# ru-wang/slam-plus-plus

Measured on AMD Instinct MI355X. Metric: Λ-solve block-nnz/sec + batch GN iters/sec, Venice BA, 1→8 MI355X, higher is better.
Workload: dtype f64; 1 GPU; venice871-shaped synthetic BA (871 cams, 530304 points, 2838740 observations, LM-damped); nnzb=3369915, n=1596138, mode=schur+dense, n_reduced=5226, schur_pairs=12875640, parallelism=single GPU

## Files before the change

include/spp_hip.h:

```cpp
#ifndef SPP_HIP_H
#define SPP_HIP_H

#include <stddef.h>
#include <stdint.h>

#ifdef __cplusplus
extern "C" {
#endif

#define SPP_OK            0
#define SPP_NOT_POSDEF    1
#define SPP_E_BADARG     -1
#define SPP_E_NOMEM      -2
#define SPP_E_HIP        -3
#define SPP_E_NO_DEVICE  -4
#define SPP_E_STATE      -5
#define SPP_E_UNSUPPORTED -6

#define SPP_MODE_AUTO     0
#define SPP_MODE_SPARSE   1
#define SPP_MODE_SCHUR    2
#define SPP_MODE_SCHUR_SPARSE 3

#define SPP_FLAG_PROFILE  1
#define SPP_FLAG_SCHUR_PARTIAL 2

typedef struct spp_ctx spp_ctx;

spp_ctx *spp_create(int device, int flags);
void spp_destroy(spp_ctx *ctx);
int spp_free_memory(spp_ctx *ctx);
int spp_last_error(const spp_ctx *ctx, char *buf, size_t buf_size);
double *spp_host_staging(spp_ctx *ctx, int64_t n_doubles);
int spp_set_stream(spp_ctx *ctx, void *hip_stream);
int spp_synchronize(spp_ctx *ctx);

int spp_analyze(spp_ctx *ctx, int64_t nb, const int64_t *h_col_ptr, const int64_t *h_row_idx,
	const int64_t *h_blk_off, const int32_t *h_dim, int mode);

int spp_set_shard(spp_ctx *ctx, int rank, int world_size);

#define SPP_MODE_SCHUR_MIS 4

#define SPP_INFO_MODE           0
#define SPP_INFO_N              1
#define SPP_INFO_NNZB           2
#define SPP_INFO_NVALS          3
#define SPP_INFO_FACTOR_NNZ     4
#define SPP_INFO_FACTOR_FLOPS   5
#define SPP_INFO_N_REDUCED      6
#define SPP_INFO_N_POSES        7
#define SPP_INFO_N_LANDMARKS    8
#define SPP_INFO_SCHUR_PAIRS    9
#define SPP_INFO_N_OBS          10
#define SPP_INFO_SOLVE_BYTES    11
#define SPP_INFO_N_SUPERNODES   12
#define SPP_INFO_N_LEVELS       13
#define SPP_INFO_S_LD           14
#define SPP_INFO_S_NNZB         15
#define SPP_INFO_DENSE_STREAMED 16
int spp_get_info(const spp_ctx *ctx, int what, int64_t *out);
int spp_get_ordering(const spp_ctx *ctx, int64_t *h_order);

#define SPP_ORDER_AMD 0
#define SPP_ORDER_ND  1
int spp_block_ordering(int64_t nb, const int64_t *col_ptr, const int64_t *row_idx, int method, int64_t *h_order);

int spp_schur_plan_host(int64_t nb, const int32_t *dim, const int64_t *col_ptr, const int64_t *row_idx, int shard_rank,
	int shard_world, int sparse_S, int64_t *out, double *seconds);

int spp_factor_solve(spp_ctx *ctx, const double *h_vals, double *h_rhs_inout);

int spp_factor_solve_device(spp_ctx *ctx, const double *d_vals, double *d_rhs_inout);

int spp_schur_buffer_size(const spp_ctx *ctx, int64_t *n_doubles);
int spp_schur_form(spp_ctx *ctx, const double *d_vals, const double *d_rhs, double *d_S_rhs);
int spp_schur_finish(spp_ctx *ctx, const double *d_vals, double *d_S_rhs, double *d_rhs_inout);
int spp_schur_packed_size(const spp_ctx *ctx, int64_t *n_doubles);
int spp_schur_pack(spp_ctx *ctx, const double *d_S_rhs, double *d_packed);
int spp_schur_unpack(spp_ctx *ctx, const double *d_packed, double *d_S_rhs);

int spp_assemble_analyze(spp_ctx *ctx, int64_t nv, const int32_t *h_dim,
	int64_t ne, const int64_t *h_v0, const int64_t *h_v1, int d0, int d1, int rd,
	int64_t unary_vertex);
int spp_assemble_get_structure(const spp_ctx *ctx, int64_t *h_col_ptr, int64_t *h_row_idx,
	int64_t *h_blk_off);
int spp_assemble_device(spp_ctx *ctx, const double *d_J0, const double *d_J1,
	const double *d_Omega, const double *d_r, double damping, double *d_vals_out, double *d_eta_out);
int spp_assemble_set_edge_weights(spp_ctx *ctx, const double *d_w);
int spp_edge_robust_weights_device(spp_ctx *ctx, int64_t n_edges, int rd, int kind, double scale, double param,
	const double *d_r, double *d_w_out);

int spp_se2_linearize_device(spp_ctx *ctx, int64_t n_edges, const int32_t *d_v0, const int32_t *d_v1,
	const double *d_poses, const double *d_measurements, double *d_J0, double *d_J1, double *d_r);
int spp_se2_update_device(spp_ctx *ctx, int64_t n_vertices, double *d_poses, const double *d_dx, int apply,
	double *h_dx_norm2);

int spp_se3_linearize_device(spp_ctx *ctx, int64_t n_edges, const int32_t *d_v0, const int32_t *d_v1,
	const double *d_poses, const double *d_measurements, double *d_J0, double *d_J1, double *d_r);
int spp_se3_update_device(spp_ctx *ctx, int64_t n_vertices, double *d_poses, const double *d_dx, int apply,
	double *h_dx_norm2);

int spp_ba_linearize_device(spp_ctx *ctx, int64_t n_obs, const int32_t *d_cam_of, const int32_t *d_pt_of,
	const double *d_cams, const double *d_intrinsics, const double *d_points, const double *d_measurements,
	double *d_J0, double *d_J1, double *d_r);
int spp_ba_update_device(spp_ctx *ctx, int64_t n_cams, double *d_cams, const int64_t *d_cam_dxoff,
	int64_t n_points, double *d_points, const int64_t *d_pt_dxoff, const double *d_dx, int64_t n_dx, int apply,
	double *h_dx_norm2);

int spp_edge_chi2_device(spp_ctx *ctx, int64_t n_edges, int rd, const double *d_r, const double *d_Omega, double *h_chi2);
int spp_edge_hessian_maxdiag_device(spp_ctx *ctx, int64_t n_edges, int rd, int d0, int d1, const double *d_J0,
	const double *d_J1, const double *d_Omega, double *h_max);
int spp_lm_gain_denominator_device(spp_ctx *ctx, int64_t n, const double *d_dx, const double *d_eta, double alpha,
	double *h_out);

int spp_device_malloc(spp_ctx *ctx, size_t bytes, void **d_ptr);
int spp_device_free(spp_ctx *ctx, void *d_ptr);
int spp_memcpy_h2d(spp_ctx *ctx, void *d_dst, const void *h_src, size_t bytes);
int spp_memcpy_d2h(spp_ctx *ctx, void *h_dst, const void *d_src, size_t bytes);
int spp_memcpy_d2d(spp_ctx *ctx, void *d_dst, const void *d_src, size_t bytes);

int spp_set_profiling(spp_ctx *ctx, int on);

#define SPP_PHASE_PERMUTE   0
#define SPP_PHASE_SCHUR_INV 1
#define SPP_PHASE_SCHUR_GEMM 2
#define SPP_PHASE_SCHUR_RHS 3
#define SPP_PHASE_FACTOR    4
#define SPP_PHASE_TRISOLVE  5
#define SPP_PHASE_BACKSUBST 6
#define SPP_PHASE_ASSEMBLE  7
#define SPP_PHASE_TOTAL     8
#define SPP_N_PHASES        9
int spp_get_phase_ms(spp_ctx *ctx, double *ms_out );
int spp_get_dominant_kernel(spp_ctx *ctx, double *ms_total, int64_t *n_launches, double *flops);

int spp_microbench_copy(spp_ctx *ctx, size_t bytes, int iters, double *gb_per_s);
int spp_microbench_mfma_f64(spp_ctx *ctx, int iters, double *tflops);
int spp_microbench_ctile(spp_ctx *ctx, int n, int iters, double *gb_per_s);
int spp_microbench_update(spp_ctx *ctx, int64_t m, int iters, double *ms_per_launch);

int spp_dense_potrf_upper(spp_ctx *ctx, double *d_A, int64_t n, int64_t ld);
int spp_dense_posv(spp_ctx *ctx, double *d_A, int64_t n, int64_t ld, double *d_b);
int spp_dense_posv_masked(spp_ctx *ctx, double *d_A, int64_t n, int64_t ld, double *d_b, const uint64_t *words, int64_t nwords);
int spp_tile_mask_host(int64_t n, int bs, int64_t nblk, const int32_t *i1, const int32_t *i2, int has_rhs, int fill,
	uint64_t *words, int64_t *n_updates);
int spp_schur_tile_mask_host(int64_t nb, const int32_t *dim, const int64_t *col_ptr, const int64_t *row_idx, int shard_rank,
	int shard_world, uint64_t *words);
int spp_tail_order_host(int64_t n, int has_rhs, const uint64_t *words, int64_t nwords, int resident, int early, double beta,
	int32_t *table, int32_t *info);
int spp_dense_gemm_tn_sub(spp_ctx *ctx, int64_t m, int64_t n, int64_t k,
	const double *d_A, int64_t lda, const double *d_B, int64_t ldb, double *d_C, int64_t ldc);
int spp_dense_gemm_tn_sub_upper(spp_ctx *ctx, int64_t m, int64_t n, int64_t k,
	const double *d_A, int64_t lda, const double *d_B, int64_t ldb, double *d_C, int64_t ldc);
int spp_dense_front_factor(spp_ctx *ctx, double *d_F, int64_t ld, int64_t w, int64_t h, double *d_image);

const char *spp_version(void);

#ifdef __cplusplus
}
#endif
#endif
```

slam_plus_plus_amd/api.py:

```python
import ctypes
import os

import numpy as np

_HERE = os.path.dirname(os.path.abspath(__file__))
LIB_PATH = os.environ.get("SPP_LIB") or os.path.join(_HERE, "libspp_hip.so")

SPP_OK, SPP_NOT_POSDEF = 0, 1
MODE_AUTO, MODE_SPARSE, MODE_SCHUR, MODE_SCHUR_SPARSE, MODE_SCHUR_MIS = 0, 1, 2, 3, 4
FLAG_PROFILE = 1
INFO = dict(MODE=0, N=1, NNZB=2, NVALS=3, FACTOR_NNZ=4, FACTOR_FLOPS=5, N_REDUCED=6, N_POSES=7,
            N_LANDMARKS=8, SCHUR_PAIRS=9, N_OBS=10, SOLVE_BYTES=11, N_SUPERNODES=12, N_LEVELS=13, S_LD=14, S_NNZB=15, DENSE_STREAMED=16)
PHASES = ["permute", "schur_inv", "schur_gemm", "schur_rhs", "factor", "trisolve", "backsubst", "assemble", "total"]

EXPORTS = [
    "spp_create", "spp_destroy", "spp_free_memory", "spp_last_error", "spp_host_staging", "spp_set_stream", "spp_synchronize",
    "spp_analyze", "spp_set_shard", "spp_get_info", "spp_get_ordering", "spp_factor_solve",
    "spp_factor_solve_device", "spp_schur_buffer_size", "spp_schur_form", "spp_schur_finish",
    "spp_schur_packed_size", "spp_schur_pack", "spp_schur_unpack",
    "spp_assemble_analyze", "spp_assemble_get_structure", "spp_assemble_device", "spp_assemble_set_edge_weights", "spp_device_malloc",
    "spp_device_free", "spp_memcpy_h2d", "spp_memcpy_d2h", "spp_memcpy_d2d", "spp_get_phase_ms", "spp_get_dominant_kernel",
    "spp_microbench_copy", "spp_microbench_mfma_f64", "spp_microbench_ctile", "spp_microbench_update", "spp_block_ordering", "spp_schur_plan_host", "spp_set_profiling", "spp_se2_linearize_device", "spp_se2_update_device", "spp_ba_linearize_device", "spp_ba_update_device", "spp_se3_linearize_device", "spp_se3_update_device", "spp_edge_chi2_device", "spp_edge_robust_weights_device", "spp_edge_hessian_maxdiag_device",
    "spp_lm_gain_denominator_device", "spp_dense_potrf_upper", "spp_dense_posv",
    "spp_dense_posv_masked", "spp_tile_mask_host", "spp_schur_tile_mask_host", "spp_tail_order_host",
    "spp_dense_gemm_tn_sub", "spp_dense_gemm_tn_sub_upper", "spp_dense_front_factor", "spp_version",
]

_lib = None
_c_i64p = ctypes.POINTER(ctypes.c_int64)
_c_i32p = ctypes.POINTER(ctypes.c_int32)
_c_f64p = ctypes.POINTER(ctypes.c_double)


class SppError(RuntimeError):
    """std::runtime_error of the C++ adapter (reference LinearSolver_Schur_GPU.cpp:734-797)."""


def load_library():
    global _lib
    if _lib is not None:
        return _lib
    if not os.path.exists(LIB_PATH):
        raise SppError("libspp_hip.so is not built: run `python -m slam_plus_plus_amd.build` "
                       "(hipcc --offload-arch=gfx950); there is no CPU fallback")
    lib = ctypes.CDLL(LIB_PATH)
    vp, i64, i32, dbl, cint = ctypes.c_void_p, ctypes.c_int64, ctypes.c_int32, ctypes.c_double, ctypes.c_int
    sig = {
        "spp_create": (vp, [cint, cint]),
        "spp_destroy": (None, [vp]),
        "spp_free_memory": (cint, [vp]),
        "spp_last_error": (cint, [vp, ctypes.c_char_p, ctypes.c_size_t]),
        "spp_host_staging": (vp, [vp, i64]),
        "spp_set_stream": (cint, [vp, vp]),
        "spp_synchronize": (cint, [vp]),
        "spp_analyze": (cint, [vp, i64, vp, vp, vp, vp, cint]),
        "spp_set_shard": (cint, [vp, cint, cint]),
        "spp_get_info": (cint, [vp, cint, _c_i64p]),
        "spp_get_ordering": (cint, [vp, vp]),
        "spp_factor_solve": (cint, [vp, vp, vp]),
        "spp_factor_solve_device": (cint, [vp, vp, vp]),
        "spp_schur_buffer_size": (cint, [vp, _c_i64p]),
        "spp_schur_form": (cint, [vp, vp, vp, vp]),
        "spp_schur_finish": (cint, [vp, vp, vp, vp]),
        "spp_schur_packed_size": (cint, [vp, _c_i64p]),
        "spp_schur_pack": (cint, [vp, vp, vp]),
        "spp_schur_unpack": (cint, [vp, vp, vp]),
        "spp_assemble_analyze": (cint, [vp, i64, vp, i64, vp, vp, cint, cint, cint, i64]),
        "spp_assemble_get_structure": (cint, [vp, vp, vp, vp]),
        "spp_assemble_device": (cint, [vp, vp, vp, vp, vp, dbl, vp, vp]),
        "spp_assemble_set_edge_weights": (cint, [vp, vp]),
        "spp_device_malloc": (cint, [vp, ctypes.c_size_t, ctypes.POINTER(vp)]),
        "spp_device_free": (cint, [vp, vp]),
        "spp_memcpy_h2d": (cint, [vp, vp, vp, ctypes.c_size_t]),
        "spp_memcpy_d2h": (cint, [vp, vp, vp, ctypes.c_size_t]),
        "spp_memcpy_d2d": (cint, [vp, vp, vp, ctypes.c_size_t]),
        "spp_get_phase_ms": (cint, [vp, _c_f64p]),
        "spp_get_dominant_kernel": (cint, [vp, _c_f64p, _c_i64p, _c_f64p]),
        "spp_microbench_copy": (cint, [vp, ctypes.c_size_t, cint, _c_f64p]),
        "spp_microbench_mfma_f64": (cint, [vp, cint, _c_f64p]),
        "spp_microbench_ctile": (cint, [vp, cint, cint, _c_f64p]),
        "spp_microbench_update": (cint, [vp, ctypes.c_int64, cint, _c_f64p]),
        "spp_block_ordering": (cint, [ctypes.c_int64, vp, vp, cint, vp]),
        "spp_schur_plan_host": (cint, [ctypes.c_int64, vp, vp, vp, cint, cint, cint, vp, vp]),
        "spp_set_profiling": (cint, [vp, cint]),
        "spp_se2_linearize_device": (cint, [vp, ctypes.c_int64, vp, vp, vp, vp, vp, vp, vp]),
        "spp_se2_update_device": (cint, [vp, ctypes.c_int64, vp, vp, cint, _c_f64p]),
        "spp_se3_linearize_device": (cint, [vp, ctypes.c_int64, vp, vp, vp, vp, vp, vp, vp]),
        "spp_se3_update_device": (cint, [vp, ctypes.c_int64, vp, vp, cint, _c_f64p]),
        "spp_edge_chi2_device": (cint, [vp, ctypes.c_int64, cint, vp, vp, _c_f64p]),
        "spp_edge_robust_weights_device": (cint, [vp, ctypes.c_int64, cint, cint, dbl, dbl, vp, vp]),
        "spp_edge_hessian_maxdiag_device": (cint, [vp, ctypes.c_int64, cint, cint, cint, vp, vp, vp, _c_f64p]),
        "spp_lm_gain_denominator_device": (cint, [vp, ctypes.c_int64, vp, vp, ctypes.c_double, _c_f64p]),
        "spp_ba_linearize_device": (cint, [vp, ctypes.c_int64, vp, vp, vp, vp, vp, vp, vp, vp, vp]),
        "spp_ba_update_device": (cint, [vp, ctypes.c_int64, vp, vp, ctypes.c_int64, vp, vp, vp, ctypes.c_int64, cint, _c_f64p]),
        "spp_dense_potrf_upper": (cint, [vp, vp, i64, i64]),
        "spp_dense_posv": (cint, [vp, vp, i64, i64, vp]),
        "spp_dense_posv_masked": (cint, [vp, vp, i64, i64, vp, vp, i64]),
        "spp_tile_mask_host": (cint, [i64, cint, i64, vp, vp, cint, cint, vp, vp]),
        "spp_schur_tile_mask_host": (cint, [i64, vp, vp, vp, cint, cint, vp]),
        "spp_tail_order_host": (cint, [i64, cint, vp, i64, cint, cint, dbl, vp, vp]),
        "spp_dense_gemm_tn_sub": (cint, [vp, i64, i64, i64, vp, i64, vp, i64, vp, i64]),
        "spp_dense_gemm_tn_sub_upper": (cint, [vp, i64, i64, i64, vp, i64, vp, i64, vp, i64]),
        "spp_dense_front_factor": (cint, [vp, vp, i64, i64, i64, vp]),
        "spp_version": (ctypes.c_char_p, []),
    }
    for name, (res, args) in sig.items():
        fn = getattr(lib, name)
        fn.restype = res
        fn.argtypes = args
    _lib = lib
    return lib


def _ptr(a):
    return a.ctypes.data_as(ctypes.c_void_p)


ORDER_AMD, ORDER_ND = 0, 1


def block_ordering(lam, method=ORDER_AMD):
    lib = load_library()
    col_ptr = np.ascontiguousarray(lam.col_ptr, dtype=np.int64)
    row_idx = np.ascontiguousarray(lam.row_idx, dtype=np.int64)
    out = np.empty(lam.nb, dtype=np.int64)
    code = lib.spp_block_ordering(lam.nb, _ptr(col_ptr), _ptr(row_idx), method, _ptr(out))
    if code != 0:
        raise SppError("spp_block_ordering failed: %d" % code)
    return out


def schur_plan_host(lam, shard_rank=0, shard_world=1, sparse_S=False, mis=False):
    lib = load_library()
    col_ptr = np.ascontiguousarray(lam.col_ptr, dtype=np.int64)
    row_idx = np.ascontiguousarray(lam.row_idx, dtype=np.int64)
    dim = np.ascontiguousarray(lam.dim, dtype=np.int32)
    out = np.zeros(8, dtype=np.int64)
    sec = ctypes.c_double(0.0)
    code = lib.spp_schur_plan_host(lam.nb, _ptr(dim), _ptr(col_ptr), _ptr(row_idx), shard_rank, shard_world,
                                   (1 if sparse_S else 0) | (2 if mis else 0), _ptr(out), ctypes.byref(sec))
    if code != 0:
        raise SppError("spp_schur_plan_host failed: %d" % code)
    keys = ("nc", "nl", "no", "n_pairs", "n_sblk", "n_items", "n_multi", "checksum")
    d = dict(zip(keys, (int(v) for v in out)))
    d["seconds"] = sec.value
    return d


def tile_mask_host(n, bs, i1, i2, has_rhs=True, fill=True):
    lib = load_library()
    i1 = np.ascontiguousarray(i1, dtype=np.int32)
    i2 = np.ascontiguousarray(i2, dtype=np.int32)
    words = np.zeros(64, dtype=np.uint64)
    upd = ctypes.c_int64(0)
    code = lib.spp_tile_mask_host(n, bs, i1.size, _ptr(i1), _ptr(i2), 1 if has_rhs else 0, 1 if fill else 0, _ptr(words),
                                  ctypes.byref(upd))
    if code < 0:
        raise SppError("spp_tile_mask_host failed: %d" % code)
    return words[:code].copy(), upd.value


def schur_tile_mask_host(lam, shard_rank=0, shard_world=1):
    lib = load_library()
    col_ptr = np.ascontiguousarray(lam.col_ptr, dtype=np.int64)
    row_idx = np.ascontiguousarray(lam.row_idx, dtype=np.int64)
    dim = np.ascontiguousarray(lam.dim, dtype=np.int32)
    words = np.zeros(64, dtype=np.uint64)
    code = lib.spp_schur_tile_mask_host(lam.nb, _ptr(dim), _ptr(col_ptr), _ptr(row_idx), shard_rank, shard_world, _ptr(words))
    if code < 0:
        raise SppError("spp_schur_tile_mask_host failed: %d" % code)
    return words[:code].copy()


def tail_order_host(n, words, has_rhs=True, resident=256, early=True, beta=0.0):
    lib = load_library()
    words = np.ascontiguousarray(words if words is not None else [], dtype=np.uint64)
    table = np.zeros(64 * 65 // 2 + 64, dtype=np.int32)
    info = np.zeros(5, dtype=np.int32)
    code = lib.spp_tail_order_host(int(n), 1 if has_rhs else 0, _ptr(words) if words.size else None, words.size, int(resident),
                                   1 if early else 0, float(beta), _ptr(table), _ptr(info))
    if code < 0:
        raise SppError("spp_tail_order_host failed: %d" % code)
    tiles = [(int(t) >> 16, int(t) & 0xffff) for t in table[:code]]
    return tiles, dict(zip(("n_early", "r_star", "rows_resident", "live_demand", "widest"), (int(v) for v in info)))


class DeviceArray:

    def __init__(self, ctx, n, dtype=np.float64):
        self.ctx, self.n, self.dtype = ctx, int(n), np.dtype(dtype)
        p = ctypes.c_void_p()
        ctx._check(ctx.lib.spp_device_malloc(ctx.h, self.n * self.dtype.itemsize, ctypes.byref(p)))
        self.ptr = p.value

    @classmethod
    def from_host(cls, ctx, arr):
        arr = np.ascontiguousarray(arr)
        d = cls(ctx, arr.size, arr.dtype)
        d.upload(arr)
        return d

    def upload(self, arr):
        arr = np.ascontiguousarray(arr, dtype=self.dtype)
        assert arr.size == self.n
        self.ctx._check(self.ctx.lib.spp_memcpy_h2d(self.ctx.h, self.ptr, _ptr(arr), arr.nbytes))

    def download(self):
        out = np.empty(self.n, dtype=self.dtype)
        self.ctx._check(self.ctx.lib.spp_memcpy_d2h(self.ctx.h, _ptr(out), self.ptr, out.nbytes))
        return out

    def copy_from(self, other):
        assert other.n * other.dtype.itemsize <= self.n * self.dtype.itemsize
        self.ctx._check(self.ctx.lib.spp_memcpy_d2d(self.ctx.h, self.ptr, other.ptr, other.n * other.dtype.itemsize))

    def free(self):
        if self.ptr:
            self.ctx.lib.spp_device_free(self.ctx.h, self.ptr)
            self.ptr = None


class Context:

    def __init__(self, device=0, flags=0):
        self.lib = load_library()
        self.h = self.lib.spp_create(int(device), int(flags))
        if not self.h:
            raise SppError("spp_create failed: no usable HIP device %d (the solver has no CPU fallback)" % device)

    def close(self):
        if getattr(self, "h", None):
            self.lib.spp_destroy(self.h)
            self.h = None

    def __del__(self):
        try:
            self.close()
        except Exception:
            pass

    def last_error(self):
        buf = ctypes.create_string_buffer(1024)
        self.lib.spp_last_error(self.h, buf, 1024)
        return buf.value.decode(errors="replace")

    def _check(self, code):
        if code < 0:
            if code == -2:
                raise MemoryError(self.last_error())
            raise SppError("spp error %d: %s" % (code, self.last_error()))
        return code

    def analyze(self, bcsc, mode=MODE_AUTO):
        self._keep = bcsc
        return self._check(self.lib.spp_analyze(self.h, bcsc.nb, _ptr(bcsc.col_ptr), _ptr(bcsc.row_idx),
                                                 _ptr(bcsc.blk_off), _ptr(bcsc.dim), mode))

    def set_shard(self, rank, world):
        return self._check(self.lib.spp_set_shard(self.h, rank, world))

    def info(self, key):
        out = ctypes.c_int64()
        self._check(self.lib.spp_get_info(self.h, INFO[key], ctypes.byref(out)))
        return out.value

    def ordering(self, nb):
        out = np.empty(nb, dtype=np.int64)
        self._check(self.lib.spp_get_ordering(self.h, _ptr(out)))
        return out

    def se2_linearize_device(self, n_edges, d_v0, d_v1, d_poses, d_meas, d_J0, d_J1, d_r):
        return self._check(self.lib.spp_se2_linearize_device(self.h, n_edges, d_v0, d_v1, d_poses, d_meas, d_J0, d_J1, d_r))

    def se2_update_device(self, n_vertices, d_poses, d_dx, apply=True):
        out = ctypes.c_double()
        self._check(self.lib.spp_se2_update_device(self.h, n_vertices, d_poses, d_dx, 1 if apply else 0, ctypes.byref(out)))
        return out.value ** 0.5

    def se3_linearize_device(self, n_edges, d_v0, d_v1, d_poses, d_meas, d_J0, d_J1, d_r):
        return self._check(self.lib.spp_se3_linearize_device(self.h, n_edges, d_v0, d_v1, d_poses, d_meas, d_J0, d_J1, d_r))

    def se3_update_device(self, n_vertices, d_poses, d_dx, apply=True):
        out = ctypes.c_double()
        self._check(self.lib.spp_se3_update_device(self.h, n_vertices, d_poses, d_dx, 1 if apply else 0, ctypes.byref(out)))
        return out.value ** 0.5

    def edge_robust_weights_device(self, n_edges, rd, d_r, d_w, scale, param=1.345, kind=0):
        return self._check(self.lib.spp_edge_robust_weights_device(self.h, n_edges, rd, kind, float(scale), float(param), d_r, d_w))

    def edge_chi2_device(self, n_edges, rd, d_r, d_Om):
        out = ctypes.c_double()
        self._check(self.lib.spp_edge_chi2_device(self.h, n_edges, rd, d_r, d_Om, ctypes.byref(out)))
        return out.value

    def edge_hessian_maxdiag_device(self, n_edges, rd, d0, d1, d_J0, d_J1, d_Om):
        out = ctypes.c_double()
        self._check(self.lib.spp_edge_hessian_maxdiag_device(self.h, n_edges, rd, d0, d1, d_J0, d_J1, d_Om, ctypes.byref(out)))
        return out.value

    def lm_gain_denominator_device(self, n, d_dx, d_eta, alpha):
        out = ctypes.c_double()
        self._check(self.lib.spp_lm_gain_denominator_device(self.h, n, d_dx, d_eta, float(alpha), ctypes.byref(out)))
        return out.value

    def ba_linearize_device(self, n_obs, d_cam_of, d_pt_of, d_cams, d_intr, d_points, d_meas, d_J0, d_J1, d_r):
        return self._check(self.lib.spp_ba_linearize_device(self.h, n_obs, d_cam_of, d_pt_of, d_cams, d_intr, d_points,
                                                            d_meas, d_J0, d_J1, d_r))

    def ba_update_device(self, n_cams, d_cams, d_cam_dxoff, n_points, d_points, d_pt_dxoff, d_dx, n_dx, apply=True):
        out = ctypes.c_double()
        self._check(self.lib.spp_ba_update_device(self.h, n_cams, d_cams, d_cam_dxoff, n_points, d_points, d_pt_dxoff,
                                                  d_dx, n_dx, 1 if apply else 0, ctypes.byref(out)))
        return out.value ** 0.5

    def set_profiling(self, on):
        return self._check(self.lib.spp_set_profiling(self.h, 1 if on else 0))

    def set_stream(self, stream_handle):
        return self._check(self.lib.spp_set_stream(self.h, ctypes.c_void_p(stream_handle)))

    def synchronize(self):
        return self._check(self.lib.spp_synchronize(self.h))

    def host_staging(self, n):
        p = self.lib.spp_host_staging(self.h, int(n))
        if not p:
            raise MemoryError(self.last_error())
        return np.ctypeslib.as_array(ctypes.cast(p, ctypes.POINTER(ctypes.c_double)), shape=(int(n),))

    def factor_solve(self, vals, rhs):
        vals = np.ascontiguousarray(vals, dtype=np.float64)
        x = np.array(rhs, dtype=np.float64, copy=True)
        code = self._check(self.lib.spp_factor_solve(self.h, _ptr(vals), _ptr(x)))
        return code, x

    def factor_solve_device(self, d_vals, d_rhs):
        return self._check(self.lib.spp_factor_solve_device(self.h, d_vals, d_rhs))

    def schur_buffer_size(self):
        out = ctypes.c_int64()
        self._check(self.lib.spp_schur_buffer_size(self.h, ctypes.byref(out)))
        return out.value

    def schur_packed_size(self):
        out = ctypes.c_int64()
        self._check(self.lib.spp_schur_packed_size(self.h, ctypes.byref(out)))
        return out.value

    def schur_pack(self, d_S, d_packed):
        return self._check(self.lib.spp_schur_pack(self.h, d_S, d_packed))

    def schur_unpack(self, d_packed, d_S):
        return self._check(self.lib.spp_schur_unpack(self.h, d_packed, d_S))

    def schur_form(self, d_vals, d_rhs, d_S):
        return self._check(self.lib.spp_schur_form(self.h, d_vals, d_rhs, d_S))

    def schur_finish(self, d_vals, d_S, d_rhs):
        return self._check(self.lib.spp_schur_finish(self.h, d_vals, d_S, d_rhs))

    def assemble_analyze(self, dim, v0, v1, d0, d1, rd, unary_vertex=-1):
        dim = np.ascontiguousarray(dim, dtype=np.int32)
        v0 = np.ascontiguousarray(v0, dtype=np.int64)
        v1 = np.ascontiguousarray(v1, dtype=np.int64)
        self._check(self.lib.spp_assemble_analyze(self.h, dim.size, _ptr(dim), v0.size, _ptr(v0), _ptr(v1),
                                                   d0, d1, rd, int(unary_vertex)))
        nb, nnzb = dim.size, self.info("NNZB")
        col_ptr = np.empty(nb + 1, dtype=np.int64)
        row_idx = np.empty(nnzb, dtype=np.int64)
        blk_off = np.empty(nnzb, dtype=np.int64)
        self._check(self.lib.spp_assemble_get_structure(self.h, _ptr(col_ptr), _ptr(row_idx), _ptr(blk_off)))
        from .blockcsc import BlockCSC
        return BlockCSC(dim, col_ptr, row_idx, blk_off, None, nvals=self.info("NVALS"))

    def assemble_set_edge_weights(self, d_w):
        return self._check(self.lib.spp_assemble_set_edge_weights(self.h, d_w))

    def assemble_device(self, d_J0, d_J1, d_Om, d_r, damping, d_vals, d_eta):
        return self._check(self.lib.spp_assemble_device(self.h, d_J0, d_J1, d_Om, d_r, float(damping), d_vals, d_eta))

    def phase_ms(self):
        out = np.zeros(len(PHASES))
        self._check(self.lib.spp_get_phase_ms(self.h, out.ctypes.data_as(_c_f64p)))
        return dict(zip(PHASES, out.tolist()))

    def dominant_kernel(self):
        ms, n, fl = ctypes.c_double(), ctypes.c_int64(), ctypes.c_double()
        self._check(self.lib.spp_get_dominant_kernel(self.h, ctypes.byref(ms), ctypes.byref(n), ctypes.byref(fl)))
        return ms.value, n.value, fl.value

    def microbench_copy(self, nbytes=1 << 30, iters=10):
        out = ctypes.c_double()
        self._check(self.lib.spp_microbench_copy(self.h, nbytes, iters, ctypes.byref(out)))
        return out.value

    def microbench_ctile(self, n=8192, iters=10):
        out = ctypes.c_double()
        self._check(self.lib.spp_microbench_ctile(self.h, n, iters, ctypes.byref(out)))
        return out.value

    def microbench_update(self, m=5120, iters=20):
        out = ctypes.c_double()
        self._check(self.lib.spp_microbench_update(self.h, m, iters, ctypes.byref(out)))
        return out.value

    def microbench_mfma_f64(self, iters=4000):
        out = ctypes.c_double()
        self._check(self.lib.spp_microbench_mfma_f64(self.h, iters, ctypes.byref(out)))
        return out.value


class CLinearSolver_HIP:
    _Tag = "CBlockwiseLinearSolverTag"

    def __init__(self, device=0, mode=MODE_AUTO, flags=0):
        self._ctx = Context(device, flags)
        self._mode = mode
        self._have_symbolic = False
        self._sig = None

    def Free_Memory(self):
        self._ctx._check(self._ctx.lib.spp_free_memory(self._ctx.h))
        self._have_symbolic = False

    def Clear_SymbolicDecomposition(self):
        self._have_symbolic = False

    def SymbolicDecomposition_Blocky(self, r_lambda):
        self._ctx.analyze(r_lambda, self._mode)
        self._have_symbolic = True
        self._sig = self._signature(r_lambda)
        return True

    @staticmethod
    def _signature(r_lambda):
        try:
            import xxhash
            h = xxhash.xxh3_64()
            for a in (r_lambda.col_ptr, r_lambda.row_idx, r_lambda.dim):
                h.update(np.ascontiguousarray(a).view(np.uint8))
            digest = h.intdigest()
        except ImportError:
            import zlib
            digest = 0
            for a in (r_lambda.col_ptr, r_lambda.row_idx, r_lambda.dim):
                digest = zlib.adler32(np.ascontiguousarray(a).view(np.uint8), digest)
        return (r_lambda.nb, r_lambda.nnzb, digest)

    def Solve_PosDef_Blocky(self, r_lambda, r_eta):
        assert r_eta.shape[0] == r_lambda.n, "eta length must equal the matrix dimension"
        if not self._have_symbolic or self._sig is None or self._sig != self._signature(r_lambda):
            self.SymbolicDecomposition_Blocky(r_lambda)
        code, x = self._ctx.factor_solve(r_lambda.vals, r_eta)
        if code == SPP_NOT_POSDEF:
            return False
        r_eta[:] = x
        return True

    def Solve_PosDef(self, r_lambda, r_eta):
        self.Clear_SymbolicDecomposition()
        return self.Solve_PosDef_Blocky(r_lambda, r_eta)

    @property
    def ctx(self):
        return self._ctx
```

slam_plus_plus_amd/csrc/spp_api.cpp:

```cpp

#include "spp_internal.h"
#include <string.h>
#include <new>

using namespace spp;

namespace spp {

void phases_reset(spp_ctx *ctx)
{
	if(!(ctx->flags & SPP_FLAG_PROFILE))
		return;
	if(!ctx->timer.created) {
		for(int i = 0; i < 2 * SPP_N_PHASES; ++ i)
			SPP_HIP_CHECK(hipEventCreate(&ctx->timer.ev[i]));
		ctx->timer.created = true;
	}
	for(int i = 0; i < SPP_N_PHASES; ++ i) {
		ctx->timer.used[i] = false;
		ctx->phase_ms[i] = 0;
	}
	ctx->dom_used = 0;
	ctx->dom_flops = 0;
}
// ... 166 lines not shown
	if(!ctx || n_doubles < 0)
		return nullptr;
	if((size_t)n_doubles <= ctx->h_staging_cap && ctx->h_staging)
		return ctx->h_staging;
	(void)hipSetDevice(ctx->device);
	(void)hipStreamSynchronize(ctx->stream);
	if(ctx->h_staging) {
		(void)hipHostFree(ctx->h_staging);
		ctx->h_staging = nullptr;
		ctx->h_staging_cap = 0;
	}
	const size_t want = (size_t)(n_doubles > 0 ? n_doubles : 1);
	if(hipHostMalloc((void**)&ctx->h_staging, want * sizeof(double), hipHostMallocDefault) != hipSuccess) {
		(void)hipGetLastError();
		ctx->h_staging = nullptr;
		ctx->last_error = "hipHostMalloc of the staging buffer failed";
		return nullptr;
	}
	ctx->h_staging_cap = want;
	return ctx->h_staging;
}

int spp_set_stream(spp_ctx *ctx, void *hip_stream)
{
	if(!ctx)
		return SPP_E_BADARG;
	(void)hipStreamSynchronize(ctx->stream);
	if(ctx->own_stream && ctx->stream)
		(void)hipStreamDestroy(ctx->stream);
	ctx->stream = (hipStream_t)hip_stream;
	ctx->own_stream = false;
	return SPP_OK;
}

int spp_synchronize(spp_ctx *ctx)
{
	if(!ctx)
		return SPP_E_BADARG;
	SPP_TRY(ctx)
	SPP_HIP_CHECK(hipStreamSynchronize(ctx->stream));
	dense_chain_check(ctx);
	return SPP_OK;
	SPP_CATCH(ctx)
}

int spp_set_profiling(spp_ctx *ctx, int on)
{
	if(!ctx)
		return SPP_E_BADARG;
	ctx->flags = on ? (ctx->flags | SPP_FLAG_PROFILE) : (ctx->flags & ~SPP_FLAG_PROFILE);
	return SPP_OK;
}

int spp_set_shard(spp_ctx *ctx, int rank, int world_size)
{
	if(!ctx || world_size < 1 || rank < 0 || rank >= world_size)
		return SPP_E_BADARG;
	ctx->shard_rank = rank;
	ctx->shard_world = world_size;
	return SPP_OK;
}

int spp_analyze(spp_ctx *ctx, int64_t nb, const int64_t *col_ptr, const int64_t *row_idx,
	const int64_t *blk_off, const int32_t *dim, int mode)
{
	if(!ctx)
		return SPP_E_BADARG;
	SPP_TRY(ctx)
	SPP_REQUIRE(nb > 0 && col_ptr && row_idx && blk_off && dim, SPP_E_BADARG, "spp_analyze: null or empty structure");
	SPP_REQUIRE(col_ptr[0] == 0 && col_ptr[nb] >= nb, SPP_E_BADARG, "spp_analyze: column pointers must start at 0 and hold every diagonal block");
	SPP_HIP_CHECK(hipSetDevice(ctx->device));
	ctx->mode = -1;
	VClock clk("spp_analyze");
	Structure st;
	st.nb = nb;
	st.nnzb = col_ptr[nb];
	st.col_ptr.assign(col_ptr, col_ptr + nb + 1);
	SPP_REQUIRE(st.nnzb >= nb, SPP_E_BADARG, "spp_analyze: fewer blocks than block columns");
	for(int64_t j = 0; j < nb; ++ j)
		SPP_REQUIRE(col_ptr[j + 1] > col_ptr[j], SPP_E_BADARG, "every block column needs its diagonal block");
	st.dim.assign(dim, dim + nb);
	st.base.resize(nb + 1);
	st.base[0] = 0;
	for(int64_t j = 0; j < nb; ++ j) {
		SPP_REQUIRE(dim[j] > 0 && dim[j] <= 8, SPP_E_BADARG, "block widths must be in 1..8");
		st.base[j + 1] = st.base[j] + dim[j];
	}
	st.n = st.base[nb];
	st.row_idx.resize(st.nnzb);
	st.blk_off.resize(st.nnzb);
	{
		const int nt = plan_threads(st.nnzb);
		std::vector<int64_t> jcut, nvals_t(nt, 0);
		balanced_cuts(st.col_ptr, nt, jcut);
		run_threads(nt, [&](int t) {
			const int64_t p0 = col_ptr[jcut[t]], p1 = col_ptr[jcut[t + 1]];
			if(p1 > p0) {
				memcpy(st.row_idx.data() + p0, row_idx + p0, (size_t)(p1 - p0) * sizeof(int64_t));
				memcpy(st.blk_off.data() + p0, blk_off + p0, (size_t)(p1 - p0) * sizeof(int64_t));
			}
			int64_t nv = 0;
			for(int64_t j = jcut[t]; j < jcut[t + 1]; ++ j) {
				for(int64_t p = col_ptr[j]; p < col_ptr[j + 1]; ++ p) {
					const int64_t i = row_idx[p];
					SPP_REQUIRE(i >= 0 && i <= j, SPP_E_BADARG, "only the upper triangle may be stored");
					SPP_REQUIRE(p == col_ptr[j] || row_idx[p - 1] < i, SPP_E_BADARG, "rows must ascend within a column");
					SPP_REQUIRE(blk_off[p] >= 0, SPP_E_BADARG, "negative block offset");
					nv = std::max<int64_t>(nv, blk_off[p] + (int64_t)dim[i] * dim[j]);
				}
				SPP_REQUIRE(row_idx[col_ptr[j + 1] - 1] == j, SPP_E_BADARG, "diagonal block missing (must be last in its column)");
			}
			nvals_t[t] = nv;
		});
		st.nvals = 0;
		for(int t = 0; t < nt; ++ t)
			st.nvals = std::max(st.nvals, nvals_t[t]);
	}
	ctx->st = std::move(st);
	Structure &st_ref = ctx->st;
	clk.lap("structure copied + validated");
	ctx->schur.release_all();
	sparse_release(ctx);
	clk.lap("old plans released");
	int dp, dl;
	int chosen = mode;
	if(mode == SPP_MODE_AUTO) {
		chosen = SPP_MODE_SPARSE;
		if(schur_applicable(st_ref, &dp, &dl)) {
			int64_t n_red = 0;
			for(int64_t j = 0; j < nb; ++ j)
				n_red += (dim[j] == dp) ? dp : 0;
			chosen = (n_red <= 16384) ? SPP_MODE_SCHUR : SPP_MODE_SCHUR_SPARSE;
		}
	}
	SPP_REQUIRE(chosen == SPP_MODE_SCHUR || chosen == SPP_MODE_SPARSE || chosen == SPP_MODE_SCHUR_SPARSE ||
		chosen == SPP_MODE_SCHUR_MIS, SPP_E_BADARG, "unknown mode");
	SPP_REQUIRE((chosen != SPP_MODE_SPARSE && chosen != SPP_MODE_SCHUR_MIS) || ctx->shard_world == 1, SPP_E_UNSUPPORTED,
		"only the Schur modes shard (over landmarks); pose graphs run as replicas (DESIGN.md, multi-GPU)");
	ctx->mode = -1;
	if(chosen == SPP_MODE_SCHUR || chosen == SPP_MODE_SCHUR_SPARSE || chosen == SPP_MODE_SCHUR_MIS) {
		const bool mis = chosen == SPP_MODE_SCHUR_MIS;
		const bool sparse_S = chosen != SPP_MODE_SCHUR;
		build_schur_plan(ctx, sparse_S, mis);
		clk.lap("schur plan (all of it)");
		ctx->schur.mis = mis;
		ctx->order.clear();
		ctx->order.reserve((size_t)st_ref.nb);
		if(sparse_S) {
			sparse_analyze(ctx, ctx->schur.s_st);
			std::vector<int64_t> red = ctx->order;
			ctx->order.clear();
			for(size_t i = 0; i < red.size(); ++ i)
				ctx->order.push_back(ctx->schur.pose_block[red[i]]);
			chosen = SPP_MODE_SCHUR;
		} else
		for(size_t i = 0; i < ctx->schur.pose_block.size(); ++ i)
			ctx->order.push_back(ctx->schur.pose_block[i]);
		for(int64_t j = 0; j < st_ref.nb; ++ j)
			if(ctx->schur.is_lm[j])
				ctx->order.push_back(j);
	} else
		sparse_analyze(ctx, ctx->st);
	ctx->mode = chosen;
	clk.lap("plan + ordering");
	return SPP_OK;
	SPP_CATCH(ctx)
}

int spp_get_info(const spp_ctx *ctx, int what, int64_t *out)
{
	if(!ctx || !out)
		return SPP_E_BADARG;
	if(ctx->mode < 0 && what != SPP_INFO_NNZB && what != SPP_INFO_NVALS && what != SPP_INFO_N && what != SPP_INFO_DENSE_STREAMED)
		return SPP_E_STATE;
	switch(what) {
	case SPP_INFO_MODE: *out = (ctx->mode != SPP_MODE_SCHUR) ? ctx->mode : ctx->schur.mis ? SPP_MODE_SCHUR_MIS :
		ctx->schur.sparse_S ? SPP_MODE_SCHUR_SPARSE : SPP_MODE_SCHUR; break;
	case SPP_INFO_N: *out = ctx->st.n; break;
	case SPP_INFO_NNZB: *out = ctx->st.nnzb; break;
	case SPP_INFO_NVALS: *out = ctx->st.nvals; break;
	case SPP_INFO_FACTOR_NNZ: *out = ctx->factor_nnz; break;
	case SPP_INFO_FACTOR_FLOPS: *out = ctx->factor_flops; break;
	case SPP_INFO_N_REDUCED: *out = (ctx->mode == SPP_MODE_SCHUR) ? ctx->schur.n_red : 0; break;
	case SPP_INFO_N_POSES: *out = (ctx->mode == SPP_MODE_SCHUR) ? ctx->schur.nc : ctx->st.nb; break;
	case SPP_INFO_N_LANDMARKS: *out = (ctx->mode == SPP_MODE_SCHUR) ? ctx->schur.nl : 0; break;
	case SPP_INFO_SCHUR_PAIRS: *out = (ctx->mode == SPP_MODE_SCHUR) ? ctx->schur.n_pairs : 0; break;
	case SPP_INFO_N_OBS: *out = (ctx->mode == SPP_MODE_SCHUR) ? ctx->schur.no : 0; break;
	case SPP_INFO_SOLVE_BYTES: *out = ctx->solve_bytes; break;
	case SPP_INFO_N_SUPERNODES: *out = ctx->sparse ? sparse_info(ctx, what) : 0; break;
	case SPP_INFO_N_LEVELS: *out = ctx->sparse ? sparse_info(ctx, what) : 0; break;
	case SPP_INFO_S_LD: *out = (ctx->mode == SPP_MODE_SCHUR && !ctx->schur.sparse_S) ? ctx->schur.ld : 0; break;
	case SPP_INFO_S_NNZB: *out = (ctx->mode == SPP_MODE_SCHUR) ? ctx->schur.n_sblk : 0; break;
	case SPP_INFO_DENSE_STREAMED: *out = ctx->dense.tail_rows_last; break;
	default: return SPP_E_BADARG;
	}
	return SPP_OK;
}

int spp_get_ordering(const spp_ctx *ctx, int64_t *h_order)
{
	if(!ctx || !h_order)
		return SPP_E_BADARG;
	if(ctx->mode < 0)
		return SPP_E_STATE;
	for(size_t i = 0; i < ctx->order.size(); ++ i)
		h_order[i] = ctx->order[i];
	return SPP_OK;
}

int spp_block_ordering(int64_t nb, const int64_t *col_ptr, const int64_t *row_idx, int method, int64_t *h_order)
{
	if(nb <= 0 || !col_ptr || !row_idx || !h_order || (method != SPP_ORDER_AMD && method != SPP_ORDER_ND))
		return SPP_E_BADARG;
	try {
		for(int64_t j = 0; j < nb; ++ j)
			for(int64_t p = col_ptr[j]; p < col_ptr[j + 1]; ++ p)
				if(row_idx[p] < 0 || row_idx[p] > j)
					return SPP_E_BADARG;
		std::vector<int64_t> order;
		if(method == SPP_ORDER_AMD)
			min_degree_order(nb, col_ptr, row_idx, order);
		else
			nested_dissection_order(nb, col_ptr, row_idx, order);
		for(int64_t k = 0; k < nb; ++ k)
			h_order[k] = order[k];
		return SPP_OK;
	} catch(const std::bad_alloc &) {
		return SPP_E_NOMEM;
	} catch(...) {
		return SPP_E_HIP;
	}
}

static bool structure_of_pattern(int64_t nb, const int32_t *dim, const int64_t *col_ptr, const int64_t *row_idx, Structure &st)
{
	st.nb = nb;
	st.nnzb = col_ptr[nb];
	st.col_ptr.assign(col_ptr, col_ptr + nb + 1);
	st.row_idx.assign(row_idx, row_idx + st.nnzb);
	st.dim.assign(dim, dim + nb);
	st.base.resize(nb + 1);
	st.base[0] = 0;
	for(int64_t j = 0; j < nb; ++ j)
		st.base[j + 1] = st.base[j] + dim[j];
	st.n = st.base[nb];
	st.blk_off.resize(st.nnzb);
	int64_t off = 0;
	for(int64_t j = 0; j < nb; ++ j)
		for(int64_t p = col_ptr[j]; p < col_ptr[j + 1]; ++ p) {
			if(row_idx[p] < 0 || row_idx[p] > j)
				return false;
			st.blk_off[p] = off;
			off += (int64_t)dim[row_idx[p]] * dim[j];
		}
	st.nvals = off;
	return true;
}

int spp_schur_plan_host(int64_t nb, const int32_t *dim, const int64_t *col_ptr, const int64_t *row_idx, int shard_rank,
	int shard_world, int sparse_S, int64_t *out, double *seconds)
{
	if(nb <= 0 || !dim || !col_ptr || !row_idx || !out || shard_world < 1 || shard_rank < 0 || shard_rank >= shard_world)
		return SPP_E_BADARG;
	try {
		Structure st;
		if(!structure_of_pattern(nb, dim, col_ptr, row_idx, st))
			return SPP_E_BADARG;
		const double sec = schur_plan_host_probe(st, shard_rank, shard_world, (sparse_S & 1) != 0, (sparse_S & 2) != 0, out);
		if(seconds)
			*seconds = sec;
		return SPP_OK;
	} catch(const Error &e) {
		return e.code;
	} catch(const std::bad_alloc &) {
		return SPP_E_NOMEM;
	} catch(...) {
		return SPP_E_HIP;
	}
}

int spp_schur_tile_mask_host(int64_t nb, const int32_t *dim, const int64_t *col_ptr, const int64_t *row_idx, int shard_rank,
	int shard_world, uint64_t *words)
{
	if(nb <= 0 || !dim || !col_ptr || !row_idx || !words || shard_world < 1 || shard_rank < 0 || shard_rank >= shard_world)
		return SPP_E_BADARG;
	try {
		Structure st;
		if(!structure_of_pattern(nb, dim, col_ptr, row_idx, st))
			return SPP_E_BADARG;
		std::vector<uint64_t> w;
		schur_tile_mask_host_probe(st, shard_rank, shard_world, w);
		for(size_t q = 0; q < w.size(); ++ q)
			words[q] = w[q];
		return (int)w.size();
	} catch(const Error &e) {
		return e.code;
	} catch(const std::bad_alloc &) {
		return SPP_E_NOMEM;
	} catch(...) {
		return SPP_E_HIP;
	}
}

int spp_schur_buffer_size(const spp_ctx *ctx, int64_t *n_doubles)
{
	if(!ctx || !n_doubles)
		return SPP_E_BADARG;
	if(ctx->mode != SPP_MODE_SCHUR)
		return SPP_E_STATE;
	*n_doubles = schur_buffer_doubles(ctx);
	return SPP_OK;
}

int spp_schur_form(spp_ctx *ctx, const double *d_vals, const double *d_rhs, double *d_S_rhs)
{
	if(!ctx || !d_vals || !d_rhs || !d_S_rhs)
		return SPP_E_BADARG;
	SPP_TRY(ctx)
	SPP_REQUIRE(ctx->mode == SPP_MODE_SCHUR, SPP_E_STATE, "spp_schur_form: analyze in Schur mode first");
	SPP_HIP_CHECK(hipSetDevice(ctx->device));
	phases_reset(ctx);
	phase_begin(ctx, SPP_PHASE_TOTAL);
	schur_form(ctx, d_vals, d_rhs, d_S_rhs);
	return SPP_OK;
	SPP_CATCH(ctx)
}

int spp_schur_packed_size(const spp_ctx *ctx, int64_t *n_doubles)
{
	if(!ctx || !n_doubles)
		return SPP_E_BADARG;
	if(ctx->mode != SPP_MODE_SCHUR)
		return SPP_E_STATE;
	if(ctx->schur.sparse_S) {
		*n_doubles = schur_buffer_doubles(ctx);
		return SPP_OK;
	}
	const int64_t nblk = ctx->schur.ld / DENSE_NB;
	*n_doubles = (int64_t)DENSE_NB * DENSE_NB * (nblk * (nblk + 1) / 2);
	return SPP_OK;
}

int spp_schur_pack(spp_ctx *ctx, const double *d_S_rhs, double *d_packed)
{
	if(!ctx || !d_S_rhs || !d_packed)
		return SPP_E_BADARG;
	SPP_TRY(ctx)
	SPP_REQUIRE(ctx->mode == SPP_MODE_SCHUR, SPP_E_STATE, "spp_schur_pack: analyze in Schur mode first");
	SPP_HIP_CHECK(hipSetDevice(ctx->device));
	if(ctx->schur.sparse_S)
		SPP_HIP_CHECK(hipMemcpyAsync(d_packed, d_S_rhs, (size_t)schur_buffer_doubles(ctx) * sizeof(double),
			hipMemcpyDeviceToDevice, ctx->stream));
	else
		schur_pack(ctx, const_cast<double*>(d_S_rhs), d_packed, true);
	return SPP_OK;
	SPP_CATCH(ctx)
}

int spp_schur_unpack(spp_ctx *ctx, const double *d_packed, double *d_S_rhs)
{
	if(!ctx || !d_S_rhs || !d_packed)
		return SPP_E_BADARG;
	SPP_TRY(ctx)
	SPP_REQUIRE(ctx->mode == SPP_MODE_SCHUR, SPP_E_STATE, "spp_schur_unpack: analyze in Schur mode first");
	SPP_HIP_CHECK(hipSetDevice(ctx->device));
	if(ctx->schur.sparse_S)
		SPP_HIP_CHECK(hipMemcpyAsync(d_S_rhs, d_packed, (size_t)schur_buffer_doubles(ctx) * sizeof(double),
			hipMemcpyDeviceToDevice, ctx->stream));
	else
		schur_pack(ctx, d_S_rhs, const_cast<double*>(d_packed), false);
	return SPP_OK;
	SPP_CATCH(ctx)
}

int spp_schur_finish(spp_ctx *ctx, const double *d_vals, double *d_S_rhs, double *d_rhs_inout)
{
	if(!ctx || !d_vals || !d_rhs_inout || !d_S_rhs)
		return SPP_E_BADARG;
	SPP_TRY(ctx)
	SPP_REQUIRE(ctx->mode == SPP_MODE_SCHUR, SPP_E_STATE, "spp_schur_finish: analyze in Schur mode first");
	SPP_HIP_CHECK(hipSetDevice(ctx->device));
	int ret = schur_finish(ctx, d_vals, d_S_rhs, d_rhs_inout);
	phase_end(ctx, SPP_PHASE_TOTAL);
	phases_collect(ctx);
	dense_chain_check(ctx);
	return ret;
	SPP_CATCH(ctx)
}

int spp_factor_solve_device(spp_ctx *ctx, const double *d_vals, double *d_rhs)
{
	if(!ctx || !d_vals || !d_rhs)
		return SPP_E_BADARG;
	SPP_TRY(ctx)
	SPP_REQUIRE(ctx->mode >= 0, SPP_E_STATE, "spp_factor_solve: call spp_analyze first");
	SPP_HIP_CHECK(hipSetDevice(ctx->device));
	phases_reset(ctx);
	phase_begin(ctx, SPP_PHASE_TOTAL);
	int ret;
	if(ctx->mode == SPP_MODE_SCHUR) {
		SPP_REQUIRE(ctx->shard_world == 1, SPP_E_STATE,
			"sharded ctx: use spp_schur_form / all-reduce / spp_schur_finish");
		ctx->schur.S.reserve((size_t)schur_buffer_doubles(ctx));
		schur_form(ctx, d_vals, d_rhs, ctx->schur.S.p);
		ret = schur_finish(ctx, d_vals, ctx->schur.S.p, d_rhs);
	} else
		ret = sparse_factor_solve(ctx, d_vals, d_rhs);
	phase_end(ctx, SPP_PHASE_TOTAL);
	phases_collect(ctx);
	SPP_HIP_CHECK(hipStreamSynchronize(ctx->stream));
	dense_chain_check(ctx);
	return ret;
	SPP_CATCH(ctx)
}

int spp_factor_solve(spp_ctx *ctx, const double *h_vals, double *h_rhs)
{
	if(!ctx || !h_vals || !h_rhs)
		return SPP_E_BADARG;
	SPP_TRY(ctx)
	SPP_REQUIRE(ctx->mode >= 0, SPP_E_STATE, "spp_factor_solve: call spp_analyze first");
	SPP_HIP_CHECK(hipSetDevice(ctx->device));
	ctx->d_vals.reserve((size_t)ctx->st.nvals);
	ctx->d_rhs.reserve((size_t)ctx->st.n);
	SPP_HIP_CHECK(hipMemcpyAsync(ctx->d_vals.p, h_vals, ctx->st.nvals * sizeof(double), hipMemcpyHostToDevice, ctx->stream));
	SPP_HIP_CHECK(hipMemcpyAsync(ctx->d_rhs.p, h_rhs, ctx->st.n * sizeof(double), hipMemcpyHostToDevice, ctx->stream));
	int ret = spp_factor_solve_device(ctx, ctx->d_vals.p, ctx->d_rhs.p);
	if(ret != SPP_OK)
		return ret;
	SPP_HIP_CHECK(hipMemcpyAsync(h_rhs, ctx->d_rhs.p, ctx->st.n * sizeof(double), hipMemcpyDeviceToHost, ctx->stream));
	SPP_HIP_CHECK(hipStreamSynchronize(ctx->stream));
	return SPP_OK;
	SPP_CATCH(ctx)
}

int spp_assemble_analyze(spp_ctx *ctx, int64_t nv, const int32_t *h_dim, int64_t ne, const int64_t *h_v0,
	const int64_t *h_v1, int d0, int d1, int rd, int64_t unary_vertex)
{
	if(!ctx || !h_dim || !h_v0 || !h_v1 || nv <= 0 || ne <= 0)
		return SPP_E_BADARG;
	SPP_TRY(ctx)
	SPP_HIP_CHECK(hipSetDevice(ctx->device));
	assemble_analyze(ctx, nv, h_dim, ne, h_v0, h_v1, d0, d1, rd, unary_vertex);
	return SPP_OK;
	SPP_CATCH(ctx)
}

int spp_assemble_get_structure(const spp_ctx *ctx, int64_t *h_col_ptr, int64_t *h_row_idx, int64_t *h_blk_off)
{
	if(!ctx || !ctx->assemble)
		return SPP_E_STATE;
	assemble_get_structure(ctx, h_col_ptr, h_row_idx, h_blk_off);
	return SPP_OK;
}

int spp_assemble_device(spp_ctx *ctx, const double *d_J0, const double *d_J1, const double *d_Omega,
	const double *d_r, double damping, double *d_vals_out, double *d_eta_out)
{
	if(!ctx || !d_J0 || !d_J1 || !d_Omega || !d_r || !d_vals_out || !d_eta_out)
		return SPP_E_BADARG;
	SPP_TRY(ctx)
	SPP_REQUIRE(ctx->assemble, SPP_E_STATE, "spp_assemble_device: call spp_assemble_analyze first");
	SPP_HIP_CHECK(hipSetDevice(ctx->device));
	phases_reset(ctx);
	phase_begin(ctx, SPP_PHASE_ASSEMBLE);
	assemble_run(ctx, d_J0, d_J1, d_Omega, d_r, damping, d_vals_out, d_eta_out);
	phase_end(ctx, SPP_PHASE_ASSEMBLE);
	phases_collect(ctx);
	return SPP_OK;
	SPP_CATCH(ctx)
}

int spp_assemble_set_edge_weights(spp_ctx *ctx, const double *d_w)
{
	if(!ctx)
		return SPP_E_BADARG;
	SPP_TRY(ctx)
	SPP_REQUIRE(ctx->assemble, SPP_E_STATE, "spp_assemble_set_edge_weights: call spp_assemble_analyze first");
	assemble_set_edge_weights(ctx, d_w);
	return SPP_OK;
	SPP_CATCH(ctx)
}

int spp_se2_linearize_device(spp_ctx *ctx, int64_t n_edges, const int32_t *d_v0, const int32_t *d_v1,
	const double *d_poses, const double *d_measurements, double *d_J0, double *d_J1, double *d_r)
{
	if(!ctx || n_edges < 0 || !d_v0 || !d_v1 || !d_poses || !d_measurements || !d_J0 || !d_J1 || !d_r)
		return SPP_E_BADARG;
	SPP_TRY(ctx)
	SPP_HIP_CHECK(hipSetDevice(ctx->device));
	se2_linearize(ctx, n_edges, d_v0, d_v1, d_poses, d_measurements, d_J0, d_J1, d_r);
	return SPP_OK;
	SPP_CATCH(ctx)
}

int spp_se2_update_device(spp_ctx *ctx, int64_t n_vertices, double *d_poses, const double *d_dx, int apply,
	double *h_dx_norm2)
{
	if(!ctx || n_vertices < 0 || !d_poses || !d_dx)
		return SPP_E_BADARG;
	SPP_TRY(ctx)
	SPP_HIP_CHECK(hipSetDevice(ctx->device));
	const double n2 = se2_update(ctx, n_vertices, d_poses, d_dx, apply != 0);
	if(h_dx_norm2)
		*h_dx_norm2 = n2;
	return SPP_OK;
	SPP_CATCH(ctx)
}

int spp_se3_linearize_device(spp_ctx *ctx, int64_t n_edges, const int32_t *d_v0, const int32_t *d_v1,
	const double *d_poses, const double *d_measurements, double *d_J0, double *d_J1, double *d_r)
{
	if(!ctx || n_edges < 0 || !d_v0 || !d_v1 || !d_poses || !d_measurements || !d_J0 || !d_J1 || !d_r)
		return SPP_E_BADARG;
	SPP_TRY(ctx)
	SPP_HIP_CHECK(hipSetDevice(ctx->device));
	se3_linearize(ctx, n_edges, d_v0, d_v1, d_poses, d_measurements, d_J0, d_J1, d_r);
	return SPP_OK;
	SPP_CATCH(ctx)
}

int spp_se3_update_device(spp_ctx *ctx, int64_t n_vertices, double *d_poses, const double *d_dx, int apply,
	double *h_dx_norm2)
{
	if(!ctx || n_vertices < 0 || !d_poses || !d_dx)
		return SPP_E_BADARG;
	SPP_TRY(ctx)
	SPP_HIP_CHECK(hipSetDevice(ctx->device));
	const double n2 = se3_update(ctx, n_vertices, d_poses, d_dx, apply != 0);
	if(h_dx_norm2)
		*h_dx_norm2 = n2;
	return SPP_OK;
	SPP_CATCH(ctx)
}

int spp_ba_linearize_device(spp_ctx *ctx, int64_t n_obs, const int32_t *d_cam_of, const int32_t *d_pt_of,
	const double *d_cams, const double *d_intrinsics, const double *d_points, const double *d_measurements,
	double *d_J0, double *d_J1, double *d_r)
{
	if(!ctx || n_obs < 0 || !d_cam_of || !d_pt_of || !d_cams || !d_intrinsics || !d_points || !d_measurements ||
	   !d_J0 || !d_J1 || !d_r)
		return SPP_E_BADARG;
	SPP_TRY(ctx)
	SPP_HIP_CHECK(hipSetDevice(ctx->device));
	ba_linearize(ctx, n_obs, d_cam_of, d_pt_of, d_cams, d_intrinsics, d_points, d_measurements, d_J0, d_J1, d_r);
	return SPP_OK;
	SPP_CATCH(ctx)
}

int spp_ba_update_device(spp_ctx *ctx, int64_t n_cams, double *d_cams, const int64_t *d_cam_dxoff,
	int64_t n_points, double *d_points, const int64_t *d_pt_dxoff, const double *d_dx, int64_t n_dx, int apply,
	double *h_dx_norm2)
{
	if(!ctx || n_cams < 0 || n_points < 0 || n_dx < 0 || !d_dx || (n_cams && (!d_cams || !d_cam_dxoff)) ||
	   (n_points && (!d_points || !d_pt_dxoff)))
		return SPP_E_BADARG;
	SPP_TRY(ctx)
	SPP_HIP_CHECK(hipSetDevice(ctx->device));
	const double n2 = ba_update(ctx, n_cams, d_cams, d_cam_dxoff, n_points, d_points, d_pt_dxoff, d_dx, n_dx, apply != 0);
	if(h_dx_norm2)
		*h_dx_norm2 = n2;
	return SPP_OK;
	SPP_CATCH(ctx)
}

int spp_edge_robust_weights_device(spp_ctx *ctx, int64_t n_edges, int rd, int kind, double scale, double param,
	const double *d_r, double *d_w_out)
{
	if(!ctx || n_edges < 0 || !d_r || !d_w_out)
		return SPP_E_BADARG;
	SPP_TRY(ctx)
	SPP_HIP_CHECK(hipSetDevice(ctx->device));
	edge_robust_weights(ctx, n_edges, rd, kind, scale, param, d_r, d_w_out);
	return SPP_OK;
	SPP_CATCH(ctx)
}

int spp_edge_chi2_device(spp_ctx *ctx, int64_t n_edges, int rd, const double *d_r, const double *d_Omega, double *h_chi2)
{
	if(!ctx || n_edges < 0 || !d_r || !d_Omega || !h_chi2)
		return SPP_E_BADARG;
	SPP_TRY(ctx)
	SPP_HIP_CHECK(hipSetDevice(ctx->device));
	*h_chi2 = edge_chi2(ctx, n_edges, rd, d_r, d_Omega);
	return SPP_OK;
	SPP_CATCH(ctx)
}

int spp_edge_hessian_maxdiag_device(spp_ctx *ctx, int64_t n_edges, int rd, int d0, int d1, const double *d_J0,
	const double *d_J1, const double *d_Omega, double *h_max)
{
	if(!ctx || n_edges < 0 || !d_J0 || !d_J1 || !d_Omega || !h_max)
		return SPP_E_BADARG;
	SPP_TRY(ctx)
	SPP_HIP_CHECK(hipSetDevice(ctx->device));
	*h_max = edge_hessian_maxdiag(ctx, n_edges, rd, d0, d1, d_J0, d_J1, d_Omega);
	return SPP_OK;
	SPP_CATCH(ctx)
}

int spp_lm_gain_denominator_device(spp_ctx *ctx, int64_t n, const double *d_dx, const double *d_eta, double alpha,
	double *h_out)
{
	if(!ctx || n < 0 || !d_dx || !d_eta || !h_out)
		return SPP_E_BADARG;
	SPP_TRY(ctx)
// ... 279 lines not shown
```

slam_plus_plus_amd/csrc/spp_internal.h:

```cpp
#pragma once

#include <hip/hip_runtime.h>
#include <stdint.h>
#include <string>
#include <vector>
#include <sys/mman.h>
#include <utility>
#include <new>
#include <exception>
#include <thread>
#include <stdexcept>
#include <algorithm>
#include <string.h>
#include <chrono>
#include <stdio.h>
#include <stdlib.h>
#include "../../include/spp_hip.h"
#include "spp_switches.h"

namespace spp {

struct Error : std::runtime_error {
	int code;
	Error(int c, const std::string &what) : std::runtime_error(what), code(c) {}
};

#define SPP_HIP_CHECK(expr) do { hipError_t e_ = (expr); if(e_ != hipSuccess) \
	throw spp::Error(SPP_E_HIP, std::string(#expr " failed: ") + hipGetErrorString(e_)); } while(0)
#define SPP_REQUIRE(cond, code, msg) do { if(!(cond)) throw spp::Error((code), (msg)); } while(0)

inline bool first_on_this_device(uint64_t &seen)
{
	int dev = 0;
	(void)hipGetDevice(&dev);
	const uint64_t bit = uint64_t(1) << (dev & 63);
	if(seen & bit)
		return false;
	seen |= bit;
	return true;
}

struct VClock {
	const char *who;
	std::chrono::steady_clock::time_point t;
	bool on;
	explicit VClock(const char *w) : who(w), t(std::chrono::steady_clock::now()), on(switches().verbose) {}
	void lap(const char *what)
	{
		if(!on)
			return;
		const std::chrono::steady_clock::time_point n = std::chrono::steady_clock::now();
		fprintf(stderr, "[spp] %s: %-34s %8.2f ms\n", who, what, std::chrono::duration<double>(n - t).count() * 1e3);
		t = n;
	}
};

template <class T>
struct HugeAlloc {
	typedef T value_type;
	HugeAlloc() {}
	template <class U> HugeAlloc(const HugeAlloc<U>&) {}
	T *allocate(size_t n)
	{
		const size_t bytes = n * sizeof(T), huge = (size_t)2 << 20;
		void *q = nullptr;
		if(bytes >= ((size_t)4 << 20)) {
			if(posix_memalign(&q, huge, (bytes + huge - 1) & ~(huge - 1)) != 0)
				q = nullptr;
#ifdef MADV_HUGEPAGE
			if(q)
				madvise(q, bytes, MADV_HUGEPAGE);
#endif
		}
		if(!q)
			q = malloc(bytes ? bytes : 1);
		if(!q)
			throw std::bad_alloc();
		return (T*)q;
	}
	void deallocate(T *p, size_t) { free(p); }
	template <class U> void construct(U *p) { ::new((void*)p) U; }
	template <class U, class A0, class... A> void construct(U *p, A0 &&a0, A &&... a) { ::new((void*)p) U(std::forward<A0>(a0), std::forward<A>(a)...); }
	template <class U> bool operator==(const HugeAlloc<U>&) const { return true; }
	template <class U> bool operator!=(const HugeAlloc<U>&) const { return false; }
};
template <class T> using HVec = std::vector<T, HugeAlloc<T> >;

template <class T>
struct DevBuf {
	T *p = nullptr;
	size_t cap = 0;
	bool owned = true;
	DevBuf() {}
	DevBuf(const DevBuf&) = delete;
	DevBuf &operator=(const DevBuf&) = delete;
	~DevBuf() { release(); }
	void release()
	{
		if(p && owned)
			(void)hipFree(p);
		p = nullptr;
		cap = 0;
		owned = true;
	}
	void view(T *ptr, size_t n)
	{
		release();
		p = ptr;
		cap = n;
		owned = false;
	}
	void reserve(size_t n)
	{
		if(n <= cap && owned)
			return;
		release();
		size_t want = n;
		hipError_t e = hipMalloc((void**)&p, want * sizeof(T));
		if(e != hipSuccess) {
			p = nullptr;
			throw Error(SPP_E_NOMEM, "hipMalloc of " + std::to_string(want * sizeof(T)) + " bytes failed");
		}
		cap = want;
	}
	template <class A>
	void upload(const std::vector<T, A> &h, hipStream_t s)
	{
		reserve(h.size() ? h.size() : 1);
		if(!h.empty())
			SPP_HIP_CHECK(hipMemcpyAsync(p, h.data(), h.size() * sizeof(T), hipMemcpyHostToDevice, s));
	}
};

struct UploadArena {
	hipStream_t stream;
	std::vector<unsigned char> host;
	struct Item { void **pp; size_t *pcap; bool *powned; size_t off, n; };
	std::vector<Item> items;
	explicit UploadArena(hipStream_t s) : stream(s) { host.reserve(size_t(1) << 20); }
	template <class T, class A>
	void add(DevBuf<T> &b, const std::vector<T, A> &v)
	{
		if(v.size() * sizeof(T) > (size_t(256) << 10)) {
			b.upload(v, stream);
			return;
		}
		b.release();
		const size_t off = (host.size() + 255) & ~(size_t)255, bytes = std::max<size_t>(v.size(), 1) * sizeof(T);
		host.resize(off + bytes);
		if(!v.empty())
			memcpy(host.data() + off, v.data(), v.size() * sizeof(T));
		Item it = {(void**)&b.p, &b.cap, &b.owned, off, std::max<size_t>(v.size(), 1)};
		items.push_back(it);
	}
	void commit(DevBuf<unsigned char> &store)
	{
		store.release();
		store.reserve(std::max<size_t>(host.size(), 256));
		if(!host.empty())
			SPP_HIP_CHECK(hipMemcpyAsync(store.p, host.data(), host.size(), hipMemcpyHostToDevice, stream));
		for(size_t i = 0; i < items.size(); ++ i) {
			*items[i].pp = store.p + items[i].off;
			*items[i].pcap = items[i].n;
			*items[i].powned = false;
		}
	}
};

struct Structure {
	int64_t nb = 0, n = 0, nnzb = 0, nvals = 0;
	HVec<int64_t> col_ptr, row_idx, blk_off, base;
	HVec<int32_t> dim;
};

struct SaccItem {
	int32_t beg, end;
	int32_t kind;
	int32_t pad;
	int64_t dst;
	int64_t aoff;
};

struct SchurPlan {
	int dp = 0, dl = 0;
	int64_t nc = 0, nl = 0;
	int64_t nl_total = 0;
	int64_t no = 0;
	int64_t n_red = 0, ld = 0;
	int64_t n_sblk = 0;
	int64_t n_pairs = 0;
	int64_t n_items = 0, n_multi = 0;
	bool add_A = true;
	bool u_landmark_major = true;
	bool factored = true;
	bool sparse_S = false;
	bool mis = false;
	Structure s_st;
	DevBuf<int64_t> sblk_voff;
	std::vector<int64_t> pose_block;
	std::vector<int64_t> lm_block;
	std::vector<uint8_t> is_lm;
	std::vector<uint64_t> tile_mask;
	DevBuf<int32_t> lm_ptr;
	DevBuf<int32_t> bs_ptr;
	int64_t n_bs = 0;
	DevBuf<int64_t> lm_coff;
	DevBuf<int64_t> lm_rbase;
	DevBuf<int32_t> obs_pose;
	DevBuf<int32_t> obs_lm;
	DevBuf<int64_t> obs_off;
	DevBuf<int64_t> pose_rbase;
	DevBuf<int32_t> cam_ptr;
	DevBuf<int32_t> cam_obs;
	DevBuf<int32_t> obs_wpos;
	DevBuf<SaccItem> items;
	DevBuf<int32_t> xcd_beg;
	int32_t xcd_max_items = 0;
	DevBuf<int32_t> sblk_i1, sblk_i2;
	DevBuf<int64_t> sblk_aoff;
	DevBuf<int32_t> pair_a, pair_b;
	DevBuf<int32_t> multi_blk;
	DevBuf<int32_t> multi_ptr;
	DevBuf<double> cinv;
	DevBuf<double> lfac;
	DevBuf<double> W;
	DevBuf<double> Up;
	DevBuf<double> xw;
	DevBuf<double> partial;
	DevBuf<double> S;
	void release_all();
};

struct DenseWork {
	DevBuf<double> tinv;
	DevBuf<int> info;
	DevBuf<double> tinv_all;
	int64_t tinv_half = 0;
	DevBuf<double> xtmp;
	DevBuf<int> flags;
	DevBuf<int> tail_pub;
	DevBuf<double> tail_dinv;
	int tail_epoch = 0;
	DevBuf<int> tail_order;
	std::vector<int> tail_order_host;
	int tail_order_tr = 0, tail_order_tc = 0;
	std::vector<uint64_t> tail_order_bits;
	bool tail_order_pre = false, tail_order_masked = false;
	int tail_resident = -1;
	const std::vector<uint64_t> *tile_mask = nullptr;
	int tail_rows_last = 0;
	bool tail_disabled = false;
	DevBuf<double> trsv_m;
	DevBuf<double> trsv_pay;
	uint64_t epoch = 0;
	int *h_chain_err = nullptr;
	hipStream_t aux = nullptr;
	hipEvent_t ev[2] = {nullptr, nullptr};
	DevBuf<int> sync;
	DevBuf<int> fuse_cnt;
	std::vector<int> fuse_expect;
	bool fuse_dirty = false;
	int64_t ident_from = -1;
	hipStream_t chain = nullptr;
	hipEvent_t ev_chain = nullptr;
	DevBuf<int> la_cnt;
	DevBuf<long long> la_trace;
	int la_state = 0;
	int la_reserve = 0;
	int la_ncu = 0;
	int sync_epoch = 0;
	int sync_state = 0;
	hipStream_t sync_stream = nullptr;
};

struct SparsePlan;

struct AssemblePlan;

struct PhaseTimer {
	hipEvent_t ev[2 * SPP_N_PHASES];
	bool used[SPP_N_PHASES];
	bool created = false;
};

}

struct spp_ctx {
	int device = 0;
	int flags = 0;
	hipStream_t stream = nullptr;
	bool own_stream = false;
	std::string last_error;
	int mode = -1;
	int shard_rank = 0, shard_world = 1;
	spp::Structure st;
	std::vector<int64_t> order;
	std::thread plan_trash;
	spp::SchurPlan schur;
	spp::DenseWork dense;
	spp::SparsePlan *sparse = nullptr;
	spp::AssemblePlan *assemble = nullptr;
	spp::DevBuf<double> d_vals, d_rhs;
	double *h_staging = nullptr;
	size_t h_staging_cap = 0;
	spp::DevBuf<double> geom_partial;
	spp::PhaseTimer timer;
	double phase_ms[SPP_N_PHASES] = {0};
	std::vector<hipEvent_t> dom_events;
	size_t dom_used = 0;
	double dom_flops = 0;
	int64_t factor_flops = 0, solve_bytes = 0, factor_nnz = 0;
};

namespace spp {

void se2_linearize(spp_ctx *ctx, int64_t ne, const int32_t *d_v0, const int32_t *d_v1, const double *d_poses,
	const double *d_meas, double *d_J0, double *d_J1, double *d_r);
double se2_update(spp_ctx *ctx, int64_t nv, double *d_poses, const double *d_dx, bool apply);
double edge_chi2(spp_ctx *ctx, int64_t ne, int rd, const double *d_r, const double *d_Om);
void edge_robust_weights(spp_ctx *ctx, int64_t ne, int rd, int kind, double scale, double param, const double *d_r, double *d_w);
double edge_hessian_maxdiag(spp_ctx *ctx, int64_t ne, int rd, int d0, int d1, const double *d_J0, const double *d_J1,
	const double *d_Om);
double lm_gain_denominator(spp_ctx *ctx, int64_t n, const double *d_dx, const double *d_rhs, double alpha);
void se3_linearize(spp_ctx *ctx, int64_t ne, const int32_t *d_v0, const int32_t *d_v1, const double *d_poses,
	const double *d_meas, double *d_J0, double *d_J1, double *d_r);
double se3_update(spp_ctx *ctx, int64_t nv, double *d_poses, const double *d_dx, bool apply);
void ba_linearize(spp_ctx *ctx, int64_t no, const int32_t *d_cam_of, const int32_t *d_pt_of, const double *d_cams,
	const double *d_intr, const double *d_pts, const double *d_meas, double *d_J0, double *d_J1, double *d_r);
double ba_update(spp_ctx *ctx, int64_t nc, double *d_cams, const int64_t *d_cam_dxoff, int64_t np, double *d_pts,
	const int64_t *d_pt_dxoff, const double *d_dx, int64_t n_dx, bool apply);

void min_degree_order(int64_t nb, const int64_t *col_ptr, const int64_t *row_idx, std::vector<int64_t> &order);
void nested_dissection_order(int64_t nb, const int64_t *col_ptr, const int64_t *row_idx, std::vector<int64_t> &order);
void build_schur_plan(spp_ctx *ctx, bool sparse_S, bool mis = false);
int64_t schur_buffer_doubles(const spp_ctx *ctx);
bool schur_applicable(const Structure &st, int *dp, int *dl);
double schur_plan_host_probe(const Structure &st, int shard_rank, int shard_world, bool sparse_S, bool mis, int64_t *out);

void sparse_analyze(spp_ctx *ctx, const Structure &st);
int sparse_factor_solve(spp_ctx *ctx, const double *d_vals, double *d_rhs);
void sparse_release(spp_ctx *ctx);
void sparse_dag_disable(spp_ctx *ctx);
int64_t sparse_info(const spp_ctx *ctx, int what);

void schur_form(spp_ctx *ctx, const double *d_vals, const double *d_rhs, double *d_S_rhs);
int schur_finish(spp_ctx *ctx, const double *d_vals, double *d_S_rhs, double *d_rhs);
void schur_pack(spp_ctx *ctx, double *S, double *packed, bool pack);

constexpr int DENSE_NB = 128;
int dense_potrf_upper(spp_ctx *ctx, double *d_A, int64_t n, int64_t ld, bool keep_inverses);
void dense_potrf_upper_enqueue(spp_ctx *ctx, double *d_A, int64_t n, int64_t ld);
int dense_info_fetch(spp_ctx *ctx, bool *dag_aborted = nullptr);
void dense_potrs_upper(spp_ctx *ctx, const double *d_R, int64_t n, int64_t ld, double *d_b);
void dense_aux_park(int device, hipStream_t s);
void dense_factor_steps(spp_ctx *ctx, double *d_A, int64_t ld, int64_t n, int64_t rows, int64_t ncols,
	int64_t nsteps, bool has_rhs);
void dense_info_reset(spp_ctx *ctx);
void dense_reserve(spp_ctx *ctx, int64_t nblk);

void dense_chain_check(spp_ctx *ctx);
void dense_set_padding(spp_ctx *ctx, double *d_A, int64_t ld, int64_t n);
struct TileMaskGuard {
	DenseWork &d;
	TileMaskGuard(DenseWork &dw, const std::vector<uint64_t> *m) : d(dw) { d.tile_mask = (m && !m->empty()) ? m : nullptr; }
	~TileMaskGuard() { d.tile_mask = nullptr; }
};
void tile_mask_mark(int64_t n, int bs, int64_t nblk, const int32_t *i1, const int32_t *i2, std::vector<uint64_t> &words);
int64_t tile_mask_close(int64_t n, bool has_rhs, bool fill, std::vector<uint64_t> &words);
void schur_tile_mask_host_probe(const Structure &st, int shard_rank, int shard_world, std::vector<uint64_t> &words);
void tail_order_table(const std::vector<uint64_t> &bits, int Tr, int Tc, bool have_pre, double beta, int resident, bool early,
	std::vector<int> &order, int *info);
int dense_front_factor(spp_ctx *ctx, double *d_F, int64_t ld, int64_t w, int64_t h, double *d_image);
bool dense_gemm_tn_sub(spp_ctx *ctx, int64_t m, int64_t n, int64_t k, const double *A, int64_t lda,
	const double *B, int64_t ldb, double *C, int64_t ldc, bool upper_only);
double microbench_copy(spp_ctx *ctx, size_t bytes, int iters);
double microbench_mfma_f64(spp_ctx *ctx, int iters);
double microbench_ctile(spp_ctx *ctx, int n, int iters);
double microbench_update(spp_ctx *ctx, int64_t m, int iters);

void assemble_analyze(spp_ctx *ctx, int64_t nv, const int32_t *dim, int64_t ne, const int64_t *v0,
	const int64_t *v1, int d0, int d1, int rd, int64_t unary_vertex);
void assemble_run(spp_ctx *ctx, const double *J0, const double *J1, const double *Om, const double *r,
	double damping, double *vals, double *eta);
void assemble_set_edge_weights(spp_ctx *ctx, const double *d_w);
void assemble_release(spp_ctx *ctx);
void assemble_get_structure(const spp_ctx *ctx, int64_t *col_ptr, int64_t *row_idx, int64_t *blk_off);

void phase_begin(spp_ctx *ctx, int phase);
void phase_end(spp_ctx *ctx, int phase);
void phases_reset(spp_ctx *ctx);
void phases_collect(spp_ctx *ctx);
void dom_begin(spp_ctx *ctx);
void dom_end(spp_ctx *ctx, double flops);

template <class F>
inline void run_threads(int nt, F fn)
{
	if(nt <= 1) {
		fn(0);
		return;
	}
	std::vector<std::thread> th;
	std::exception_ptr err[64];
	for(int t = 1; t < nt; ++ t)
		th.emplace_back([&, t]() { try { fn(t); } catch(...) { err[t] = std::current_exception(); } });
	try { fn(0); } catch(...) { err[0] = std::current_exception(); }
	for(size_t t = 0; t < th.size(); ++ t)
		th[t].join();
	for(int t = 0; t < nt; ++ t)
		if(err[t])
			std::rethrow_exception(err[t]);
}

inline int plan_threads(int64_t work)
{
	const int env = switches().plan_threads;
	int nt = env ? env : (int)std::min<unsigned>(16u, std::max(1u, std::thread::hardware_concurrency()));
	if(work < switches().plan_min_work)
		nt = 1;
	return std::min(nt, 64);
}

template <class V>
inline void balanced_cuts(const V &w_prefix, int nt, std::vector<int64_t> &cut)
{
	const int64_t n = (int64_t)w_prefix.size() - 1, total = w_prefix[n];
	cut.assign(nt + 1, n);
	cut[0] = 0;
	for(int t = 1; t < nt; ++ t)
		cut[t] = std::lower_bound(w_prefix.begin(), w_prefix.end(), total * t / nt) - w_prefix.begin();
	for(int t = 1; t <= nt; ++ t)
		cut[t] = std::max(cut[t], cut[t - 1]);
	cut[nt] = n;
}


}
```

slam_plus_plus_amd/csrc/spp_schur.hip:

```cpp

#include "spp_internal.h"

namespace spp {

template <int DL>
__device__ __forceinline__ void cinv_block(const double *__restrict__ m, double *o)
{
	if(DL == 3) {
#define M_(i, j) m[(i) + 3 * (j)]
#define COF_(i, j) (M_(((i) + 1) % 3, ((j) + 1) % 3) * M_(((i) + 2) % 3, ((j) + 2) % 3) - \
	M_(((i) + 1) % 3, ((j) + 2) % 3) * M_(((i) + 2) % 3, ((j) + 1) % 3))
		const double c00 = COF_(0, 0), c10 = COF_(1, 0), c20 = COF_(2, 0);
		const double det = c00 * M_(0, 0) + c10 * M_(1, 0) + c20 * M_(2, 0);
		const double id = -1.0 / det;
		o[0] = c00 * id; o[3] = c10 * id; o[6] = c20 * id;
		o[1] = COF_(0, 1) * id; o[4] = COF_(1, 1) * id; o[7] = COF_(2, 1) * id;
		o[2] = COF_(0, 2) * id; o[5] = COF_(1, 2) * id; o[8] = COF_(2, 2) * id;
#undef COF_
#undef M_
	} else if(DL == 2) {
		const double det = m[0] * m[3] - m[2] * m[1];
		const double id = -1.0 / det;
		o[0] = m[3] * id; o[2] = -m[2] * id;
		o[1] = -m[1] * id; o[3] = m[0] * id;
	} else {
		double a[DL][DL], b[DL][DL];
#pragma unroll
		for(int i = 0; i < DL; ++ i)
#pragma unroll
			for(int j = 0; j < DL; ++ j) {
				a[i][j] = m[i + DL * j];
				b[i][j] = (i == j) ? 1.0 : 0.0;
			}
#pragma unroll
		for(int k = 0; k < DL; ++ k) {
			const double ip = 1.0 / a[k][k];
#pragma unroll
			for(int j = 0; j < DL; ++ j) {
				a[k][j] *= ip;
				b[k][j] *= ip;
			}
#pragma unroll
			for(int i = 0; i < DL; ++ i) {
				if(i == k)
					continue;
				const double f = a[i][k];
#pragma unroll
				for(int j = 0; j < DL; ++ j) {
					a[i][j] -= f * a[k][j];
					b[i][j] -= f * b[k][j];
				}
			}
		}
#pragma unroll
		for(int i = 0; i < DL; ++ i)
#pragma unroll
			for(int j = 0; j < DL; ++ j)
				o[i + DL * j] = -b[i][j];
	}
}

template <int DL>
__device__ __forceinline__ void lfac_block(const double *__restrict__ m, double *F)
{
	double G[DL][DL], Gi[DL][DL];
#pragma unroll
	for(int j = 0; j < DL; ++ j)
#pragma unroll
		for(int i = 0; i < DL; ++ i) {
			G[i][j] = 0;
			if(i < j)
				continue;
			double sum = m[i + DL * j];
#pragma unroll
			for(int t = 0; t < DL; ++ t)
				if(t < j)
					sum -= G[i][t] * G[j][t];
			G[i][j] = (i == j) ? sqrt(sum) : sum / G[j][j];
		}
#pragma unroll
	for(int j = 0; j < DL; ++ j)
#pragma unroll
		for(int i = 0; i < DL; ++ i) {
			Gi[i][j] = 0;
			if(i < j)
				continue;
			if(i == j) {
				Gi[i][j] = 1.0 / G[j][j];
				continue;
			}
			double sum = 0;
#pragma unroll
			for(int t = 0; t < DL; ++ t)
				if(t >= j && t < i)
					sum += G[i][t] * Gi[t][j];
			Gi[i][j] = -sum / G[i][i];
		}
#pragma unroll
	for(int q = 0; q < DL; ++ q)
#pragma unroll
		for(int t = 0; t < DL; ++ t)
			F[t + DL * q] = Gi[q][t];
}

template <int DL>
__global__ __launch_bounds__(256)
void cinv_kernel(int64_t nl, const int64_t *__restrict__ lm_coff, const double *__restrict__ vals,
	double *__restrict__ cinv, double *__restrict__ lfac)
{
	const int64_t l = (int64_t)blockIdx.x * blockDim.x + threadIdx.x;
	if(l >= nl)
		return;
	const double *m = vals + lm_coff[l];
	double o[DL * DL];
	cinv_block<DL>(m, o);
#pragma unroll
	for(int e = 0; e < DL * DL; ++ e)
		cinv[l * DL * DL + e] = o[e];
	if(lfac) {
		double F[DL * DL];
		lfac_block<DL>(m, F);
#pragma unroll
		for(int e = 0; e < DL * DL; ++ e)
			lfac[l * DL * DL + e] = F[e];
	}
}

template <int DP, int DL>
__device__ __forceinline__ void load_U(const double *__restrict__ vals, int64_t oo, double *U)
{
	const double *src = vals + (oo >> 1);
	if(oo & 1) {
#pragma unroll
		for(int r = 0; r < DP; ++ r)
#pragma unroll
			for(int q = 0; q < DL; ++ q)
				U[r + DP * q] = src[q + DL * r];
	} else {
#pragma unroll
		for(int e = 0; e < DP * DL; ++ e)
			U[e] = src[e];
	}
}

template <int DP, int DL>
__global__ __launch_bounds__(256)
void obs_kernel(int64_t no, const int32_t *__restrict__ obs_lm, const int64_t *__restrict__ obs_off,
	const int64_t *__restrict__ lm_rbase, const double *__restrict__ vals, const double *__restrict__ rhs,
	const double *__restrict__ cinv, const int32_t *__restrict__ obs_wpos, double *__restrict__ W,
	double *__restrict__ Up, double *__restrict__ xw, int u_lm)
{
	constexpr int BLK = DP * DL, ST = BLK | 1;
	__shared__ double img_all[4][64 * ST];
	__shared__ int32_t slot_all[4][64];
	const int lane = threadIdx.x & 63, wave = threadIdx.x >> 6;
	double *img = img_all[wave];
	int32_t *slot = slot_all[wave];
	const int64_t a0 = ((int64_t)blockIdx.x * 4 + wave) * 64, a = a0 + lane;
	const bool active = a < no;
	const int nact = (no - a0 < 64) ? (int)((no - a0 > 0) ? (no - a0) : 0) : 64;
	const int64_t oo = active ? obs_off[a] : 0;
	const int32_t l = active ? obs_lm[a] : 0;
	slot[lane] = active ? obs_wpos[a] : 0;
	double U[BLK];
	if(active)
		load_U<DP, DL>(vals, oo, U);
	else {
#pragma unroll
		for(int e = 0; e < BLK; ++ e)
			U[e] = 0;
	}
	double Ci[DL * DL];
#pragma unroll
	for(int e = 0; e < DL * DL; ++ e)
		Ci[e] = cinv[(int64_t)l * DL * DL + e];
	double lv[DL];
#pragma unroll
	for(int q = 0; q < DL; ++ q)
		lv[q] = active ? rhs[lm_rbase[l] + q] : 0.0;
	double Wl[DP], Wv[BLK];
#pragma unroll
	for(int r = 0; r < DP; ++ r)
		Wl[r] = 0;
#pragma unroll
	for(int q = 0; q < DL; ++ q)
#pragma unroll
		for(int r = 0; r < DP; ++ r) {
			double sum = 0;
#pragma unroll
			for(int t = 0; t < DL; ++ t)
				sum += U[r + DP * t] * Ci[t + DL * q];
			Wv[r + DP * q] = sum;
			Wl[r] += sum * lv[q];
		}
#pragma unroll
	for(int e = 0; e < BLK; ++ e)
		img[lane * ST + e] = Wv[e];
	__syncthreads();
	for(int p = lane; p < nact * BLK; p += 64) {
		const int j = p / BLK, e = p - j * BLK;
		W[(int64_t)slot[j] * BLK + e] = img[j * ST + e];
	}
	__syncthreads();
#pragma unroll
	for(int e = 0; e < BLK; ++ e)
		img[lane * ST + e] = U[e];
	__syncthreads();
	for(int p = lane; p < nact * BLK; p += 64) {
		const int j = p / BLK, e = p - j * BLK;
		Up[(u_lm ? a0 + j : (int64_t)slot[j]) * BLK + e] = img[j * ST + e];
	}
	__syncthreads();
#pragma unroll
	for(int r = 0; r < DP; ++ r)
		img[lane * (DP | 1) + r] = Wl[r];
	__syncthreads();
	for(int p = lane; p < nact * DP; p += 64) {
		const int j = p / DP, r = p - j * DP;
		xw[(int64_t)slot[j] * DP + r] = img[j * (DP | 1) + r];
	}
}

template <int BLK> struct VSplit { static constexpr int IL = (BLK == 18) ? 16 : BLK, SIDE = BLK - IL; };

template <int DP, int DL>
__global__ __launch_bounds__(256)
void obs_fact_kernel(int64_t no, const int32_t *__restrict__ obs_lm, const int64_t *__restrict__ obs_off,
	const int64_t *__restrict__ lm_rbase, const double *__restrict__ vals, const double *__restrict__ rhs,
	const double *__restrict__ lfac, const int64_t *__restrict__ lm_coff, const int32_t *__restrict__ obs_wpos, double *__restrict__ Vm, double *__restrict__ Vs,
	double *__restrict__ xw)
{
	constexpr int BLK = DP * DL, ST = BLK | 1, IL = VSplit<BLK>::IL, SIDE = VSplit<BLK>::SIDE;
	__shared__ double img_all[4][64 * ST];
	__shared__ int32_t slot_all[4][64];
	const int lane = threadIdx.x & 63, wave = threadIdx.x >> 6;
	double *img = img_all[wave];
	int32_t *slot = slot_all[wave];
	const int64_t a0 = ((int64_t)blockIdx.x * 4 + wave) * 64, a = a0 + lane;
	const bool active = a < no;
	const int nact = (no - a0 < 64) ? (int)((no - a0 > 0) ? (no - a0) : 0) : 64;
	const int64_t oo = active ? obs_off[a] : 0;
	const int32_t l = active ? obs_lm[a] : 0;
	slot[lane] = active ? obs_wpos[a] : 0;
	double U[BLK];
	if(active)
		load_U<DP, DL>(vals, oo, U);
	else {
#pragma unroll
		for(int e = 0; e < BLK; ++ e)
			U[e] = 0;
	}
	double F[DL * DL], lv[DL], tv[DL];
	if(lfac) {
#pragma unroll
		for(int e = 0; e < DL * DL; ++ e)
			F[e] = lfac[(int64_t)l * DL * DL + e];
	} else
		lfac_block<DL>(vals + lm_coff[l], F);
#pragma unroll
	for(int q = 0; q < DL; ++ q)
		lv[q] = active ? rhs[lm_rbase[l] + q] : 0.0;
#pragma unroll
	for(int q = 0; q < DL; ++ q) {
		double sum = 0;
#pragma unroll
		for(int u = 0; u < DL; ++ u)
			if(u <= q)
				sum += F[u + DL * q] * lv[u];
		tv[q] = sum;
	}
	double V[BLK], Wl[DP];
#pragma unroll
	for(int r = 0; r < DP; ++ r)
		Wl[r] = 0;
#pragma unroll
	for(int q = 0; q < DL; ++ q)
#pragma unroll
		for(int r = 0; r < DP; ++ r) {
			double sum = 0;
#pragma unroll
			for(int t = 0; t < DL; ++ t)
				if(t <= q)
					sum += U[r + DP * t] * F[t + DL * q];
			V[r + DP * q] = sum;
			Wl[r] -= sum * tv[q];
		}
#pragma unroll
	for(int e = 0; e < BLK; ++ e)
		img[lane * ST + e] = V[e];
	__syncthreads();
	for(int p = lane; p < nact * IL; p += 64) {
		const int j = p / IL, e = p - j * IL;
		Vm[a0 * IL + p] = img[j * ST + e];
	}
	if(SIDE)
		for(int p = lane; p < nact * SIDE; p += 64) {
			const int j = p / (SIDE ? SIDE : 1), e = p - j * SIDE;
			Vs[a0 * SIDE + p] = img[j * ST + IL + e];
		}
	__syncthreads();
#pragma unroll
	for(int r = 0; r < DP; ++ r)
		img[lane * (DP | 1) + r] = Wl[r];
	__syncthreads();
	for(int p = lane; p < nact * DP; p += 64) {
		const int j = p / DP, r = p - j * DP;
		xw[(int64_t)slot[j] * DP + r] = img[j * (DP | 1) + r];
	}
}

constexpr int SACC_WAVES = 4;
#ifndef SPP_SACC_RP
#define SPP_SACC_RP 64
#endif
#ifndef SPP_SACC_UCOL
#define SPP_SACC_UCOL 0
#endif
#ifndef SPP_SACC_GLDS
#define SPP_SACC_GLDS 1
#endif

__device__ __forceinline__ SaccItem sacc_load_item(const SaccItem *__restrict__ items, int32_t idx, int32_t lim)
{
	SaccItem r;
	r.beg = r.end = 0;
	r.kind = -1;
	r.pad = 0;
	r.dst = 0;
	r.aoff = -1;
	if(idx < lim)
		r = items[idx];
	return r;
}

#ifndef SPP_SACC_EU
#define SPP_SACC_EU 2
#endif
template <int DP, int DL, bool FACT>
__global__ __launch_bounds__(SACC_WAVES * 64) __attribute__((amdgpu_waves_per_eu(SPP_SACC_EU, SPP_SACC_EU)))
void s_accum_kernel(const SaccItem *__restrict__ items, const int32_t *__restrict__ xcd_beg, int chunk,
	const int32_t *__restrict__ pair_a, const int32_t *__restrict__ pair_b,
	const double *__restrict__ W, const double *__restrict__ Up, const double *__restrict__ vals,
	double *__restrict__ S, int64_t ld, double *__restrict__ partial)
{
	constexpr int NE = DP * DP, BLK = DP * DL;
	constexpr int IL = VSplit<BLK>::IL, SIDE = VSplit<BLK>::SIDE;
	constexpr int PW = (BLK & 1) ? 1 : 2;
	constexpr int PCS = BLK / PW;
	constexpr int PPI = 64 / PCS;
	constexpr int RP = SPP_SACC_RP;
	constexpr int NG = (RP + PPI - 1) / PPI;
	constexpr bool GLDS = (PW == 2) && (SPP_SACC_GLDS != 0);
	constexpr int ST = GLDS ? BLK : (BLK | 1);
	constexpr int NE2 = (NE + 1) / 2;
	constexpr int RS = 2 * NE2 + 2;
	constexpr int NSEG = 64 / NE2 < 3 ? 64 / NE2 : 3;
	constexpr int LW = (2 * RP * ST > RP * RS) ? 2 * RP * ST : RP * RS;
	__shared__ __attribute__((aligned(16))) double lds[SACC_WAVES][LW];
	const int wave = __builtin_amdgcn_readfirstlane(threadIdx.x >> 6), lane = threadIdx.x & 63;
	const int x = blockIdx.x & 7;
	const int32_t lim = xcd_beg[x + 1];
	int32_t idx = xcd_beg[x] + (int32_t)(blockIdx.x >> 3) * SACC_WAVES * chunk + wave;
	if(idx >= lim)
		return;
	int left = chunk;
	double *sw = lds[wave], *su = sw + RP * ST, *rw = sw;
	const int my_pair = lane / PCS, my_piece = lane % PCS;
	SaccItem cur = sacc_load_item(items, idx, lim);
	SaccItem nxt = sacc_load_item(items, (left > 1) ? idx + SACC_WAVES : lim, lim);
	SaccItem nn = nxt;
	int32_t q0 = cur.beg;
	int32_t pa = -1, pb = -1;
	if(lane < RP && q0 + lane < cur.end) {
		pa = pair_a[q0 + lane];
		pb = pair_b[q0 + lane];
	}
	double acc[NE];
#pragma unroll
	for(int e = 0; e < NE; ++ e)
		acc[e] = 0;
	for(;;) {
		const int nround = (cur.end - q0 < RP) ? cur.end - q0 : RP;
		const bool mine = lane < nround;
		const bool last = q0 + RP >= cur.end;
		const int32_t nq0 = last ? nxt.beg : q0 + RP, nend = last ? nxt.end : cur.end;
		int32_t pa_n = -1, pb_n = -1;
		if(lane < RP && nq0 + lane < nend) {
			pa_n = pair_a[nq0 + lane];
			pb_n = pair_b[nq0 + lane];
		}
		double aval0 = 0, aval1 = 0;
		if(last) {
			nn = sacc_load_item(items, (left > 2) ? idx + 2 * SACC_WAVES : lim, lim);
			if(cur.aoff >= 0 && lane < NE2) {
				aval0 = vals[cur.aoff + 2 * lane];
				if(2 * lane + 1 < NE)
					aval1 = vals[cur.aoff + 2 * lane + 1];
			}
		}
		if constexpr(GLDS) {
			int32_t ia[NG], ib[NG];
#pragma unroll
			for(int g = 0; g < NG; ++ g) {
				const int p = g * PPI + my_pair;
				ia[g] = __shfl(pa, p & 63);
				ib[g] = __shfl(pb, p & 63);
			}
#pragma unroll
			for(int g = 0; g < NG; ++ g) {
				const int p = g * PPI + my_pair;
				if(my_pair < PPI && p < nround) {
					const double *srca, *srcb;
					if(FACT) {
						const bool side = SIDE && 2 * my_piece >= IL;
						srca = side ? Up + (int64_t)ia[g] * SIDE + (2 * my_piece - IL) : W + (int64_t)ia[g] * IL + 2 * my_piece;
						srcb = side ? Up + (int64_t)ib[g] * SIDE + (2 * my_piece - IL) : W + (int64_t)ib[g] * IL + 2 * my_piece;
					} else {
						srca = W + (int64_t)ia[g] * BLK + 2 * my_piece;
						srcb = Up + (int64_t)ib[g] * BLK + 2 * my_piece;
					}
					__builtin_amdgcn_global_load_lds((const __attribute__((address_space(1))) void*)srca,
						(__attribute__((address_space(3))) void*)(sw + g * PPI * BLK), 16, 0, 0);
					__builtin_amdgcn_global_load_lds((const __attribute__((address_space(1))) void*)srcb,
						(__attribute__((address_space(3))) void*)(su + g * PPI * BLK), 16, 0, 0);
				}
			}
			asm volatile("s_waitcnt vmcnt(0)" ::: "memory");
		} else {
		constexpr int GC = (NG < 10) ? NG : 10;
#pragma unroll
		for(int g0 = 0; g0 < NG; g0 += GC) {
			int32_t ia[GC], ib[GC];
#pragma unroll
			for(int gg = 0; gg < GC; ++ gg) {
				const int p = (g0 + gg) * PPI + my_pair;
				ia[gg] = __shfl(pa, p & 63);
				ib[gg] = __shfl(pb, p & 63);
			}
			double tw[GC][PW], tu[GC][PW];
#pragma unroll
			for(int gg = 0; gg < GC; ++ gg) {
				int32_t xa = ia[gg] < 0 ? 0 : ia[gg], xb = ib[gg] < 0 ? 0 : ib[gg];
				if(PW == 2) {
					const double2 a2 = *(const double2*)(W + (int64_t)xa * BLK + 2 * my_piece);
					const double2 b2 = *(const double2*)((FACT ? W : Up) + (int64_t)xb * BLK + 2 * my_piece);
					tw[gg][0] = a2.x; tw[gg][PW - 1] = a2.y;
					tu[gg][0] = b2.x; tu[gg][PW - 1] = b2.y;
				} else {
					tw[gg][0] = W[(int64_t)xa * BLK + my_piece];
					tu[gg][0] = (FACT ? W : Up)[(int64_t)xb * BLK + my_piece];
				}
			}
#pragma unroll
			for(int gg = 0; gg < GC; ++ gg) {
				const int g = g0 + gg;
				const int p = g * PPI + my_pair;
				if(g < NG && my_pair < PPI && p < RP) {
#pragma unroll
					for(int t = 0; t < PW; ++ t) {
						sw[p * ST + PW * my_piece + t] = tw[gg][t];
						su[p * ST + PW * my_piece + t] = tu[gg][t];
					}
				}
			}
		}
		}
		__builtin_amdgcn_fence(__ATOMIC_ACQ_REL, "wavefront");
		__builtin_amdgcn_wave_barrier();
		if(mine) {
#if SPP_SACC_UCOL
			double w[BLK];
#pragma unroll
			for(int e = 0; e < BLK; ++ e)
				w[e] = sw[lane * ST + e];
#pragma unroll
			for(int c = 0; c < DP; ++ c) {
				double uc[DL];
#pragma unroll
				for(int t = 0; t < DL; ++ t)
					uc[t] = su[lane * ST + c + DP * t];
#pragma unroll
				for(int r = 0; r < DP; ++ r) {
					double sp = 0;
#pragma unroll
					for(int t = 0; t < DL; ++ t)
						sp += w[r + DP * t] * uc[t];
					acc[r + DP * c] += sp;
				}
			}
#else
			double w[BLK], u[BLK];
#pragma unroll
			for(int e = 0; e < BLK; ++ e) {
				w[e] = sw[lane * ST + e];
				u[e] = su[lane * ST + e];
			}
#pragma unroll
			for(int c = 0; c < DP; ++ c)
#pragma unroll
				for(int r = 0; r < DP; ++ r) {
					double sp = 0;
#pragma unroll
					for(int t = 0; t < DL; ++ t)
						sp += w[r + DP * t] * u[c + DP * t];
					acc[r + DP * c] += FACT ? -sp : sp;
				}
#endif
		}
		__builtin_amdgcn_fence(__ATOMIC_ACQ_REL, "wavefront");
		__builtin_amdgcn_wave_barrier();
		if(last) {
			int nact = cur.end - cur.beg;
			if(nact > RP)
				nact = RP;
			if(lane < RP) {
#pragma unroll
				for(int e = 0; e < NE; ++ e)
					rw[lane * RS + e] = acc[e];
			}
			__builtin_amdgcn_fence(__ATOMIC_ACQ_REL, "wavefront");
			__builtin_amdgcn_wave_barrier();
			const int seg_len = (nact + NSEG - 1) / NSEG;
			const int e2 = lane % NE2, sq = lane / NE2;
			double s0 = 0, s1 = 0;
			if(sq < NSEG) {
				const double *src = rw + (sq * seg_len) * RS + 2 * e2;
				const int len = (seg_len < RP - sq * seg_len) ? seg_len : RP - sq * seg_len;
				int l = 0;
				for(; l + 8 <= len; l += 8) {
					double2 t[8];
#pragma unroll
					for(int u = 0; u < 8; ++ u)
						t[u] = *(const double2*)(src + (l + u) * RS);
#pragma unroll
					for(int u = 0; u < 8; ++ u) {
						s0 += t[u].x;
						s1 += t[u].y;
					}
				}
				for(; l < len; ++ l) {
					const double2 t = *(const double2*)(src + l * RS);
					s0 += t.x;
					s1 += t.y;
				}
			}
			__builtin_amdgcn_fence(__ATOMIC_ACQ_REL, "wavefront");
			__builtin_amdgcn_wave_barrier();
			{
				const double g0 = s0, g1 = s1;
#pragma unroll
				for(int q = 1; q < NSEG; ++ q) {
					s0 += __shfl(g0, (lane + q * NE2) & 63);
					s1 += __shfl(g1, (lane + q * NE2) & 63);
				}
			}
			if(lane < NE2) {
				const int e = 2 * lane;
				const bool two = e + 1 < NE;
				double *dst;
				int64_t o0 = e, o1 = e + 1;
				if(cur.kind == 2)
					dst = partial + cur.dst;
				else {
					dst = S + cur.dst;
					if(cur.aoff >= 0) {
						s0 = aval0 + s0;
						s1 = aval1 + s1;
					}
					if(cur.kind == 0) {
						o0 = e % DP + (e / DP) * ld;
						o1 = (e + 1) % DP + ((e + 1) / DP) * ld;
					}
				}
				dst[o0] = s0;
				if(two)
					dst[o1] = s1;
			}
#pragma unroll
			for(int e = 0; e < NE; ++ e)
				acc[e] = 0;
			idx += SACC_WAVES;
			-- left;
			cur = nxt;
			nxt = nn;
			if(left == 0 || cur.kind < 0)
				break;
		}
		q0 = nq0;
		pa = pa_n;
		pb = pb_n;
	}
}

template <int DP>
__global__ __launch_bounds__(256)
void s_multi_kernel(int64_t n_multi, const int32_t *__restrict__ multi_blk, const int32_t *__restrict__ multi_ptr,
	const int32_t *__restrict__ sblk_i1, const int32_t *__restrict__ sblk_i2, const int64_t *__restrict__ sblk_aoff,
	const double *__restrict__ partial, const double *__restrict__ vals, int add_A, double *__restrict__ S, int64_t ld,
	const int64_t *__restrict__ sblk_voff)
{
	const int64_t m = (int64_t)blockIdx.x * (blockDim.x >> 6) + (threadIdx.x >> 6);
	const int lane = threadIdx.x & 63;
	if(m >= n_multi || lane >= DP * DP)
		return;
	const int32_t b = multi_blk[m];
	double acc = 0;
	for(int32_t s = multi_ptr[m]; s < multi_ptr[m + 1]; ++ s)
		acc += partial[(int64_t)s * DP * DP + lane];
	const int64_t aoff = sblk_aoff[b];
	if(add_A && aoff >= 0)
		acc = vals[aoff + lane] + acc;
	if(sblk_voff) {
		S[sblk_voff[b] + lane] = acc;
		return;
	}
	const int r = lane % DP, c = lane / DP;
	S[((int64_t)sblk_i1[b] * DP + r) + ((int64_t)sblk_i2[b] * DP + c) * ld] = acc;
}

template <int DP>
__global__ __launch_bounds__(256)
void rhs_kernel(int64_t nc, const int32_t *__restrict__ cam_ptr, const int32_t *__restrict__ cam_obs,
	const int64_t *__restrict__ pose_rbase, const double *__restrict__ xw, const double *__restrict__ rhs,
	int add_eta, double *__restrict__ xcol)
{
	const int64_t i = (int64_t)blockIdx.x * (blockDim.x >> 6) + (threadIdx.x >> 6);
	const int lane = threadIdx.x & 63;
	if(i >= nc)
		return;
	double s[DP];
#pragma unroll
	for(int r = 0; r < DP; ++ r)
		s[r] = 0;
	for(int32_t q = cam_ptr[i] + lane; q < cam_ptr[i + 1]; q += 64) {
		const double *x = xw + (int64_t)q * DP;
#pragma unroll
		for(int r = 0; r < DP; ++ r)
			s[r] += x[r];
	}
#pragma unroll
	for(int r = 0; r < DP; ++ r) {
#pragma unroll
		for(int off = 32; off > 0; off >>= 1)
			s[r] += __shfl_xor(s[r], off);
	}
	if(lane < DP) {
		double v = 0;
#pragma unroll
		for(int r = 0; r < DP; ++ r)
			if(lane == r)
				v = s[r];
		if(add_eta)
			v += rhs[pose_rbase[i] + lane];
		xcol[i * DP + lane] = v;
	}
}

template <int DP, int DL>
__global__ __launch_bounds__(256)
void backsubst_obs_kernel(int64_t no, const int32_t *__restrict__ obs_pose, const int64_t *__restrict__ obs_off,
	const double *__restrict__ vals, const double *__restrict__ dx, double *__restrict__ tq)
{
	const int64_t a = (int64_t)blockIdx.x * blockDim.x + threadIdx.x;
	if(a >= no)
		return;
	double u[DP * DL];
	load_U<DP, DL>(vals, obs_off[a], u);
	double dv[DP];
	const double *d = dx + (int64_t)obs_pose[a] * DP;
#pragma unroll
	for(int r = 0; r < DP; ++ r)
		dv[r] = d[r];
#pragma unroll
	for(int q = 0; q < DL; ++ q) {
		double sum = 0;
#pragma unroll
		for(int r = 0; r < DP; ++ r)
			sum += dv[r] * u[r + DP * q];
		tq[a * DL + q] = sum;
	}
}

template <int DL>
__global__ __launch_bounds__(256)
void backsubst_lm_kernel(int64_t nl, const int32_t *__restrict__ lm_ptr, const int64_t *__restrict__ lm_rbase,
	const double *__restrict__ tq, const double *__restrict__ cinv, const int64_t *__restrict__ lm_coff, const double *__restrict__ vals,
	double *__restrict__ rhs)
{
	const int64_t l = (int64_t)blockIdx.x * blockDim.x + threadIdx.x;
	if(l >= nl)
		return;
	double t[DL];
	const int64_t rb = lm_rbase[l];
#pragma unroll
	for(int q = 0; q < DL; ++ q)
		t[q] = -rhs[rb + q];
	for(int32_t a = lm_ptr[l]; a < lm_ptr[l + 1]; ++ a) {
#pragma unroll
		for(int q = 0; q < DL; ++ q)
			t[q] += tq[(int64_t)a * DL + q];
	}
	double Ci[DL * DL];
	if(cinv) {
#pragma unroll
		for(int e = 0; e < DL * DL; ++ e)
			Ci[e] = cinv[l * DL * DL + e];
	} else
		cinv_block<DL>(vals + lm_coff[l], Ci);
#pragma unroll
	for(int q = 0; q < DL; ++ q) {
		double sum = 0;
#pragma unroll
		for(int u = 0; u < DL; ++ u)
			sum += Ci[q + DL * u] * t[u];
		rhs[rb + q] = sum;
	}
}

template <int DP, int DL>
__global__ __launch_bounds__(256)
void backsubst_fused_kernel(const int32_t *__restrict__ bs_ptr, const int32_t *__restrict__ lm_ptr, const int32_t *__restrict__ obs_pose,
	const int64_t *__restrict__ obs_off, const int64_t *__restrict__ lm_rbase, const double *__restrict__ cinv,
	const int64_t *__restrict__ lm_coff, const double *__restrict__ vals, const double *__restrict__ dx, double *__restrict__ rhs)
{
	__shared__ double tq[256 * DL];
	const int32_t l0 = bs_ptr[blockIdx.x], l1 = bs_ptr[blockIdx.x + 1];
	const int32_t a0 = lm_ptr[l0], na = lm_ptr[l1] - a0;
	const int t = threadIdx.x;
	if(t < na) {
		const int64_t a = (int64_t)a0 + t;
		double u[DP * DL];
		load_U<DP, DL>(vals, obs_off[a], u);
		double dv[DP];
		const double *d = dx + (int64_t)obs_pose[a] * DP;
#pragma unroll
		for(int r = 0; r < DP; ++ r)
			dv[r] = d[r];
#pragma unroll
		for(int q = 0; q < DL; ++ q) {
			double sum = 0;
#pragma unroll
			for(int r = 0; r < DP; ++ r)
				sum += dv[r] * u[r + DP * q];
			tq[t * DL + q] = sum;
		}
	}
	__syncthreads();
	if(t >= l1 - l0)
		return;
	const int64_t l = (int64_t)l0 + t;
	double tv[DL];
	const int64_t rb = lm_rbase[l];
#pragma unroll
	for(int q = 0; q < DL; ++ q)
		tv[q] = -rhs[rb + q];
	for(int32_t a = lm_ptr[l] - a0, e = lm_ptr[l + 1] - a0; a < e; ++ a) {
#pragma unroll
		for(int q = 0; q < DL; ++ q)
			tv[q] += tq[a * DL + q];
	}
	double Ci[DL * DL];
	if(cinv) {
#pragma unroll
		for(int e = 0; e < DL * DL; ++ e)
			Ci[e] = cinv[l * DL * DL + e];
	} else
		cinv_block<DL>(vals + lm_coff[l], Ci);
#pragma unroll
	for(int q = 0; q < DL; ++ q) {
		double sum = 0;
#pragma unroll
		for(int u = 0; u < DL; ++ u)
			sum += Ci[q + DL * u] * tv[u];
		rhs[rb + q] = sum;
	}
}

template <int DP>
__global__ __launch_bounds__(256)
void scatter_dx_kernel(int64_t nc, const int64_t *__restrict__ pose_rbase, const double *__restrict__ dx,
	double *__restrict__ rhs)
{
	const int64_t e = (int64_t)blockIdx.x * blockDim.x + threadIdx.x;
	if(e >= nc * DP)
		return;
	rhs[pose_rbase[e / DP] + e % DP] = dx[e];
}

template <int DP, int DL>
static void schur_form_t(spp_ctx *ctx, const double *d_vals, const double *d_rhs, double *S)
{
	SchurPlan &sp = ctx->schur;
	hipStream_t s = ctx->stream;
	const int64_t ld = sp.ld;
	const int64_t *voff = sp.sparse_S ? sp.sblk_voff.p : nullptr;
	double *xcol = sp.sparse_S ? S + sp.s_st.nvals : S + sp.n_red * ld;
	phase_begin(ctx, SPP_PHASE_SCHUR_INV);
	if(S == sp.S.p && !sp.sparse_S && ctx->shard_world == 1 && sp.n_sblk == sp.nc * (sp.nc + 1) / 2 && sp.n_red == sp.nc * DP)
		SPP_HIP_CHECK(hipMemsetAsync(S + sp.n_red * ld, 0, (size_t)(schur_buffer_doubles(ctx) - sp.n_red * ld) * sizeof(double), s));
	else
		SPP_HIP_CHECK(hipMemsetAsync(S, 0, (size_t)schur_buffer_doubles(ctx) * sizeof(double), s));
	constexpr int VIL = VSplit<DP * DL>::IL;
	double *Vm = sp.W.p, *Vs = sp.W.p + sp.no * VIL;
	const bool onfly = sp.factored && DL <= 3;
	if(sp.nl && !onfly)
		hipLaunchKernelGGL((cinv_kernel<DL>), dim3((unsigned)((sp.nl + 255) / 256)), dim3(256), 0, s,
			sp.nl, sp.lm_coff.p, d_vals, sp.cinv.p, sp.factored ? sp.lfac.p : nullptr);
	if(sp.no && sp.factored)
		hipLaunchKernelGGL((obs_fact_kernel<DP, DL>), dim3((unsigned)((sp.no + 255) / 256)), dim3(256), 0, s,
			sp.no, sp.obs_lm.p, sp.obs_off.p, sp.lm_rbase.p, d_vals, d_rhs, onfly ? (const double*)nullptr : (const double*)sp.lfac.p, sp.lm_coff.p,
			sp.obs_wpos.p, Vm, Vs, sp.xw.p);
	else if(sp.no)
		hipLaunchKernelGGL((obs_kernel<DP, DL>), dim3((unsigned)((sp.no + 255) / 256)), dim3(256), 0, s,
			sp.no, sp.obs_lm.p, sp.obs_off.p, sp.lm_rbase.p, d_vals, d_rhs, sp.cinv.p, sp.obs_wpos.p, sp.W.p, sp.Up.p, sp.xw.p, sp.u_landmark_major ? 1 : 0);
	phase_end(ctx, SPP_PHASE_SCHUR_INV);
	phase_begin(ctx, SPP_PHASE_SCHUR_GEMM);
	if(sp.n_items) {
		int chunk = switches().sacc_chunk;
		if(chunk <= 0)
			chunk = (int)((sp.xcd_max_items + SACC_WAVES * 64 - 1) / (SACC_WAVES * 64));
		const int64_t per = (int64_t)SACC_WAVES * chunk;
		if(sp.factored)
			hipLaunchKernelGGL((s_accum_kernel<DP, DL, true>), dim3((unsigned)(8 * ((sp.xcd_max_items + per - 1) / per))), dim3(SACC_WAVES * 64), 0, s,
				sp.items.p, sp.xcd_beg.p, chunk, sp.pair_a.p, sp.pair_b.p, Vm, Vs, d_vals, S, ld, sp.partial.p);
		else
			hipLaunchKernelGGL((s_accum_kernel<DP, DL, false>), dim3((unsigned)(8 * ((sp.xcd_max_items + per - 1) / per))), dim3(SACC_WAVES * 64), 0, s,
				sp.items.p, sp.xcd_beg.p, chunk, sp.pair_a.p, sp.pair_b.p, sp.W.p, sp.Up.p, d_vals, S, ld, sp.partial.p);
	}
	if(sp.n_multi)
		hipLaunchKernelGGL((s_multi_kernel<DP>), dim3((unsigned)((sp.n_multi + 3) / 4)), dim3(256), 0, s,
			sp.n_multi, sp.multi_blk.p, sp.multi_ptr.p, sp.sblk_i1.p, sp.sblk_i2.p, sp.sblk_aoff.p,
			sp.partial.p, d_vals, sp.add_A ? 1 : 0, S, ld, voff);
	phase_end(ctx, SPP_PHASE_SCHUR_GEMM);
	phase_begin(ctx, SPP_PHASE_SCHUR_RHS);
	if(sp.nc)
		hipLaunchKernelGGL((rhs_kernel<DP>), dim3((unsigned)((sp.nc + 3) / 4)), dim3(256), 0, s,
			sp.nc, sp.cam_ptr.p, sp.cam_obs.p, sp.pose_rbase.p, sp.xw.p, d_rhs, sp.add_A ? 1 : 0, xcol);
	phase_end(ctx, SPP_PHASE_SCHUR_RHS);
	SPP_HIP_CHECK(hipGetLastError());
}

template <int DP, int DL>
static int schur_finish_t(spp_ctx *ctx, const double *d_vals, double *S, double *d_rhs)
{
	SchurPlan &sp = ctx->schur;
	hipStream_t s = ctx->stream;
	const int64_t ld = sp.ld;
	double *xcol;
	if(sp.sparse_S) {
		xcol = S + sp.s_st.nvals;
		const int ret = sparse_factor_solve(ctx, S, xcol);
		if(ret != SPP_OK)
			return ret;
	} else {
		phase_begin(ctx, SPP_PHASE_FACTOR);
		dense_set_padding(ctx, S, ld, sp.n_red);
		{
			TileMaskGuard guard(ctx->dense, &sp.tile_mask);
			dense_potrf_upper_enqueue(ctx, S, sp.n_red, ld);
		}
		phase_end(ctx, SPP_PHASE_FACTOR);
		xcol = S + sp.n_red * ld;
		phase_begin(ctx, SPP_PHASE_TRISOLVE);
		dense_potrs_upper(ctx, S, sp.n_red, ld, xcol);
		phase_end(ctx, SPP_PHASE_TRISOLVE);
	}
	phase_begin(ctx, SPP_PHASE_BACKSUBST);
	static_assert(DL <= DP, "the products U^T dx reuse the W l buffer (DP doubles per observation)");
	const int bs_fused = switches().backsubst_fused;
	const double *cinv_arg = (sp.factored && DL <= 3) ? (const double*)nullptr : (const double*)sp.cinv.p;
	if(bs_fused && sp.n_bs > 0)
		hipLaunchKernelGGL((backsubst_fused_kernel<DP, DL>), dim3((unsigned)sp.n_bs), dim3(256), 0, s,
			sp.bs_ptr.p, sp.lm_ptr.p, sp.obs_pose.p, sp.obs_off.p, sp.lm_rbase.p, cinv_arg, sp.lm_coff.p, d_vals, xcol, d_rhs);
	else {
		if(sp.no)
			hipLaunchKernelGGL((backsubst_obs_kernel<DP, DL>), dim3((unsigned)((sp.no + 255) / 256)), dim3(256), 0, s,
				sp.no, sp.obs_pose.p, sp.obs_off.p, d_vals, xcol, sp.xw.p);
		if(sp.nl)
			hipLaunchKernelGGL((backsubst_lm_kernel<DL>), dim3((unsigned)((sp.nl + 255) / 256)), dim3(256), 0, s,
				sp.nl, sp.lm_ptr.p, sp.lm_rbase.p, sp.xw.p, cinv_arg, sp.lm_coff.p, d_vals, d_rhs);
	}
	if(sp.nc)
		hipLaunchKernelGGL((scatter_dx_kernel<DP>), dim3((unsigned)((sp.nc * DP + 255) / 256)), dim3(256), 0, s,
			sp.nc, sp.pose_rbase.p, xcol, d_rhs);
	phase_end(ctx, SPP_PHASE_BACKSUBST);
	SPP_HIP_CHECK(hipGetLastError());
	if(!sp.sparse_S && dense_info_fetch(ctx))
		return SPP_NOT_POSDEF;
	return SPP_OK;
}

template <bool PACK>
__global__ __launch_bounds__(256)
void schur_pack_kernel(double *__restrict__ S, int64_t ld, double *__restrict__ packed)
{
	const int64_t k = blockIdx.y;
	const int64_t rows = 128 * (k + 1);
	const int64_t e = (int64_t)blockIdx.x * 256 + threadIdx.x;
	if(e >= rows * 128)
		return;
	const int64_t r = e % rows, c = e / rows;
	double *ps = S + r + (128 * k + c) * ld;
	double *pp = packed + 128 * 128 * (k * (k + 1) / 2) + e;
	if(PACK)
		*pp = *ps;
	else
		*ps = *pp;
}

void schur_pack(spp_ctx *ctx, double *S, double *packed, bool pack)
{
	const int64_t ld = ctx->schur.ld, nblk = ld / 128;
	dim3 grid((unsigned)((ld * 128 + 255) / 256), (unsigned)nblk);
	if(pack)
// ... 28 lines not shown
```

slam_plus_plus_amd/csrc/spp_switches.h:

```cpp
#pragma once

#include <stdint.h>
#include <stdlib.h>
#include <string.h>
#include <algorithm>

namespace spp {

constexpr long long WAIT_TICKS_PER_MS = 100000;
constexpr long long WAIT_TICKS_DEFAULT = 500 * WAIT_TICKS_PER_MS;

enum Ordering { ORDERING_AUTO, ORDERING_AMD, ORDERING_ND };
constexpr int MID_FRONT_MAX = 640;

struct Switches {
	bool verbose;
	int plan_threads;
	int64_t plan_min_work;

	int dense_sched;
	int fused;
	int aux_reserve_cus;
	int tile_444;
	int dense_la;
	int la_chain_mask;
	int la_g2;
	int la_bulk_acquire;
	int64_t la_slots;
	int la_trace;
	int tail_rows;
	int tail_mask;
	double tail_order_beta;
	int tail_early;
	long long tail_timeout_ticks;
	int tail_trace;
	int trsv_chain;
	int trsv_mform;

	bool sacc_ulm;
	bool sacc_factored;
	int64_t sacc_tile;
	int64_t sacc_tile_cols;
	int sacc_xcd;
	int sacc_chunk;
	int backsubst_fused;

	int mid_front_max;
	Ordering ordering;
	int64_t amalg_small;
	double amalg_zeros;
	int64_t amalg_relax_h;
	double amalg_zeros_small;
	bool sparse_teams;
	int sparse_team_max;
	int sparse_team_cols;
	int sparse_dag;
	int dag_split;
	long long dag_timeout_ticks;
	int dag_trace;
};

inline int env_int(const char *name, int dflt)
{
	const char *e = getenv(name);
	return e ? atoi(e) : dflt;
}

inline long long env_i64(const char *name, long long dflt)
{
	const char *e = getenv(name);
	return e ? atoll(e) : dflt;
}

inline double env_double(const char *name, double dflt)
{
	const char *e = getenv(name);
	return e ? atof(e) : dflt;
}

inline Switches parse_switches()
{
	Switches w;
	w.verbose = getenv("SPP_VERBOSE") != nullptr;
	const char *threads = getenv("SPP_PLAN_THREADS");
	w.plan_threads = threads ? std::max(1, atoi(threads)) : 0;
	w.plan_min_work = std::max<int64_t>(1, env_i64("SPP_PLAN_MIN_WORK", int64_t(1) << 18));

	w.dense_sched = env_int("SPP_DENSE_SCHED", 1);
	w.fused = env_int("SPP_FUSED", 1);
	w.aux_reserve_cus = env_int("SPP_AUX_RESERVE_CUS", 32);
	w.tile_444 = env_int("SPP_TILE_444", 0);
	w.dense_la = env_int("SPP_DENSE_LA", 0);
	w.la_chain_mask = env_int("SPP_LA_CHAIN_MASK", 1);
	w.la_g2 = env_int("SPP_LA_G2", 0);
	w.la_bulk_acquire = env_int("SPP_LA_BULK_ACQUIRE", 1);
	w.la_slots = env_i64("SPP_LA_SLOTS", 0);
	w.la_trace = env_int("SPP_LA_TRACE", 0);
	w.tail_rows = env_int("SPP_DENSE_TAIL", 1) ? env_int("SPP_TAIL_ROWS", 44) : 0;
	w.tail_mask = env_int("SPP_TAIL_MASK", 1);
	w.tail_order_beta = env_double("SPP_TAIL_ORDER_BETA", 0.0);
	w.tail_early = env_int("SPP_TAIL_EARLY", 1);
	w.tail_timeout_ticks = env_i64("SPP_TAIL_TIMEOUT_TICKS", WAIT_TICKS_DEFAULT);
	w.tail_trace = env_int("SPP_TAIL_TRACE", 0);
	w.trsv_chain = env_int("SPP_TRSV_CHAIN", 2);
	w.trsv_mform = env_int("SPP_TRSV_MFORM", 1);

	w.sacc_ulm = env_int("SPP_SACC_ULM", 1) != 0;
	w.sacc_factored = env_int("SPP_SACC_FACTORED", 1) != 0;
	w.sacc_tile = std::max<int64_t>(1, env_i64("SPP_SACC_TILE", 4));
	w.sacc_tile_cols = env_i64("SPP_SACC_TILE_COLS", -2);
	w.sacc_xcd = env_int("SPP_SACC_XCD", 1);
	w.sacc_chunk = env_int("SPP_SACC_CHUNK", 1);
	w.backsubst_fused = env_int("SPP_BACKSUBST_FUSED", 1);

	w.mid_front_max = std::max(128, std::min(MID_FRONT_MAX, env_int("SPP_MID_FRONT_MAX", 320)));
	const char *ordering = getenv("SPP_ORDERING");
	w.ordering = !ordering ? ORDERING_AUTO : (!strcmp(ordering, "nd") ? ORDERING_ND : ORDERING_AMD);
	w.amalg_small = env_i64("SPP_AMALG_SMALL", 32);
	w.amalg_zeros = env_double("SPP_AMALG_ZEROS", 0.12);
	w.amalg_relax_h = env_i64("SPP_AMALG_RELAX_H", 96);
	w.amalg_zeros_small = env_double("SPP_AMALG_ZEROS_SMALL", 0.2);
	w.sparse_teams = env_int("SPP_SPARSE_TEAMS", 1) != 0;
	w.sparse_team_max = std::max(1, std::min(64, env_int("SPP_SPARSE_TEAM_MAX", 40)));
	w.sparse_team_cols = std::max(8, std::min(256, env_int("SPP_SPARSE_TEAM_COLS", 16)));
	w.sparse_dag = env_int("SPP_SPARSE_DAG", 1);
	w.dag_split = env_int("SPP_DAG_SPLIT", 1);
	w.dag_timeout_ticks = env_i64("SPP_DAG_TIMEOUT_TICKS", WAIT_TICKS_DEFAULT);
	w.dag_trace = env_int("SPP_DAG_TRACE", 0);
	return w;
}

inline const Switches &switches()
{
	static const Switches w = parse_switches();
	return w;
}

}
```

slam_plus_plus_amd/csrc/spp_symbolic.cpp:

```cpp

#include "spp_internal.h"
#include <sys/mman.h>
#include <stdlib.h>
#include <algorithm>
#include <numeric>
#include <string.h>
#include <stdlib.h>
#include <stdio.h>
#include <thread>
#include <memory>
#include <chrono>
#include <exception>

namespace spp {

void SchurPlan::release_all()
{
	lm_ptr.release(); bs_ptr.release(); n_bs = 0; lm_coff.release(); lm_rbase.release(); obs_pose.release(); obs_lm.release();
	obs_off.release(); pose_rbase.release(); cam_ptr.release(); cam_obs.release(); items.release();
	obs_wpos.release(); xcd_beg.release(); sblk_i1.release(); sblk_i2.release(); sblk_aoff.release();
	sblk_voff.release(); s_st = Structure(); sparse_S = false; mis = false;
	pair_a.release(); pair_b.release(); multi_blk.release(); multi_ptr.release(); cinv.release(); lfac.release();
	W.release(); Up.release(); xw.release(); partial.release(); S.release();
	pose_block.clear(); lm_block.clear(); is_lm.clear(); tile_mask.clear();
}

bool schur_applicable(const Structure &st, int *dp_out, int *dl_out)
{
	int d_a = -1, d_b = -1;
	for(int64_t j = 0; j < st.nb; ++ j) {
		int d = st.dim[j];
		if(d_a < 0 || d == d_a) d_a = d;
		else if(d_b < 0 || d == d_b) d_b = d;
		else return false;
	}
	if(d_a < 0 || d_b < 0)
		return false;
	int dp = std::max(d_a, d_b), dl = std::min(d_a, d_b);
	if(!((dp == 6 && dl == 3) || (dp == 3 && dl == 2)))
		return false;
	int64_t n_lm = 0;
	for(int64_t j = 0; j < st.nb; ++ j) {
		if(st.dim[j] == dl)
			++ n_lm;
		for(int64_t p = st.col_ptr[j]; p < st.col_ptr[j + 1]; ++ p) {
			int64_t i = st.row_idx[p];
			if(i != j && st.dim[i] == dl && st.dim[j] == dl)
				return false;
		}
	}
	if(n_lm == 0)
		return false;
	*dp_out = dp;
	*dl_out = dl;
	return true;
}

static const int PAIR_CHUNK = 2048;

int64_t schur_buffer_doubles(const spp_ctx *ctx)
{
	const SchurPlan &sp = ctx->schur;
	return sp.sparse_S ? sp.s_st.nvals + sp.n_red : sp.ld * sp.ld;
}

static bool mis_partition(const Structure &st, std::vector<uint8_t> &is_lm, int *d_out)
{
	const int d = st.dim[0];
	for(int64_t j = 0; j < st.nb; ++ j)
		if(st.dim[j] != d)
			return false;
	if(d != 3 && d != 6)
		return false;
	std::vector<std::vector<int32_t> > adj(st.nb);
	for(int64_t j = 0; j < st.nb; ++ j)
		for(int64_t p = st.col_ptr[j]; p < st.col_ptr[j + 1]; ++ p) {
			const int64_t i = st.row_idx[p];
			if(i != j) {
				adj[i].push_back((int32_t)j);
				adj[j].push_back((int32_t)i);
			}
		}
	std::vector<int32_t> order(st.nb);
	for(int64_t j = 0; j < st.nb; ++ j)
		order[j] = (int32_t)j;
	std::stable_sort(order.begin(), order.end(), [&](int32_t a, int32_t b) { return adj[a].size() < adj[b].size(); });
	is_lm.assign(st.nb, 0);
	std::vector<uint8_t> blocked(st.nb, 0);
	int64_t n_lm = 0;
	for(int64_t q = 0; q < st.nb; ++ q) {
		const int32_t v = order[q];
		if(blocked[v])
			continue;
		is_lm[v] = 1;
		++ n_lm;
		for(size_t e = 0; e < adj[v].size(); ++ e)
			blocked[adj[v][e]] = 1;
	}
	*d_out = d;
	return n_lm > 0 && n_lm < st.nb;
}

template <class T>
struct RawBuf {
	T *p = nullptr;
	size_t n = 0;
	RawBuf() {}
	RawBuf(const RawBuf&) = delete;
	RawBuf &operator=(const RawBuf&) = delete;
	~RawBuf() { free(p); }
	void resize(size_t m)
	{
		free(p);
		p = nullptr;
		if(m) {
			const size_t bytes = m * sizeof(T);
			if(bytes >= ((size_t)8 << 20)) {
				void *q = nullptr;
				if(posix_memalign(&q, (size_t)2 << 20, (bytes + (((size_t)2 << 20) - 1)) & ~(((size_t)2 << 20) - 1)) == 0) {
					p = (T*)q;
#ifdef MADV_HUGEPAGE
					madvise(q, bytes, MADV_HUGEPAGE);
#endif
				}
			}
			if(!p)
				p = (T*)malloc(bytes);
			if(!p)
				throw std::bad_alloc();
		}
		n = m;
	}
	size_t size() const { return n; }
	T &operator[](size_t i) { return p[i]; }
	const T &operator[](size_t i) const { return p[i]; }
};

void tile_mask_mark(int64_t n, int bs, int64_t nblk, const int32_t *i1, const int32_t *i2, std::vector<uint64_t> &words)
{
	words.clear();
	const int64_t Tr = (n + DENSE_NB - 1) / DENSE_NB, Tc = n / DENSE_NB + 1;
	if(Tr < 1 || Tc > 64)
		return;
	words.assign((size_t)Tr, 0);
	for(int64_t q = 0; q < nblk; ++ q) {
		const int64_t a = std::min(i1[q], i2[q]), b = std::max(i1[q], i2[q]);
		const int64_t r0 = a * bs / DENSE_NB, r1 = std::min<int64_t>(a * bs + bs - 1, n - 1) / DENSE_NB;
		const int64_t c0 = b * bs / DENSE_NB, c1 = std::min<int64_t>(b * bs + bs - 1, n - 1) / DENSE_NB;
		if(a < 0 || r0 >= Tr || c0 >= Tr)
			continue;
		words[r0] |= (1ull << c0) | (1ull << c1);
		words[r1] |= (1ull << c0) | (1ull << c1);
	}
}

int64_t tile_mask_close(int64_t n, bool has_rhs, bool fill, std::vector<uint64_t> &words)
{
	const int64_t Tr = (n + DENSE_NB - 1) / DENSE_NB, Tc = has_rhs ? n / DENSE_NB + 1 : Tr;
	if(Tr < 1 || Tc > 64 || (int64_t)words.size() != Tr) {
		words.clear();
		return -1;
	}
	const uint64_t cols = Tc == 64 ? ~0ull : (1ull << Tc) - 1;
	for(int64_t i = 0; i < Tr; ++ i) {
		words[i] |= 1ull << i;
		if(has_rhs)
			words[i] |= 1ull << (n / DENSE_NB);
		words[i] &= cols & ~((1ull << i) - 1);
	}
	int64_t updates = 0;
	for(int64_t k = 0; k < Tr; ++ k) {
		const uint64_t r = words[k] & ~((2ull << k) - 1);
		for(uint64_t m = r; m; m &= m - 1) {
			const int a = __builtin_ctzll(m);
			if(a >= Tr)
				break;
			const uint64_t f = r & ~((1ull << a) - 1);
			if(fill)
				words[a] |= f;
			updates += __builtin_popcountll(words[a] & f);
		}
	}
	return updates;
}

void tail_order_table(const std::vector<uint64_t> &bits, int Tr, int Tc, bool have_pre, double beta, int resident, bool early,
	std::vector<int> &order, int *info)
{
	std::vector<std::pair<double, int> > key;
	for(int i = 0; i < Tr; ++ i)
		for(int j = i; j < Tc; ++ j)
			if((bits[(size_t)i + 1] >> j) & 1)
				key.push_back(std::make_pair((double)i + beta * (double)j, (i << 16) | j));
	std::stable_sort(key.begin(), key.end(), [](const std::pair<double, int> &x, const std::pair<double, int> &y) { return x.first < y.first; });
	order.resize(key.size());
	for(size_t q = 0; q < key.size(); ++ q)
		order[q] = key[q].second;
	int widest = 1;
	for(int i = 0; i < Tr; ++ i)
		widest = std::max(widest, (int)__builtin_popcountll(bits[(size_t)i + 1]));
	const int D = std::max(resident, 0) / widest;
	if(info) {
		info[0] = 0;
		info[1] = Tr;
		info[2] = D;
		info[3] = 0;
		info[4] = widest;
	}
	if(!early || resident <= 0)
		return;
	auto first_step = [&](const int i, const int j) -> int {
		for(int k = have_pre ? -1 : 0; k < i; ++ k) {
			const uint64_t w = bits[(size_t)k + 1];
			if((w >> i) & (w >> j) & 1)
				return k;
		}
		return i;
	};
	int r_star = Tr;
	for(int i = Tr - 1; i >= 0; -- i) {
		bool all_lag = true;
		for(int j = i; j < Tc && all_lag; ++ j)
			if((bits[(size_t)i + 1] >> j) & 1)
				all_lag = i - first_step(i, j) > D;
		if(!all_lag)
			break;
		r_star = i;
	}
	int n_early = 0;
	std::vector<int> live((size_t)Tr + 1, 0);
	for(size_t q = 0; q < order.size(); ++ q) {
		const int i = order[q] >> 16, j = order[q] & 0xffff;
		if(i >= r_star)
			++ n_early;
		else {
			++ live[(size_t)std::max(first_step(i, j), 0)];
			-- live[(size_t)i + 1];
		}
	}
	int demand = 0;
	for(int r = 0, run = 0; r < Tr; ++ r) {
		run += live[(size_t)r];
		demand = std::max(demand, run);
	}
	if(info)
		info[3] = demand;
	if(n_early == 0 || n_early > resident / 2 || resident - n_early < demand)
		return;
	std::stable_partition(order.begin(), order.end(), [r_star](const int t) { return (t >> 16) >= r_star; });
	if(info) {
		info[0] = n_early;
		info[1] = r_star;
	}
}

static void schur_tile_mask(const Structure &st, const std::vector<uint8_t> &is_lm, const std::vector<int32_t> &pose_of,
	int dp, int64_t n_red, std::vector<uint64_t> &words)
{
	tile_mask_mark(n_red, dp, 0, nullptr, nullptr, words);
	if(words.empty())
		return;
	const int64_t Tr = (int64_t)words.size();
	auto tiles_of = [&](int32_t pose) -> uint64_t {
		return (1ull << ((int64_t)pose * dp / DENSE_NB)) | (1ull << (((int64_t)pose * dp + dp - 1) / DENSE_NB));
	};
	auto mark = [&](uint64_t rows, const uint64_t cols) {
		for(; rows; rows &= rows - 1) {
			const int a = __builtin_ctzll(rows);
			if(a < Tr)
				words[a] |= cols;
		}
	};
	std::vector<uint64_t> seen(st.nb, 0);
	for(int64_t j = 0; j < st.nb; ++ j)
		for(int64_t p = st.col_ptr[j]; p < st.col_ptr[j + 1]; ++ p) {
			const int64_t i = st.row_idx[p];
			if(!is_lm[i] && !is_lm[j])
				mark(tiles_of(pose_of[i]), tiles_of(pose_of[j]));
			else if(!is_lm[i])
				seen[j] |= tiles_of(pose_of[i]);
			else if(!is_lm[j])
				seen[i] |= tiles_of(pose_of[j]);
		}
	for(int64_t j = 0; j < st.nb; ++ j)
		if(seen[j])
			mark(seen[j], seen[j]);
	tile_mask_close(n_red, true, true, words);
}

struct SchurPlanHost {
	int dp = 0, dl = 0;
	int64_t nc = 0, nl = 0, nl_total = 0, no = 0, n_red = 0, ld = 0, n_sblk = 0, n_pairs = 0, n_items = 0, n_multi = 0, n_ablk = 0;
	int32_t n_slots = 0, xcd_max_items = 0;
	bool u_landmark_major = true, factored = true;
	std::vector<int64_t> pose_block, lm_block;
	std::vector<uint8_t> is_lm;
	HVec<int32_t> lm_ptr, obs_pose, obs_lm, cam_obs, wpos;
	std::vector<int32_t> bs_ptr;
	std::vector<int32_t> cam_ptr, sblk_i1, sblk_i2, multi_blk, multi_ptr, xb;
	RawBuf<int32_t> pair_a, pair_b;
	HVec<int64_t> lm_coff, obs_off, lm_rbase;
	std::vector<int64_t> sblk_aoff, sblk_voff, pose_rbase;
	std::vector<SaccItem> recs;
	Structure s_st;
	std::vector<uint64_t> tile_mask;
};

static void schur_plan_host(const Structure &st, int shard_rank, int shard_world, bool sparse_S, bool mis, SchurPlanHost &h)
{
	VClock clk("schur plan");
	int dp, dl;
	std::vector<uint8_t> &is_lm = h.is_lm;
	if(mis) {
		SPP_REQUIRE(mis_partition(st, is_lm, &dp), SPP_E_UNSUPPORTED,
			"MIS Schur mode needs a graph of one block width (3 or 6) with at least one edge");
		dl = dp;
	} else {
		SPP_REQUIRE(schur_applicable(st, &dp, &dl), SPP_E_UNSUPPORTED,
			"Schur mode needs exactly two block widths ({6,3} or {3,2}) and a block-diagonal landmark part");
		is_lm.assign(st.nb, 0);
		for(int64_t j = 0; j < st.nb; ++ j)
			is_lm[j] = st.dim[j] == dl;
	}
	h.dp = dp;
	h.dl = dl;

	std::vector<int32_t> pose_of(st.nb, -1), lm_of(st.nb, -1);
	int64_t nc = 0, nl_total = 0, nl = 0;
	for(int64_t j = 0; j < st.nb; ++ j) {
		if(!is_lm[j]) {
			pose_of[j] = (int32_t)nc ++;
			h.pose_block.push_back(j);
		} else {
			if(nl_total % shard_world == shard_rank) {
				lm_of[j] = (int32_t)nl ++;
				h.lm_block.push_back(j);
			}
			++ nl_total;
		}
	}
	h.nc = nc;
	h.nl = nl;
	h.nl_total = nl_total;
	const bool add_A = (shard_rank == 0);
	h.n_red = nc * dp;
	h.ld = ((h.n_red + 1 + DENSE_NB - 1) / DENSE_NB) * DENSE_NB;
	SPP_REQUIRE(sparse_S || h.ld <= 65536, SPP_E_UNSUPPORTED,
		"reduced camera system too large for the dense path (use SPP_MODE_SCHUR_SPARSE)");
	if(!sparse_S)
		schur_tile_mask(st, is_lm, pose_of, dp, h.n_red, h.tile_mask);

	struct Obs { int32_t lm, pose; int64_t off; };
	HVec<int64_t> &lm_coff = h.lm_coff;
	lm_coff.assign(nl, -1);
	struct ABlk { int32_t i1, i2; int64_t off; };
	std::vector<ABlk> ablk;
	HVec<int32_t> &lm_ptr = h.lm_ptr, &obs_pose = h.obs_pose, &obs_lm = h.obs_lm;
	HVec<int64_t> &obs_off = h.obs_off;
	bool obs_sorted = true;
	const int nts = plan_threads(st.nnzb);
	std::vector<int64_t> jcut;
	balanced_cuts(st.col_ptr, nts, jcut);
	{
		std::vector<int64_t> n_obs_t(nts + 1, 0), n_ab_t(nts + 1, 0);
		auto classify = [&](int64_t j, int64_t p, Obs &o) -> int {
			const int64_t i = st.row_idx[p];
			const bool pi = !is_lm[i], pj = !is_lm[j];
			if(pi && pj)
				return 0;
			if(!pi && !pj)
				return 1;
			if(pi) {
				if(lm_of[j] < 0)
					return 3;
				o = {lm_of[j], pose_of[i], st.blk_off[p] << 1};
			} else {
				if(lm_of[i] < 0)
					return 3;
				o = {lm_of[i], pose_of[j], (st.blk_off[p] << 1) | 1};
			}
			return 2;
		};
		run_threads(nts, [&](int t) {
			int64_t n_o = 0, n_a = 0;
			Obs o;
			for(int64_t j = jcut[t]; j < jcut[t + 1]; ++ j)
				for(int64_t p = st.col_ptr[j]; p < st.col_ptr[j + 1]; ++ p) {
					const int k = classify(j, p, o);
					n_o += k == 2;
					n_a += k == 0;
				}
			n_obs_t[t + 1] = n_o;
			n_ab_t[t + 1] = n_a;
		});
		for(int t = 0; t < nts; ++ t) {
			n_obs_t[t + 1] += n_obs_t[t];
			n_ab_t[t + 1] += n_ab_t[t];
		}
		const int64_t no_all = n_obs_t[nts];
		SPP_REQUIRE(no_all < (int64_t(1) << 31), SPP_E_UNSUPPORTED, "too many observations for 32-bit obs indices");
		obs_pose.resize(no_all);
		obs_lm.resize(no_all);
		obs_off.resize(no_all);
		ablk.resize(n_ab_t[nts]);
		std::vector<char> sorted_t(nts, 1);
		run_threads(nts, [&](int t) {
			int64_t a = n_obs_t[t], q = n_ab_t[t];
			Obs o, prev = {-1, -1, 0};
			bool sorted = true;
			for(int64_t j = jcut[t]; j < jcut[t + 1]; ++ j)
				for(int64_t p = st.col_ptr[j]; p < st.col_ptr[j + 1]; ++ p) {
					const int k = classify(j, p, o);
					if(k == 0)
						ablk[q ++] = {pose_of[st.row_idx[p]], pose_of[j], st.blk_off[p]};
					else if(k == 1) {
						if(lm_of[j] >= 0)
							lm_coff[lm_of[j]] = st.blk_off[p];
					} else if(k == 2) {
						if(o.lm < prev.lm || (o.lm == prev.lm && o.pose < prev.pose))
							sorted = false;
						prev = o;
						obs_lm[a] = o.lm;
						obs_pose[a] = o.pose;
						obs_off[a] = o.off;
						++ a;
					}
				}
			sorted_t[t] = sorted;
		});
		for(int t = 0; t < nts; ++ t)
			obs_sorted = obs_sorted && sorted_t[t];
		for(int t = 1; t < nts && obs_sorted; ++ t) {
			const int64_t a = n_obs_t[t];
			if(a > 0 && a < no_all && (obs_lm[a] < obs_lm[a - 1] || (obs_lm[a] == obs_lm[a - 1] && obs_pose[a] < obs_pose[a - 1])))
				obs_sorted = false;
		}
	}
	h.n_ablk = (int64_t)ablk.size();
	clk.lap("partition + observation scan");
	for(int64_t l = 0; l < nl; ++ l)
		SPP_REQUIRE(lm_coff[l] >= 0, SPP_E_BADARG, "landmark without a diagonal block");
	std::vector<std::vector<int32_t> > foreign_cols;
	if(sparse_S && shard_world > 1) {
		std::vector<int64_t> lm_gidx(st.nb, -1);
		int64_t g = 0;
		for(int64_t j = 0; j < st.nb; ++ j)
			if(is_lm[j])
				lm_gidx[j] = g ++;
		std::vector<std::vector<int32_t> > poses_of(g);
		for(int64_t j = 0; j < st.nb; ++ j)
			for(int64_t p = st.col_ptr[j]; p < st.col_ptr[j + 1]; ++ p) {
				const int64_t i = st.row_idx[p];
				const bool pi = !is_lm[i], pj = !is_lm[j];
				if(pi && !pj && lm_of[j] < 0)
					poses_of[lm_gidx[j]].push_back(pose_of[i]);
				else if(!pi && pj && lm_of[i] < 0)
					poses_of[lm_gidx[i]].push_back(pose_of[j]);
			}
		foreign_cols.resize(nc);
		for(int64_t l = 0; l < g; ++ l) {
			std::vector<int32_t> &ps = poses_of[l];
			std::sort(ps.begin(), ps.end());
			for(size_t a = 0; a < ps.size(); ++ a)
				for(size_t b = a + 1; b < ps.size(); ++ b)
					foreign_cols[ps[a]].push_back(ps[b]);
		}
		for(int64_t c = 0; c < nc; ++ c) {
			std::sort(foreign_cols[c].begin(), foreign_cols[c].end());
			foreign_cols[c].erase(std::unique(foreign_cols[c].begin(), foreign_cols[c].end()), foreign_cols[c].end());
		}
	}
	const int64_t no = (int64_t)obs_pose.size();
	h.no = no;
	if(!obs_sorted) {
		std::vector<Obs> obs(no);
		for(int64_t a = 0; a < no; ++ a)
			obs[a] = {obs_lm[a], obs_pose[a], obs_off[a]};
		std::sort(obs.begin(), obs.end(), [](const Obs &a, const Obs &b) {
			return a.lm != b.lm ? a.lm < b.lm : a.pose < b.pose; });
		for(int64_t a = 0; a < no; ++ a) {
			obs_lm[a] = obs[a].lm;
			obs_pose[a] = obs[a].pose;
			obs_off[a] = obs[a].off;
		}
	}
	lm_ptr.resize(nl + 1);
	const int nto = plan_threads(no);
	run_threads(nto, [&](int t) {
		const int64_t a0 = no * t / nto, a1 = no * (t + 1) / nto;
		for(int64_t a = a0; a < a1; ++ a) {
			const int32_t lp = a ? obs_lm[a - 1] : -1, lc = obs_lm[a];
			for(int32_t l = lp + 1; l <= lc; ++ l)
				lm_ptr[l] = (int32_t)a;
		}
	});
	for(int64_t l = (no ? obs_lm[no - 1] : -1) + 1; l <= nl; ++ l)
		lm_ptr[l] = (int32_t)no;

	{
		const int32_t BS_OBS = 256;
		std::vector<int32_t> &bp = h.bs_ptr;
		bp.clear();
		bp.reserve((size_t)(no / 160 + 2));
		bp.push_back(0);
		int32_t first = 0;
		bool ok = true;
		for(int64_t l = 0; l < nl; ++ l) {
			if(lm_ptr[l + 1] - lm_ptr[l] > BS_OBS) {
				ok = false;
				break;
			}
			if(lm_ptr[l + 1] - lm_ptr[first] > BS_OBS || l - first >= BS_OBS) {
				bp.push_back((int32_t)l);
				first = (int32_t)l;
			}
		}
		if(ok && nl)
			bp.push_back((int32_t)nl);
		else
			bp.clear();
	}

	std::vector<int32_t> &cam_ptr = h.cam_ptr;
	HVec<int32_t> &cam_obs = h.cam_obs;
	cam_ptr.assign(nc + 1, 0);
	cam_obs.resize(no);
	HVec<int32_t> cam_end(no);
	{
		std::vector<int32_t> cnt((size_t)nto * nc, 0);
		run_threads(nto, [&](int t) {
			int32_t *c = cnt.data() + (size_t)t * nc;
			for(int64_t a = no * t / nto, a1 = no * (t + 1) / nto; a < a1; ++ a)
				++ c[obs_pose[a]];
		});
		for(int64_t c = 0; c < nc; ++ c) {
			int32_t sum = cam_ptr[c];
			for(int t = 0; t < nto; ++ t) {
				const int32_t v = cnt[(size_t)t * nc + c];
				cnt[(size_t)t * nc + c] = sum;
				sum += v;
			}
			cam_ptr[c + 1] = sum;
		}
		run_threads(nto, [&](int t) {
			int32_t *fill = cnt.data() + (size_t)t * nc;
			for(int64_t a = no * t / nto, a1 = no * (t + 1) / nto; a < a1; ++ a) {
				const int32_t pos = fill[obs_pose[a]] ++;
				cam_obs[pos] = (int32_t)a;
				cam_end[pos] = lm_ptr[obs_lm[a] + 1];
			}
		});
	}

	HVec<int32_t> &wpos = h.wpos;
	wpos.resize(no);
	run_threads(nto, [&](int t) {
		for(int64_t q = no * t / nto, q1 = no * (t + 1) / nto; q < q1; ++ q)
			wpos[cam_obs[q]] = (int32_t)q;
	});

	clk.lap("observation / camera lists");
	std::vector<int64_t> lm_pairs(nl + 1, 0);
	for(int64_t l = 0; l < nl; ++ l) {
		const int64_t k = lm_ptr[l + 1] - lm_ptr[l];
		lm_pairs[l + 1] = lm_pairs[l] + k * (k + 1) / 2;
	}
	const int64_t n_pairs = lm_pairs[nl];
	SPP_REQUIRE(n_pairs < (int64_t(1) << 31), SPP_E_UNSUPPORTED, "too many block products for 32-bit pair indices");
	h.n_pairs = n_pairs;
	h.u_landmark_major = switches().sacc_ulm;
	h.factored = switches().sacc_factored;
	RawBuf<int32_t> &pair_a = h.pair_a, &pair_b = h.pair_b;
	pair_a.resize(n_pairs);
	pair_b.resize(n_pairs);
	{
		const int ntt = plan_threads(n_pairs);
		run_threads(ntt, [&](int t) {
			const int64_t b = n_pairs * t / ntt, e = n_pairs * (t + 1) / ntt;
			memset(pair_a.p + b, 0, (size_t)(e - b) * sizeof(int32_t));
			memset(pair_b.p + b, 0, (size_t)(e - b) * sizeof(int32_t));
		});
	}
	clk.lap("pair list buffers");
	std::vector<int32_t> &sblk_i1 = h.sblk_i1, &sblk_i2 = h.sblk_i2;
	std::vector<int64_t> &sblk_aoff = h.sblk_aoff;
	std::vector<int64_t> sblk_beg;
	const int nt = plan_threads(n_pairs);
	const bool ulm = h.u_landmark_major, fact = h.factored;
	std::vector<std::vector<std::pair<int32_t, int64_t> > > a_by_row(nc);
	for(size_t q = 0; q < ablk.size(); ++ q)
		a_by_row[ablk[q].i1].push_back(std::make_pair(ablk[q].i2, ablk[q].off));
	{
		std::vector<int64_t> row_cnt(nc + 1, 0);
		{
			std::vector<int64_t> ccut;
			balanced_cuts(std::vector<int64_t>(cam_ptr.begin(), cam_ptr.end()), nt, ccut);
			run_threads(nt, [&](int t) {
				for(int64_t c = ccut[t]; c < ccut[t + 1]; ++ c) {
					int64_t sum = 0;
					for(int32_t q = cam_ptr[c]; q < cam_ptr[c + 1]; ++ q)
						sum += cam_end[q] - cam_obs[q];
					row_cnt[c + 1] = sum;
				}
			});
			for(int64_t c = 0; c < nc; ++ c)
				row_cnt[c + 1] += row_cnt[c];
		}
		clk.lap("pair counts");
		std::vector<int64_t> rcut;
		{
			std::vector<int64_t> w(nc + 1, 0);
			for(int64_t c = 0; c < nc; ++ c)
				w[c + 1] = w[c] + (row_cnt[c + 1] - row_cnt[c]) + (nc - c);
			balanced_cuts(w, nt, rcut);
		}
		struct RowOut { std::vector<int32_t> i1, i2; std::vector<int64_t> aoff, beg; };
		std::vector<RowOut> rout(nt);
		run_threads(nt, [&](int t) {
			RowOut &ro = rout[t];
			std::vector<int64_t> col_cnt(nc + 1), a_of_col(nc), start(nc + 1, 0);
			std::vector<char> foreign(nc, 0);
			for(int64_t i1 = rcut[t]; i1 < rcut[t + 1]; ++ i1) {
				const int64_t b0 = row_cnt[i1], b1 = row_cnt[i1 + 1];
				std::fill(col_cnt.begin() + i1, col_cnt.end(), 0);
				std::fill(a_of_col.begin() + i1, a_of_col.end(), -1);
				const int32_t qa0 = cam_ptr[i1], qa1 = cam_ptr[i1 + 1];
				constexpr int32_t AHEAD = 24;
				for(int32_t q = qa0; q < qa1; ++ q) {
					if(q + AHEAD < (int32_t)no)
						__builtin_prefetch(&obs_pose[cam_obs[q + AHEAD]]);
					const int32_t a = cam_obs[q], e = cam_end[q];
					for(int32_t b = a; b < e; ++ b)
						++ col_cnt[obs_pose[b] + 1];
				}
				for(size_t q = 0; q < a_by_row[i1].size(); ++ q)
					a_of_col[a_by_row[i1][q].first] = a_by_row[i1][q].second;
				if(!foreign_cols.empty())
					for(size_t q = 0; q < foreign_cols[i1].size(); ++ q)
						foreign[foreign_cols[i1][q]] = 1;
				int64_t out = b0;
				for(int64_t c = i1; c < nc; ++ c) {
					start[c] = out;
					if(col_cnt[c + 1] || a_of_col[c] >= 0 || foreign[c]) {
						ro.i1.push_back((int32_t)i1);
						ro.i2.push_back((int32_t)c);
						ro.aoff.push_back(a_of_col[c]);
						ro.beg.push_back(out);
					}
					out += col_cnt[c + 1];
				}
				if(!foreign_cols.empty())
					for(size_t q = 0; q < foreign_cols[i1].size(); ++ q)
						foreign[foreign_cols[i1][q]] = 0;
				for(int32_t q = qa0; q < qa1; ++ q) {
					if(q + AHEAD < (int32_t)no)
						__builtin_prefetch(&obs_pose[cam_obs[q + AHEAD]]);
					const int32_t a = cam_obs[q], e = cam_end[q];
					const int32_t wa = fact ? a : q;
					for(int32_t b = a; b < e; ++ b) {
						int64_t &f = start[obs_pose[b]];
						pair_a[f] = wa;
						pair_b[f] = (ulm || fact) ? b : wpos[b];
						++ f;
					}
				}
				(void)b1;
			}
		});
		clk.lap("pair lists by row");
		size_t nblk = 0;
		for(int t = 0; t < nt; ++ t)
			nblk += rout[t].i1.size();
		sblk_i1.reserve(nblk);
		sblk_i2.reserve(nblk);
		sblk_aoff.reserve(nblk);
		sblk_beg.reserve(nblk + 1);
		for(int t = 0; t < nt; ++ t) {
			sblk_i1.insert(sblk_i1.end(), rout[t].i1.begin(), rout[t].i1.end());
			sblk_i2.insert(sblk_i2.end(), rout[t].i2.begin(), rout[t].i2.end());
			sblk_aoff.insert(sblk_aoff.end(), rout[t].aoff.begin(), rout[t].aoff.end());
			sblk_beg.insert(sblk_beg.end(), rout[t].beg.begin(), rout[t].beg.end());
		}
		sblk_beg.push_back(n_pairs);
	}
	const int64_t n_sblk = (int64_t)sblk_i1.size();
	h.n_sblk = n_sblk;

	if(sparse_S) {
		Structure &ss = h.s_st;
		ss.nb = nc;
		ss.nnzb = n_sblk;
		ss.dim.assign(nc, dp);
		ss.base.resize(nc + 1);
		for(int64_t c = 0; c <= nc; ++ c)
			ss.base[c] = c * dp;
		ss.n = nc * dp;
		ss.col_ptr.assign(nc + 1, 0);
		for(int64_t b = 0; b < n_sblk; ++ b)
			++ ss.col_ptr[sblk_i2[b] + 1];
		for(int64_t c = 0; c < nc; ++ c)
			ss.col_ptr[c + 1] += ss.col_ptr[c];
		ss.row_idx.resize(n_sblk);
		ss.blk_off.resize(n_sblk);
		std::vector<int64_t> fill(ss.col_ptr.begin(), ss.col_ptr.end() - 1);
		h.sblk_voff.resize(n_sblk);
		for(int64_t b = 0; b < n_sblk; ++ b) {
			const int64_t q = fill[sblk_i2[b]] ++;
			ss.row_idx[q] = sblk_i1[b];
			ss.blk_off[q] = q * dp * dp;
			h.sblk_voff[b] = q * dp * dp;
		}
		ss.nvals = n_sblk * dp * dp;
		for(int64_t c = 0; c < nc; ++ c)
			SPP_REQUIRE(ss.col_ptr[c + 1] > ss.col_ptr[c] && ss.row_idx[ss.col_ptr[c + 1] - 1] == c, SPP_E_BADARG,
				"a pose without any diagonal contribution: the reduced system is singular");
	}

	clk.lap("block lists");
	std::vector<int32_t> item_blk, item_beg, item_end, item_slot;
	std::vector<int32_t> &multi_blk = h.multi_blk, &multi_ptr = h.multi_ptr;
	int32_t n_slots = 0;
	for(int64_t b = 0; b < n_sblk; ++ b) {
		const int64_t beg = sblk_beg[b], end = sblk_beg[b + 1];
		const int64_t nchunk = std::max<int64_t>(1, (end - beg + PAIR_CHUNK - 1) / PAIR_CHUNK);
		if(nchunk > 1) {
			multi_blk.push_back((int32_t)b);
			multi_ptr.push_back(n_slots);
		}
		for(int64_t c = 0; c < nchunk; ++ c) {
			item_blk.push_back((int32_t)b);
			item_beg.push_back((int32_t)(beg + c * PAIR_CHUNK));
			item_end.push_back((int32_t)std::min<int64_t>(end, beg + (c + 1) * PAIR_CHUNK));
			item_slot.push_back(nchunk > 1 ? n_slots ++ : -1);
		}
	}
	multi_ptr.push_back(n_slots);
	h.n_slots = n_slots;
	bool interleave = false;
	std::vector<int32_t> xb_il;
	{
		const int64_t tb_env = switches().sacc_tile, tbc_env = switches().sacc_tile_cols;
		const int64_t TB = tb_env, TBC = (tbc_env == -2) ? TB : (tbc_env <= 0 ? nc : tbc_env), ntile = (nc + TBC - 1) / TBC;
		std::vector<int32_t> perm(item_blk.size());
		for(size_t q = 0; q < perm.size(); ++ q)
			perm[q] = (int32_t)q;
		interleave = switches().sacc_xcd != 0;
		std::vector<int64_t> tile_of_item(item_blk.size());
		for(size_t q = 0; q < tile_of_item.size(); ++ q)
			tile_of_item[q] = (sblk_i1[item_blk[q]] / TB) * ntile + sblk_i2[item_blk[q]] / TBC;
		auto tile_of = [&](int32_t q) { return tile_of_item[q]; };
		auto stable_by_key = [&](std::vector<int32_t> &pm, int64_t n_keys, auto key_of) {
			if(n_keys > 8 * (int64_t)pm.size() + 1024) {
				std::stable_sort(pm.begin(), pm.end(), [&](int32_t x, int32_t y) { return key_of(x) < key_of(y); });
				return;
			}
			std::vector<int32_t> start((size_t)n_keys + 1, 0), out(pm.size());
			for(size_t q = 0; q < pm.size(); ++ q)
				++ start[key_of(pm[q]) + 1];
			for(int64_t k = 0; k < n_keys; ++ k)
				start[k + 1] += start[k];
			for(size_t q = 0; q < pm.size(); ++ q)
				out[start[key_of(pm[q])] ++] = pm[q];
			pm.swap(out);
		};
		stable_by_key(perm, ((nc + TB - 1) / TB) * ntile, tile_of);
		if(interleave) {
			std::vector<int32_t> xcd_of(perm.size());
			int64_t load[8] = {0, 0, 0, 0, 0, 0, 0, 0};
			for(size_t q = 0; q < perm.size();) {
				const int64_t t = tile_of(perm[q]);
				size_t e = q;
				int64_t cost = 0;
				for(; e < perm.size() && tile_of(perm[e]) == t; ++ e)
					cost += 2 + (item_end[perm[e]] - item_beg[perm[e]] + 63) / 64;
				int x = 0;
				for(int y = 1; y < 8; ++ y)
					if(load[y] < load[x])
						x = y;
				load[x] += cost;
				for(size_t i = q; i < e; ++ i)
					xcd_of[perm[i]] = x;
				q = e;
			}
			stable_by_key(perm, 8, [&](int32_t x) { return (int64_t)xcd_of[x]; });
			xb_il.assign(9, 0);
			for(size_t q = 0; q < perm.size(); ++ q)
				++ xb_il[xcd_of[q] + 1];
			for(int x = 0; x < 8; ++ x)
				xb_il[x + 1] += xb_il[x];
		}
		std::vector<int32_t> t_blk(perm.size()), t_beg(perm.size()), t_end(perm.size()), t_slot(perm.size());
		for(size_t q = 0; q < perm.size(); ++ q) {
			t_blk[q] = item_blk[perm[q]];
			t_beg[q] = item_beg[perm[q]];
			t_end[q] = item_end[perm[q]];
			t_slot[q] = item_slot[perm[q]];
		}
		item_blk.swap(t_blk); item_beg.swap(t_beg); item_end.swap(t_end); item_slot.swap(t_slot);
	}
	h.n_items = (int64_t)item_blk.size();
	{
		std::vector<int32_t> &xb = h.xb;
		xb.assign(9, 0);
		if(interleave)
			xb = xb_il;
		else {
			std::vector<int64_t> cost(h.n_items + 1, 0);
			for(int64_t q = 0; q < h.n_items; ++ q)
				cost[q + 1] = cost[q] + 2 + (item_end[q] - item_beg[q] + 63) / 64;
			for(int x = 1; x < 8; ++ x)
				xb[x] = (int32_t)(std::lower_bound(cost.begin(), cost.end(), cost[h.n_items] * x / 8) - cost.begin());
			xb[8] = (int32_t)h.n_items;
		}
		h.xcd_max_items = 0;
		for(int x = 0; x < 8; ++ x) {
			xb[x + 1] = std::max(xb[x + 1], xb[x]);
			h.xcd_max_items = std::max(h.xcd_max_items, xb[x + 1] - xb[x]);
		}
	}
	h.n_multi = (int64_t)multi_blk.size();

	h.pose_rbase.resize(nc);
	h.lm_rbase.resize(nl);
	for(int64_t c = 0; c < nc; ++ c)
		h.pose_rbase[c] = st.base[h.pose_block[c]];
	for(int64_t l = 0; l < nl; ++ l)
		h.lm_rbase[l] = st.base[h.lm_block[l]];

	clk.lap("work items");
	h.recs.resize(item_blk.size());
	for(size_t q = 0; q < h.recs.size(); ++ q) {
		const int32_t b = item_blk[q];
		SaccItem &r = h.recs[q];
		r.beg = item_beg[q];
		r.end = item_end[q];
		r.pad = 0;
		r.aoff = -1;
		if(item_slot[q] >= 0) {
			r.kind = 2;
			r.dst = (int64_t)item_slot[q] * dp * dp;
		} else {
			r.aoff = add_A ? sblk_aoff[b] : -1;
			if(sparse_S) {
				r.kind = 1;
				r.dst = h.sblk_voff[b];
			} else {
				r.kind = 0;
				r.dst = (int64_t)sblk_i1[b] * dp + (int64_t)sblk_i2[b] * dp * h.ld;
			}
		}
	}
	clk.lap("item records");
}

void build_schur_plan(spp_ctx *ctx, bool sparse_S, bool mis)
{
	const Structure &st = ctx->st;
	SchurPlan &sp = ctx->schur;
	sp.release_all();
	sp.sparse_S = sparse_S;
	hipStream_t s = ctx->stream;
	VClock clk0("schur plan (device)");
	std::unique_ptr<SchurPlanHost> hp(new SchurPlanHost);
	SchurPlanHost &h = *hp;
	clk0.lap("old plan released");
	schur_plan_host(st, ctx->shard_rank, ctx->shard_world, sparse_S, mis, h);
	VClock clk("schur plan (device)");
	const int dp = h.dp, dl = h.dl;
	const int64_t nc = h.nc, nl = h.nl, no = h.no;
	sp.dp = dp;
	sp.dl = dl;
	sp.pose_block.swap(h.pose_block);
	sp.lm_block.swap(h.lm_block);
	sp.is_lm.swap(h.is_lm);
	sp.nc = nc;
	sp.nl = nl;
	sp.nl_total = h.nl_total;
	sp.add_A = (ctx->shard_rank == 0);
	sp.n_red = h.n_red;
	sp.ld = h.ld;
	sp.tile_mask.swap(h.tile_mask);
	sp.no = no;
	sp.n_pairs = h.n_pairs;
	sp.n_sblk = h.n_sblk;
	sp.u_landmark_major = h.u_landmark_major;
	sp.factored = h.factored;
	sp.n_items = h.n_items;
	sp.n_multi = h.n_multi;
	sp.xcd_max_items = h.xcd_max_items;
	if(sparse_S) {
		sp.s_st = h.s_st;
		sp.sblk_voff.upload(h.sblk_voff, s);
	}

	sp.xcd_beg.upload(h.xb, s);
	sp.lm_ptr.upload(h.lm_ptr, s);
	sp.n_bs = h.bs_ptr.empty() ? 0 : (int64_t)h.bs_ptr.size() - 1;
	sp.bs_ptr.upload(h.bs_ptr, s);
	sp.lm_coff.upload(h.lm_coff, s);
	sp.lm_rbase.upload(h.lm_rbase, s);
	sp.obs_pose.upload(h.obs_pose, s);
	sp.obs_lm.upload(h.obs_lm, s);
	sp.obs_off.upload(h.obs_off, s);
	sp.pose_rbase.upload(h.pose_rbase, s);
	sp.cam_ptr.upload(h.cam_ptr, s);
	sp.cam_obs.upload(h.cam_obs, s);
	sp.items.upload(h.recs, s);
	sp.obs_wpos.upload(h.wpos, s);
	sp.sblk_i1.upload(h.sblk_i1, s);
	sp.sblk_i2.upload(h.sblk_i2, s);
	sp.sblk_aoff.upload(h.sblk_aoff, s);
	sp.pair_a.reserve(std::max<size_t>(1, h.pair_a.size()));
	sp.pair_b.reserve(std::max<size_t>(1, h.pair_b.size()));
	if(h.pair_a.size()) {
		SPP_HIP_CHECK(hipMemcpyAsync(sp.pair_a.p, h.pair_a.p, h.pair_a.size() * sizeof(int32_t), hipMemcpyHostToDevice, s));
		SPP_HIP_CHECK(hipMemcpyAsync(sp.pair_b.p, h.pair_b.p, h.pair_b.size() * sizeof(int32_t), hipMemcpyHostToDevice, s));
	}
	sp.multi_blk.upload(h.multi_blk, s);
	sp.multi_ptr.upload(h.multi_ptr, s);
	clk.lap("uploads enqueued");
	sp.cinv.reserve((size_t)std::max<int64_t>(1, nl) * dl * dl);
	sp.W.reserve((size_t)std::max<int64_t>(1, no) * dp * dl);
	if(sp.factored)
		sp.lfac.reserve((size_t)std::max<int64_t>(1, nl) * dl * dl);
	else
		sp.Up.reserve((size_t)std::max<int64_t>(1, no) * dp * dl);
	sp.xw.reserve((size_t)std::max<int64_t>(1, no) * dp);
	sp.partial.reserve((size_t)std::max<int32_t>(1, h.n_slots) * dp * dp);
	clk.lap("workspaces allocated");
	SPP_HIP_CHECK(hipStreamSynchronize(s));
	clk.lap("uploads done");

	if(!sparse_S)
		dense_reserve(ctx, (sp.n_red + DENSE_NB - 1) / DENSE_NB);
	clk.lap("dense workspaces");

	const double n = (double)sp.n_red;
	ctx->factor_flops = (int64_t)(n * n * n / 3.0 + 2.0 * n * n);
	ctx->factor_nnz = sp.ld * sp.ld;
	const int64_t blk_pl = 8 * dp * dl, blk_pp = 8 * dp * dp, blk_ll = 8 * dl * dl;
	ctx->solve_bytes = blk_pl * no + blk_ll * nl + blk_pp * h.n_ablk + 8 * st.n
		+ blk_pp * sp.n_sblk + 8 * st.n
		+ 8 * sp.n_red * sp.n_red ;
	if(ctx->plan_trash.joinable())
		ctx->plan_trash.join();
	{
		SchurPlanHost *raw = hp.release();
		try {
			ctx->plan_trash = std::thread([raw]() { delete raw; });
		} catch(...) {
			delete raw;
		}
	}
	clk.lap("host plan handed to the releasing thread");
}

double schur_plan_host_probe(const Structure &st, int shard_rank, int shard_world, bool sparse_S, bool mis, int64_t *out)
{
	const auto t0 = std::chrono::steady_clock::now();
	SchurPlanHost h;
	schur_plan_host(st, shard_rank, shard_world, sparse_S || mis, mis, h);
	const double sec = std::chrono::duration<double>(std::chrono::steady_clock::now() - t0).count();
	uint64_t sum = 1469598103934665603ull;
	auto mix = [&](uint64_t v) { sum = (sum ^ v) * 1099511628211ull; };
	for(size_t q = 0; q < h.pair_a.size(); ++ q)
		mix(((uint64_t)(uint32_t)h.pair_a[q] << 32) | (uint32_t)h.pair_b[q]);
	for(size_t q = 0; q < h.sblk_i1.size(); ++ q) {
		mix(((uint64_t)(uint32_t)h.sblk_i1[q] << 32) | (uint32_t)h.sblk_i2[q]);
		mix((uint64_t)h.sblk_aoff[q]);
	}
	for(size_t q = 0; q < h.recs.size(); ++ q) {
		mix(((uint64_t)(uint32_t)h.recs[q].beg << 32) | (uint32_t)h.recs[q].end);
		mix((uint64_t)h.recs[q].dst);
		mix((uint64_t)h.recs[q].aoff + (uint64_t)h.recs[q].kind);
	}
	for(size_t q = 0; q < h.xb.size(); ++ q)
		mix((uint64_t)h.xb[q]);
	out[0] = h.nc; out[1] = h.nl; out[2] = h.no; out[3] = h.n_pairs; out[4] = h.n_sblk; out[5] = h.n_items; out[6] = h.n_multi;
	out[7] = (int64_t)sum;
	return sec;
}

void schur_tile_mask_host_probe(const Structure &st, int shard_rank, int shard_world, std::vector<uint64_t> &words)
{
	SchurPlanHost h;
	schur_plan_host(st, shard_rank, shard_world, false, false, h);
	words.swap(h.tile_mask);
}

void min_degree_order(int64_t nb, const int64_t *col_ptr, const int64_t *row_idx, std::vector<int64_t> &order)
{
	order.clear();
	order.reserve(nb);
	if(nb == 0)
		return;
	std::vector<std::vector<int32_t> > adj(nb), elems(nb);
	for(int64_t j = 0; j < nb; ++ j)
		for(int64_t p = col_ptr[j]; p < col_ptr[j + 1]; ++ p) {
			int64_t i = row_idx[p];
			if(i != j) {
				adj[i].push_back((int32_t)j);
				adj[j].push_back((int32_t)i);
			}
		}
	for(int64_t i = 0; i < nb; ++ i) {
		std::sort(adj[i].begin(), adj[i].end());
		adj[i].erase(std::unique(adj[i].begin(), adj[i].end()), adj[i].end());
	}
	std::vector<std::vector<int32_t> > elem_vars(nb);
	std::vector<uint8_t> state(nb, 0);
	std::vector<int64_t> degree(nb);
	std::vector<int64_t> w(nb, -1);
	std::vector<int64_t> mark(nb, -1);
	std::vector<int32_t> head(nb + 1, -1), next(nb, -1), prev(nb, -1);
	auto bucket_insert = [&](int32_t v) {
		int64_t d = std::min<int64_t>(degree[v], nb);
		next[v] = head[d];
		prev[v] = -1;
		if(head[d] >= 0) prev[head[d]] = v;
		head[d] = v;
	};
	auto bucket_remove = [&](int32_t v) {
		int64_t d = std::min<int64_t>(degree[v], nb);
		if(prev[v] >= 0) next[prev[v]] = next[v]; else head[d] = next[v];
		if(next[v] >= 0) prev[next[v]] = prev[v];
	};
	for(int64_t i = 0; i < nb; ++ i) {
		degree[i] = (int64_t)adj[i].size();
		bucket_insert((int32_t)i);
	}
	int64_t mindeg = 0;
	std::vector<int32_t> Lp;
	for(int64_t step = 0; step < nb; ++ step) {
		while(mindeg <= nb && head[mindeg] < 0)
			++ mindeg;
		const int32_t p = head[mindeg];
		bucket_remove(p);
		order.push_back(p);
		Lp.clear();
		mark[p] = step;
		for(size_t q = 0; q < adj[p].size(); ++ q) {
			int32_t v = adj[p][q];
			if(state[v] == 0 && mark[v] != step) {
				mark[v] = step;
				Lp.push_back(v);
			}
		}
		for(size_t q = 0; q < elems[p].size(); ++ q) {
			int32_t e = elems[p][q];
			if(state[e] != 1)
				continue;
			for(size_t t = 0; t < elem_vars[e].size(); ++ t) {
				int32_t v = elem_vars[e][t];
				if(state[v] == 0 && mark[v] != step) {
					mark[v] = step;
					Lp.push_back(v);
				}
			}
			state[e] = 2;
			std::vector<int32_t>().swap(elem_vars[e]);
		}
		state[p] = 1;
		std::vector<int32_t>().swap(adj[p]);
		std::vector<int32_t>().swap(elems[p]);
		elem_vars[p] = Lp;
		const int64_t lp = (int64_t)Lp.size();
		for(size_t q = 0; q < Lp.size(); ++ q) {
			int32_t v = Lp[q];
			for(size_t t = 0; t < elems[v].size(); ++ t) {
				int32_t e = elems[v][t];
				if(state[e] != 1)
					continue;
				if(w[e] < step * (nb + 1)) {
					int64_t sz = 0;
					for(size_t u = 0; u < elem_vars[e].size(); ++ u)
						if(state[elem_vars[e][u]] == 0)
							++ sz;
					w[e] = step * (nb + 1) + sz;
				}
				-- w[e];
			}
		}
		for(size_t q = 0; q < Lp.size(); ++ q) {
			const int32_t v = Lp[q];
			bucket_remove(v);
			{
				std::vector<int32_t> &a = adj[v];
				size_t o = 0;
				for(size_t t = 0; t < a.size(); ++ t)
					if(state[a[t]] == 0 && mark[a[t]] != step)
						a[o ++] = a[t];
				a.resize(o);
			}
			int64_t d = (int64_t)adj[v].size() + (lp - 1);
			{
				std::vector<int32_t> &el = elems[v];
				size_t o = 0;
				for(size_t t = 0; t < el.size(); ++ t) {
					int32_t e = el[t];
					if(state[e] != 1)
						continue;
					int64_t we = w[e] - step * (nb + 1);
					if(we <= 0) {
						continue;
					}
					d += we;
					el[o ++] = e;
				}
				el.resize(o);
				el.push_back(p);
			}
			degree[v] = std::min<int64_t>(std::min<int64_t>(d, nb - step - 1), degree[v] + lp - 1);
			if(degree[v] < 0) degree[v] = 0;
			bucket_insert(v);
			if(degree[v] < mindeg)
				mindeg = degree[v];
		}
	}
}


static const int ND_LEAF = 48;

void nested_dissection_order(int64_t nb, const int64_t *col_ptr, const int64_t *row_idx, std::vector<int64_t> &order)
{
	order.assign(nb, -1);
	if(nb == 0)
		return;
	std::vector<std::vector<int32_t> > adj(nb);
	for(int64_t j = 0; j < nb; ++ j)
		for(int64_t p = col_ptr[j]; p < col_ptr[j + 1]; ++ p) {
			const int64_t i = row_idx[p];
			if(i != j) {
				adj[i].push_back((int32_t)j);
				adj[j].push_back((int32_t)i);
			}
		}
	std::vector<int32_t> part(nb, 0), level(nb, -1), local(nb, -1);
	struct Task { std::vector<int32_t> verts; int64_t lo; };
	std::vector<Task> stack;
	{
		Task t;
		t.verts.resize(nb);
		for(int64_t v = 0; v < nb; ++ v)
			t.verts[v] = (int32_t)v;
		t.lo = 0;
		stack.push_back(std::move(t));
	}
	int32_t next_part = 1;
	std::vector<int32_t> queue;
	auto bfs = [&](int32_t root, int32_t pid, std::vector<int32_t> &out) {
		out.clear();
		out.push_back(root);
		level[root] = 0;
		for(size_t h = 0; h < out.size(); ++ h) {
			const int32_t v = out[h];
			for(size_t q = 0; q < adj[v].size(); ++ q) {
				const int32_t u = adj[v][q];
				if(part[u] == pid && level[u] < 0) {
					level[u] = level[v] + 1;
					out.push_back(u);
				}
			}
		}
	};
	while(!stack.empty()) {
		Task t = std::move(stack.back());
		stack.pop_back();
		const int64_t m = (int64_t)t.verts.size();
		if(m == 0)
			continue;
		const int32_t pid = part[t.verts[0]];
		if(m <= ND_LEAF) {
			for(int64_t q = 0; q < m; ++ q)
				local[t.verts[q]] = (int32_t)q;
			std::vector<int64_t> cp(m + 1, 0), ri;
			for(int64_t q = 0; q < m; ++ q) {
				const int32_t v = t.verts[q];
				for(size_t e = 0; e < adj[v].size(); ++ e) {
					const int32_t u = adj[v][e];
					if(part[u] == pid && local[u] < q)
						ri.push_back(local[u]);
				}
				std::sort(ri.begin() + cp[q], ri.end());
				ri.erase(std::unique(ri.begin() + cp[q], ri.end()), ri.end());
				ri.push_back(q);
				cp[q + 1] = (int64_t)ri.size();
			}
			std::vector<int64_t> lo;
			min_degree_order(m, cp.data(), ri.data(), lo);
			for(int64_t q = 0; q < m; ++ q)
				order[t.lo + q] = t.verts[lo[q]];
			for(int64_t q = 0; q < m; ++ q) {
				local[t.verts[q]] = -1;
				part[t.verts[q]] = -1;
			}
			continue;
		}
		bfs(t.verts[0], pid, queue);
		if((int64_t)queue.size() < m) {
			const int32_t pa = next_part ++;
			Task a, b;
			for(size_t q = 0; q < queue.size(); ++ q)
				part[queue[q]] = pa;
			for(int64_t q = 0; q < m; ++ q) {
				const int32_t v = t.verts[q];
				level[v] = -1;
				(part[v] == pa ? a : b).verts.push_back(v);
			}
			a.lo = t.lo;
			b.lo = t.lo + (int64_t)a.verts.size();
			stack.push_back(std::move(a));
			stack.push_back(std::move(b));
			continue;
		}
		int32_t far = queue.back();
		for(size_t q = 0; q < queue.size(); ++ q)
			level[queue[q]] = -1;
		bfs(far, pid, queue);
		const int32_t nlev = level[queue.back()] + 1;
		if(nlev < 3) {
			for(int64_t q = 0; q < m; ++ q) {
				local[t.verts[q]] = (int32_t)q;
				level[t.verts[q]] = -1;
			}
			std::vector<int64_t> cp(m + 1, 0), ri;
			for(int64_t q = 0; q < m; ++ q) {
				const int32_t v = t.verts[q];
				for(size_t e = 0; e < adj[v].size(); ++ e) {
					const int32_t u = adj[v][e];
					if(part[u] == pid && local[u] < q)
						ri.push_back(local[u]);
				}
				std::sort(ri.begin() + cp[q], ri.end());
				ri.erase(std::unique(ri.begin() + cp[q], ri.end()), ri.end());
				ri.push_back(q);
				cp[q + 1] = (int64_t)ri.size();
			}
			std::vector<int64_t> lo;
			min_degree_order(m, cp.data(), ri.data(), lo);
			for(int64_t q = 0; q < m; ++ q)
				order[t.lo + q] = t.verts[lo[q]];
			for(int64_t q = 0; q < m; ++ q) {
				local[t.verts[q]] = -1;
				part[t.verts[q]] = -1;
			}
			continue;
		}
		std::vector<int64_t> lsize(nlev, 0);
		for(size_t q = 0; q < queue.size(); ++ q)
			++ lsize[level[queue[q]]];
		int32_t best = -1;
		{
			int64_t below = 0;
			double best_cost = 0;
			for(int32_t l = 0; l < nlev; ++ l) {
				const int64_t above = m - below - lsize[l];
				if(l > 0 && l + 1 < nlev) {
					const double bal = (double)std::min(below, above) / (double)std::max<int64_t>(1, std::max(below, above));
					const double cost = (double)lsize[l] * (1.0 + 2.0 * (1.0 - bal) * (1.0 - bal) * 4.0);
					if(bal >= 0.25 && (best < 0 || cost < best_cost)) {
						best = l;
						best_cost = cost;
					}
				}
				below += lsize[l];
			}
			if(best < 0)
				best = nlev / 2;
		}
		const int32_t pa = next_part ++, pb = next_part ++;
		Task a, b;
		std::vector<int32_t> sep;
		for(size_t q = 0; q < queue.size(); ++ q) {
			const int32_t v = queue[q];
			if(level[v] < best)
				a.verts.push_back(v);
			else if(level[v] > best)
				b.verts.push_back(v);
			else {
				bool touches = false;
				for(size_t e = 0; e < adj[v].size() && !touches; ++ e) {
					const int32_t u = adj[v][e];
					touches = part[u] == pid && level[u] == best + 1;
				}
				if(touches)
					sep.push_back(v);
				else
					a.verts.push_back(v);
			}
// ... 21 lines not shown
```

Baseline: 1.193 billion block-nnz/s.

## Reorder cameras in dense Schur complement by co-visibility dissection to cut tile fill

Builds a camera co-visibility graph and searches for a contiguous arc separator that splits cameras into two independent groups. The resulting order is scored with a tile-DAG cost model of the dense Schur Cholesky, and it is adopted only if the modelled cost drops by at least 10% and the live-tile check passes. Because reordering can flip pose-pose A blocks below the diagonal, those blocks are read transposed through a new a_tr flag in the accumulate kernels. It also adds a cheaper per-landmark sort of observations when they are already grouped by landmark. The cost is extra host planning time, plus the risk of mistakes in the transposed-index handling.

```diff
diff --git a/include/spp_hip.h b/include/spp_hip.h
--- a/include/spp_hip.h
+++ b/include/spp_hip.h
@@ -147,6 +147,8 @@
 	uint64_t *words, int64_t *n_updates);
 int spp_schur_tile_mask_host(int64_t nb, const int32_t *dim, const int64_t *col_ptr, const int64_t *row_idx, int shard_rank,
 	int shard_world, uint64_t *words);
+int spp_schur_cam_order_host(int64_t nb, const int32_t *dim, const int64_t *col_ptr, const int64_t *row_idx, int shard_rank,
+	int shard_world, int flags, const int64_t *order_in, int64_t *cam_order, double *figures);
 int spp_tail_order_host(int64_t n, int has_rhs, const uint64_t *words, int64_t nwords, int resident, int early, double beta,
 	int32_t *table, int32_t *info);
 int spp_dense_gemm_tn_sub(spp_ctx *ctx, int64_t m, int64_t n, int64_t k,
diff --git a/slam_plus_plus_amd/api.py b/slam_plus_plus_amd/api.py
--- a/slam_plus_plus_amd/api.py
+++ b/slam_plus_plus_amd/api.py
@@ -22,7 +22,7 @@
     "spp_device_free", "spp_memcpy_h2d", "spp_memcpy_d2h", "spp_memcpy_d2d", "spp_get_phase_ms", "spp_get_dominant_kernel",
     "spp_microbench_copy", "spp_microbench_mfma_f64", "spp_microbench_ctile", "spp_microbench_update", "spp_block_ordering", "spp_schur_plan_host", "spp_set_profiling", "spp_se2_linearize_device", "spp_se2_update_device", "spp_ba_linearize_device", "spp_ba_update_device", "spp_se3_linearize_device", "spp_se3_update_device", "spp_edge_chi2_device", "spp_edge_robust_weights_device", "spp_edge_hessian_maxdiag_device",
     "spp_lm_gain_denominator_device", "spp_dense_potrf_upper", "spp_dense_posv",
-    "spp_dense_posv_masked", "spp_tile_mask_host", "spp_schur_tile_mask_host", "spp_tail_order_host",
+    "spp_dense_posv_masked", "spp_tile_mask_host", "spp_schur_tile_mask_host", "spp_tail_order_host", "spp_schur_cam_order_host",
     "spp_dense_gemm_tn_sub", "spp_dense_gemm_tn_sub_upper", "spp_dense_front_factor", "spp_version",
 ]
 
@@ -99,6 +99,7 @@
         "spp_tile_mask_host": (cint, [i64, cint, i64, vp, vp, cint, cint, vp, vp]),
         "spp_schur_tile_mask_host": (cint, [i64, vp, vp, vp, cint, cint, vp]),
         "spp_tail_order_host": (cint, [i64, cint, vp, i64, cint, cint, dbl, vp, vp]),
+        "spp_schur_cam_order_host": (cint, [i64, vp, vp, vp, cint, cint, cint, vp, vp, vp]),
         "spp_dense_gemm_tn_sub": (cint, [vp, i64, i64, i64, vp, i64, vp, i64, vp, i64]),
         "spp_dense_gemm_tn_sub_upper": (cint, [vp, i64, i64, i64, vp, i64, vp, i64, vp, i64]),
         "spp_dense_front_factor": (cint, [vp, vp, i64, i64, i64, vp]),
@@ -170,6 +171,28 @@
     if code < 0:
         raise SppError("spp_schur_tile_mask_host failed: %d" % code)
     return words[:code].copy()
+
+
+def schur_cam_order_host(lam, order=None, sparse_S=False, mis=False, shard_rank=0, shard_world=1):
+    lib = load_library()
+    col_ptr = np.ascontiguousarray(lam.col_ptr, dtype=np.int64)
+    row_idx = np.ascontiguousarray(lam.row_idx, dtype=np.int64)
+    dim = np.ascontiguousarray(lam.dim, dtype=np.int32)
+    nc = int((dim == dim.max()).sum()) if not mis else int(dim.size)
+    out = np.full(max(nc, 1), -1, dtype=np.int64)
+    fig = np.zeros(8, dtype=np.float64)
+    oin = None if order is None else np.ascontiguousarray(order, dtype=np.int64)
+    if oin is not None and oin.size != nc:
+        raise SppError("schur_cam_order_host: order must list every camera once")
+    code = lib.spp_schur_cam_order_host(lam.nb, _ptr(dim), _ptr(col_ptr), _ptr(row_idx), shard_rank, shard_world,
+                                        (1 if sparse_S else 0) | (2 if mis else 0),
+                                        _ptr(oin) if oin is not None else None, _ptr(out), _ptr(fig))
+    if code < 0:
+        raise SppError("spp_schur_cam_order_host failed: %d" % code)
+    keys = ("tiles", "updates", "path", "cost_us")
+    natural = dict(zip(keys, (int(fig[0]), int(fig[1]), int(fig[2]), float(fig[3]))))
+    chosen = dict(zip(keys, (int(fig[4]), int(fig[5]), int(fig[6]), float(fig[7]))))
+    return out[out >= 0], bool(code), natural, chosen
 
 
 def tail_order_host(n, words, has_rhs=True, resident=256, early=True, beta=0.0):
diff --git a/slam_plus_plus_amd/csrc/spp_api.cpp b/slam_plus_plus_amd/csrc/spp_api.cpp
--- a/slam_plus_plus_amd/csrc/spp_api.cpp
+++ b/slam_plus_plus_amd/csrc/spp_api.cpp
@@ -492,6 +492,48 @@
 	}
 }
 
+int spp_schur_cam_order_host(int64_t nb, const int32_t *dim, const int64_t *col_ptr, const int64_t *row_idx, int shard_rank,
+	int shard_world, int flags, const int64_t *order_in, int64_t *cam_order, double *figures)
+{
+	if(nb <= 0 || !dim || !col_ptr || !row_idx || !cam_order || !figures || shard_world < 1 || shard_rank < 0 || shard_rank >= shard_world)
+		return SPP_E_BADARG;
+	try {
+		Structure st;
+		if(!structure_of_pattern(nb, dim, col_ptr, row_idx, st))
+			return SPP_E_BADARG;
+		if(order_in) {
+			int64_t nc = 0;
+			const int dmax = *std::max_element(dim, dim + nb);
+			for(int64_t j = 0; j < nb; ++ j)
+				nc += dim[j] == dmax;
+			std::vector<char> seen((size_t)nc, 0);
+			for(int64_t q = 0; q < nc; ++ q) {
+				if(order_in[q] < 0 || order_in[q] >= nc || seen[order_in[q]])
+					return SPP_E_BADARG;
+				seen[order_in[q]] = 1;
+			}
+		}
+		std::vector<int32_t> order;
+		TileDagCost cost[2];
+		const bool used = schur_cam_order_host_probe(st, shard_rank, shard_world, (flags & 1) != 0, (flags & 2) != 0, order_in, order, cost);
+		for(size_t q = 0; q < order.size(); ++ q)
+			cam_order[q] = order[q];
+		for(int side = 0; side < 2; ++ side) {
+			figures[4 * side] = (double)cost[side].tiles;
+			figures[4 * side + 1] = (double)cost[side].updates;
+			figures[4 * side + 2] = (double)cost[side].path;
+			figures[4 * side + 3] = cost[side].cost_us;
+		}
+		return used ? 1 : 0;
+	} catch(const Error &e) {
+		return e.code;
+	} catch(const std::bad_alloc &) {
+		return SPP_E_NOMEM;
+	} catch(...) {
+		return SPP_E_HIP;
+	}
+}
+
 int spp_schur_buffer_size(const spp_ctx *ctx, int64_t *n_doubles)
 {
 	if(!ctx || !n_doubles)
diff --git a/slam_plus_plus_amd/csrc/spp_internal.h b/slam_plus_plus_amd/csrc/spp_internal.h
--- a/slam_plus_plus_amd/csrc/spp_internal.h
+++ b/slam_plus_plus_amd/csrc/spp_internal.h
@@ -176,7 +176,7 @@
 struct SaccItem {
 	int32_t beg, end;
 	int32_t kind;
-	int32_t pad;
+	int32_t a_tr;
 	int64_t dst;
 	int64_t aoff;
 };
@@ -368,6 +368,15 @@
 void tile_mask_mark(int64_t n, int bs, int64_t nblk, const int32_t *i1, const int32_t *i2, std::vector<uint64_t> &words);
 int64_t tile_mask_close(int64_t n, bool has_rhs, bool fill, std::vector<uint64_t> &words);
 void schur_tile_mask_host_probe(const Structure &st, int shard_rank, int shard_world, std::vector<uint64_t> &words);
+constexpr double TAIL_MODEL_STEP_US = 36.5, TAIL_MODEL_UPDATE_US = 2.0, TAIL_MODEL_START_US = 45.0;
+constexpr int TAIL_MODEL_RESIDENT = 256;
+struct TileDagCost {
+	int64_t tiles = 0, updates = 0, path = 0;
+	double cost_us = 0;
+};
+TileDagCost tile_dag_cost(int64_t n, const std::vector<uint64_t> &filled, int resident);
+bool schur_cam_order_host_probe(const Structure &st, int shard_rank, int shard_world, bool sparse_S, bool mis, const int64_t *order_in,
+	std::vector<int32_t> &cam_order, TileDagCost cost[2]);
 void tail_order_table(const std::vector<uint64_t> &bits, int Tr, int Tc, bool have_pre, double beta, int resident, bool early,
 	std::vector<int> &order, int *info);
 int dense_front_factor(spp_ctx *ctx, double *d_F, int64_t ld, int64_t w, int64_t h, double *d_image);
diff --git a/slam_plus_plus_amd/csrc/spp_schur.hip b/slam_plus_plus_amd/csrc/spp_schur.hip
--- a/slam_plus_plus_amd/csrc/spp_schur.hip
+++ b/slam_plus_plus_amd/csrc/spp_schur.hip
@@ -325,7 +325,7 @@
 	SaccItem r;
 	r.beg = r.end = 0;
 	r.kind = -1;
-	r.pad = 0;
+	r.a_tr = 0;
 	r.dst = 0;
 	r.aoff = -1;
 	if(idx < lim)
@@ -393,9 +393,10 @@
 		if(last) {
 			nn = sacc_load_item(items, (left > 2) ? idx + 2 * SACC_WAVES : lim, lim);
 			if(cur.aoff >= 0 && lane < NE2) {
-				aval0 = vals[cur.aoff + 2 * lane];
-				if(2 * lane + 1 < NE)
-					aval1 = vals[cur.aoff + 2 * lane + 1];
+				const int e0 = 2 * lane, e1 = 2 * lane + 1;
+				aval0 = vals[cur.aoff + (cur.a_tr ? e0 / DP + (e0 % DP) * DP : e0)];
+				if(e1 < NE)
+					aval1 = vals[cur.aoff + (cur.a_tr ? e1 / DP + (e1 % DP) * DP : e1)];
 			}
 		}
 		if constexpr(GLDS) {
@@ -610,6 +611,8 @@
 	const int64_t aoff = sblk_aoff[b];
 	if(add_A && aoff >= 0)
 		acc = vals[aoff + lane] + acc;
+	else if(add_A && aoff < -1)
+		acc = vals[(-2 - aoff) + lane / DP + (lane % DP) * DP] + acc;
 	if(sblk_voff) {
 		S[sblk_voff[b] + lane] = acc;
 		return;
diff --git a/slam_plus_plus_amd/csrc/spp_switches.h b/slam_plus_plus_amd/csrc/spp_switches.h
--- a/slam_plus_plus_amd/csrc/spp_switches.h
+++ b/slam_plus_plus_amd/csrc/spp_switches.h
@@ -43,6 +43,7 @@
 	int64_t sacc_tile_cols;
 	int sacc_xcd;
 	int sacc_chunk;
+	int schur_cam_order;
 	int backsubst_fused;
 
 	int mid_front_max;
@@ -111,6 +112,7 @@
 	w.sacc_tile_cols = env_i64("SPP_SACC_TILE_COLS", -2);
 	w.sacc_xcd = env_int("SPP_SACC_XCD", 1);
 	w.sacc_chunk = env_int("SPP_SACC_CHUNK", 1);
+	w.schur_cam_order = env_int("SPP_SCHUR_CAM_ORDER", 1);
 	w.backsubst_fused = env_int("SPP_BACKSUBST_FUSED", 1);
 
 	w.mid_front_max = std::max(128, std::min(MID_FRONT_MAX, env_int("SPP_MID_FRONT_MAX", 320)));
diff --git a/slam_plus_plus_amd/csrc/spp_symbolic.cpp b/slam_plus_plus_amd/csrc/spp_symbolic.cpp
--- a/slam_plus_plus_amd/csrc/spp_symbolic.cpp
+++ b/slam_plus_plus_amd/csrc/spp_symbolic.cpp
@@ -276,7 +276,7 @@
 		for(int64_t p = st.col_ptr[j]; p < st.col_ptr[j + 1]; ++ p) {
 			const int64_t i = st.row_idx[p];
 			if(!is_lm[i] && !is_lm[j])
-				mark(tiles_of(pose_of[i]), tiles_of(pose_of[j]));
+				mark(tiles_of(pose_of[i]), tiles_of(pose_of[j])), mark(tiles_of(pose_of[j]), tiles_of(pose_of[i]));
 			else if(!is_lm[i])
 				seen[j] |= tiles_of(pose_of[i]);
 			else if(!is_lm[j])
@@ -286,6 +286,300 @@
 		if(seen[j])
 			mark(seen[j], seen[j]);
 	tile_mask_close(n_red, true, true, words);
+}
+
+TileDagCost tile_dag_cost(int64_t n, const std::vector<uint64_t> &filled, int resident)
+{
+	TileDagCost c;
+	const int64_t Tr = (int64_t)filled.size();
+	std::vector<uint64_t> w(filled);
+	c.updates = tile_mask_close(n, true, true, w);
+	std::vector<int> depth((size_t)Tr, 1);
+	for(int64_t k = 0; k < Tr; ++ k) {
+		c.tiles += __builtin_popcountll(w[k]);
+		for(int64_t j = 0; j < k; ++ j)
+			if((w[j] >> k) & 1)
+				depth[k] = std::max(depth[k], depth[j] + 1);
+		c.path = std::max<int64_t>(c.path, depth[k]);
+	}
+	c.cost_us = std::max(c.path * TAIL_MODEL_STEP_US, c.updates * TAIL_MODEL_UPDATE_US / std::max(1, resident)) + TAIL_MODEL_START_US;
+	return c;
+}
+
+struct CamGraph {
+	int64_t nc = 0, nw = 0;
+	std::vector<uint64_t> bits;
+	uint64_t *row(int64_t c) { return bits.data() + c * nw; }
+	const uint64_t *row(int64_t c) const { return bits.data() + c * nw; }
+};
+
+static void cam_graph(const Structure &st, const std::vector<uint8_t> &is_lm, const std::vector<int32_t> &cam_of, int64_t nc, CamGraph &g)
+{
+	g.nc = nc;
+	g.nw = (nc + 63) / 64;
+	g.bits.assign((size_t)(nc * g.nw), 0);
+	auto set = [&](int64_t a, int64_t b) { g.row(a)[b >> 6] |= 1ull << (b & 63); };
+	std::vector<int64_t> ptr((size_t)st.nb + 1, 0);
+	for(int64_t j = 0; j < st.nb; ++ j)
+		for(int64_t p = st.col_ptr[j]; p < st.col_ptr[j + 1]; ++ p) {
+			const int64_t i = st.row_idx[p];
+			if(is_lm[i] != is_lm[j])
+				++ ptr[(is_lm[i] ? i : j) + 1];
+		}
+	for(int64_t j = 0; j < st.nb; ++ j)
+		ptr[j + 1] += ptr[j];
+	std::vector<int32_t> obs((size_t)ptr[st.nb]);
+	{
+		std::vector<int64_t> fill(ptr.begin(), ptr.end() - 1);
+		for(int64_t j = 0; j < st.nb; ++ j)
+			for(int64_t p = st.col_ptr[j]; p < st.col_ptr[j + 1]; ++ p) {
+				const int64_t i = st.row_idx[p];
+				if(!is_lm[i] && !is_lm[j]) {
+					set(cam_of[i], cam_of[j]);
+					set(cam_of[j], cam_of[i]);
+				} else if(is_lm[i] != is_lm[j])
+					obs[fill[is_lm[i] ? i : j] ++] = cam_of[is_lm[i] ? j : i];
+			}
+	}
+	const int nt = plan_threads((int64_t)obs.size() * 4);
+	std::vector<int64_t> lcut;
+	balanced_cuts(ptr, nt, lcut);
+	std::vector<std::vector<uint64_t> > img((size_t)nt);
+	run_threads(nt, [&](int t) {
+		std::vector<uint64_t> &im = img[t];
+		im.assign(g.bits.size(), 0);
+		std::vector<uint64_t> tmp((size_t)g.nw, 0);
+		for(int64_t l = lcut[t]; l < lcut[t + 1]; ++ l) {
+			const int64_t b = ptr[l], e = ptr[l + 1];
+			if(b == e)
+				continue;
+			int64_t lo = g.nw, hi = -1;
+			for(int64_t q = b; q < e; ++ q) {
+				const int64_t w = obs[q] >> 6;
+				tmp[w] |= 1ull << (obs[q] & 63);
+				lo = std::min(lo, w);
+				hi = std::max(hi, w);
+			}
+			for(int64_t q = b; q < e; ++ q) {
+				uint64_t *r = im.data() + obs[q] * g.nw;
+				for(int64_t w = lo; w <= hi; ++ w)
+					r[w] |= tmp[w];
+			}
+			for(int64_t w = lo; w <= hi; ++ w)
+				tmp[w] = 0;
+		}
+	});
+	for(int t = 0; t < nt; ++ t)
+		for(size_t q = 0; q < g.bits.size(); ++ q)
+			g.bits[q] |= img[t][q];
+	for(int64_t c = 0; c < nc; ++ c)
+		set(c, c);
+}
+
+static void cam_graph_mask(const CamGraph &g, const std::vector<int32_t> &pos, int dp, int64_t n_red, std::vector<uint64_t> &words)
+{
+	tile_mask_mark(n_red, dp, 0, nullptr, nullptr, words);
+	if(words.empty())
+		return;
+	const int64_t Tr = (int64_t)words.size();
+	std::vector<uint64_t> tl((size_t)g.nc);
+	for(int64_t c = 0; c < g.nc; ++ c)
+		tl[c] = (1ull << ((int64_t)pos[c] * dp / DENSE_NB)) | (1ull << (((int64_t)pos[c] * dp + dp - 1) / DENSE_NB));
+	for(int64_t c = 0; c < g.nc; ++ c) {
+		uint64_t cols = 0;
+		const uint64_t *r = g.row(c);
+		for(int64_t w = 0; w < g.nw; ++ w)
+			for(uint64_t m = r[w]; m; m &= m - 1)
+				cols |= tl[w * 64 + __builtin_ctzll(m)];
+		for(uint64_t rows = tl[c]; rows; rows &= rows - 1) {
+			const int a = __builtin_ctzll(rows);
+			if(a < Tr)
+				words[a] |= cols;
+		}
+	}
+	tile_mask_close(n_red, true, true, words);
+}
+
+static bool cam_order_live_ok(const std::vector<uint64_t> &filled, int64_t n_red)
+{
+	const int Tr = (int)filled.size(), Tc = (int)(n_red / DENSE_NB + 1);
+	std::vector<uint64_t> bits((size_t)Tr + 1);
+	bits[0] = Tc == 64 ? ~0ull : (1ull << Tc) - 1;
+	for(int i = 0; i < Tr; ++ i)
+		bits[(size_t)i + 1] = filled[i];
+	std::vector<int> order;
+	int info[5];
+	tail_order_table(bits, Tr, Tc, false, 0.0, TAIL_MODEL_RESIDENT, true, order, info);
+	return info[0] > 0 || info[3] <= TAIL_MODEL_RESIDENT;
+}
+
+static bool cam_dissect(const CamGraph &g, int dp, int64_t n_red, std::vector<int32_t> &order, TileDagCost cost[2])
+{
+	const int64_t nc = g.nc, nw = g.nw;
+	order.resize((size_t)nc);
+	std::vector<int32_t> pos((size_t)nc);
+	for(int64_t c = 0; c < nc; ++ c)
+		order[c] = pos[c] = (int32_t)c;
+	std::vector<uint64_t> words;
+	cam_graph_mask(g, pos, dp, n_red, words);
+	if(words.empty())
+		return false;
+	cost[0] = cost[1] = tile_dag_cost(n_red, words, TAIL_MODEL_RESIDENT);
+	int64_t al = DENSE_NB;
+	for(int64_t x = dp, y = DENSE_NB; y; ) {
+		const int64_t t = x % y;
+		x = y;
+		y = t;
+		if(!y)
+			al = DENSE_NB / x;
+	}
+	typedef std::vector<uint64_t> Set;
+	auto count = [&](const Set &x) { int64_t n = 0; for(int64_t w = 0; w < nw; ++ w) n += __builtin_popcountll(x[w]); return n; };
+	auto nbrs = [&](const Set &x, Set &out) {
+		out.assign((size_t)nw, 0);
+		for(int64_t w = 0; w < nw; ++ w)
+			for(uint64_t m = x[w]; m; m &= m - 1) {
+				const uint64_t *r = g.row(w * 64 + __builtin_ctzll(m));
+				for(int64_t v = 0; v < nw; ++ v)
+					out[v] |= r[v];
+			}
+	};
+	auto flood = [&](const Set &within, Set &comp) {
+		Set front(comp), nb;
+		for(;;) {
+			nbrs(front, nb);
+			bool grew = false;
+			for(int64_t w = 0; w < nw; ++ w) {
+				front[w] = nb[w] & within[w] & ~comp[w];
+				comp[w] |= front[w];
+				grew = grew || front[w];
+			}
+			if(!grew)
+				return;
+		}
+	};
+	auto first_bit = [&](const Set &x, Set &seed) {
+		seed.assign((size_t)nw, 0);
+		for(int64_t w = 0; w < nw; ++ w)
+			if(x[w]) {
+				seed[w] = x[w] & (~x[w] + 1);
+				return true;
+			}
+		return false;
+	};
+	Set all((size_t)nw, 0);
+	for(int64_t c = 0; c < nc; ++ c)
+		all[c >> 6] |= 1ull << (c & 63);
+	if(!((g.row(0)[(nc - 1) >> 6] >> ((nc - 1) & 63)) & 1))
+		return false;
+	struct Cand { int64_t shorter = 0, sep = 0, runs = 0, a = 0, m = 0; } best;
+	Set A((size_t)nw), S, B((size_t)nw), bestA, bestB, comp;
+	const int64_t stride = std::max<int64_t>(1, al / 8);
+	for(int64_t m = al; 2 * m <= nc; m += al)
+		for(int64_t a = 0; a + m <= nc; a += stride) {
+			std::fill(A.begin(), A.end(), 0);
+			for(int64_t c = a; c < a + m; ++ c)
+				A[c >> 6] |= 1ull << (c & 63);
+			nbrs(A, S);
+			for(int64_t w = 0; w < nw; ++ w) {
+				S[w] &= ~A[w];
+				B[w] = all[w] & ~A[w] & ~S[w];
+			}
+			const int64_t nB = count(B), nBal = nB - nB % al;
+			if(nBal == 0)
+				continue;
+			Cand cd;
+			cd.shorter = std::min(m, nBal);
+			cd.sep = nc - m - nBal;
+			cd.a = a;
+			cd.m = m;
+			for(int64_t c = 0; c < nc; ++ c)
+				cd.runs += ((B[c >> 6] >> (c & 63)) & 1) && !(c && ((B[(c - 1) >> 6] >> ((c - 1) & 63)) & 1));
+			if(best.m && !(cd.shorter > best.shorter || (cd.shorter == best.shorter && (cd.sep < best.sep ||
+			   (cd.sep == best.sep && cd.runs < best.runs)))))
+				continue;
+			first_bit(B, comp);
+			flood(B, comp);
+			if(comp != B)
+				continue;
+			best = cd;
+			bestA = A;
+			bestB = B;
+		}
+	if(switches().verbose)
+		fprintf(stderr, "[spp] camera order: best arc a %lld m %lld shorter %lld sep %lld runs %lld\n", (long long)best.a,
+			(long long)best.m, (long long)best.shorter, (long long)best.sep, (long long)best.runs);
+	if(!best.m)
+		return false;
+	const int64_t nBal = count(bestB) - count(bestB) % al;
+	std::vector<int32_t> cand_order;
+	cand_order.reserve((size_t)nc);
+	std::vector<uint8_t> placed((size_t)nc, 0);
+	for(int64_t c = 0; c < nc; ++ c)
+		if((bestA[c >> 6] >> (c & 63)) & 1) {
+			cand_order.push_back((int32_t)c);
+			placed[c] = 1;
+		}
+	for(int64_t c = 0, k = 0; c < nc && k < nBal; ++ c)
+		if((bestB[c >> 6] >> (c & 63)) & 1) {
+			cand_order.push_back((int32_t)c);
+			placed[c] = 1;
+			++ k;
+		}
+	for(int64_t c = 0; c < nc; ++ c)
+		if(!placed[c])
+			cand_order.push_back((int32_t)c);
+	for(int64_t q = 0; q < nc; ++ q)
+		pos[cand_order[q]] = (int32_t)q;
+	cam_graph_mask(g, pos, dp, n_red, words);
+	const TileDagCost c1 = tile_dag_cost(n_red, words, TAIL_MODEL_RESIDENT);
+	const bool live_ok = cam_order_live_ok(words, n_red);
+	if(switches().verbose)
+		fprintf(stderr, "[spp] camera order: candidate tiles %lld updates %lld chain %lld model %.0f us (natural %.0f), live ok %d\n",
+			(long long)c1.tiles, (long long)c1.updates, (long long)c1.path, c1.cost_us, cost[0].cost_us, (int)live_ok);
+	if(!(c1.cost_us <= 0.9 * cost[0].cost_us) || !live_ok)
+		return false;
+	cost[1] = c1;
+	order.swap(cand_order);
+	return true;
+}
+
+static bool schur_cam_order(const Structure &st, const std::vector<uint8_t> &is_lm, const std::vector<int32_t> &cam_of, int64_t nc,
+	int dp, bool sparse_S, bool mis, const int64_t *order_in, std::vector<int32_t> &cam_order, TileDagCost cost[2])
+{
+	cam_order.resize((size_t)nc);
+	for(int64_t c = 0; c < nc; ++ c)
+		cam_order[c] = (int32_t)c;
+	cost[0] = cost[1] = TileDagCost();
+	const int64_t n_red = nc * dp;
+	if(sparse_S || mis || n_red / DENSE_NB + 1 > 64 || nc < 2 || (!order_in && !switches().schur_cam_order))
+		return false;
+	VClock clk("camera order");
+	CamGraph g;
+	cam_graph(st, is_lm, cam_of, nc, g);
+	clk.lap("co-visibility graph");
+	if(order_in) {
+		std::vector<int32_t> pos((size_t)nc);
+		for(int64_t q = 0; q < nc; ++ q) {
+			cam_order[q] = (int32_t)order_in[q];
+			pos[order_in[q]] = (int32_t)q;
+		}
+		std::vector<uint64_t> words;
+		for(int side = 0; side < 2; ++ side) {
+			if(!side)
+				for(int64_t c = 0; c < nc; ++ c)
+					pos[c] = (int32_t)c;
+			else
+				for(int64_t q = 0; q < nc; ++ q)
+					pos[order_in[q]] = (int32_t)q;
+			cam_graph_mask(g, pos, dp, n_red, words);
+			cost[side] = tile_dag_cost(n_red, words, TAIL_MODEL_RESIDENT);
+		}
+		return false;
+	}
+	const bool used = cam_dissect(g, dp, n_red, cam_order, cost);
+	clk.lap("dissection + cost model");
+	return used;
 }
 
 struct SchurPlanHost {
@@ -304,6 +598,7 @@
 	std::vector<SaccItem> recs;
 	Structure s_st;
 	std::vector<uint64_t> tile_mask;
+	TileDagCost cam_cost[2];
 };
 
 static void schur_plan_host(const Structure &st, int shard_rank, int shard_world, bool sparse_S, bool mis, SchurPlanHost &h)
@@ -342,6 +637,22 @@
 	h.nc = nc;
 	h.nl = nl;
 	h.nl_total = nl_total;
+	{
+		std::vector<int32_t> cam_order;
+		if(schur_cam_order(st, is_lm, pose_of, nc, dp, sparse_S, mis, nullptr, cam_order, h.cam_cost)) {
+			const std::vector<int64_t> natural(h.pose_block);
+			for(int64_t q = 0; q < nc; ++ q) {
+				h.pose_block[q] = natural[cam_order[q]];
+				pose_of[h.pose_block[q]] = (int32_t)q;
+			}
+			if(switches().verbose)
+				fprintf(stderr, "[spp] camera order: tiles %lld -> %lld, updates %lld -> %lld, chain %lld -> %lld, model %.0f -> %.0f us\n",
+					(long long)h.cam_cost[0].tiles, (long long)h.cam_cost[1].tiles, (long long)h.cam_cost[0].updates,
+					(long long)h.cam_cost[1].updates, (long long)h.cam_cost[0].path, (long long)h.cam_cost[1].path,
+					h.cam_cost[0].cost_us, h.cam_cost[1].cost_us);
+		}
+		clk.lap("camera order");
+	}
 	const bool add_A = (shard_rank == 0);
 	h.n_red = nc * dp;
 	h.ld = ((h.n_red + 1 + DENSE_NB - 1) / DENSE_NB) * DENSE_NB;
@@ -411,8 +722,10 @@
 			for(int64_t j = jcut[t]; j < jcut[t + 1]; ++ j)
 				for(int64_t p = st.col_ptr[j]; p < st.col_ptr[j + 1]; ++ p) {
 					const int k = classify(j, p, o);
-					if(k == 0)
-						ablk[q ++] = {pose_of[st.row_idx[p]], pose_of[j], st.blk_off[p]};
+					if(k == 0) {
+						const int32_t pi = pose_of[st.row_idx[p]], pj = pose_of[j];
+						ablk[q ++] = pi <= pj ? ABlk{pi, pj, st.blk_off[p]} : ABlk{pj, pi, -2 - st.blk_off[p]};
+					}
 					else if(k == 1) {
 						if(lm_of[j] >= 0)
 							lm_coff[lm_of[j]] = st.blk_off[p];
@@ -472,7 +785,32 @@
 	}
 	const int64_t no = (int64_t)obs_pose.size();
 	h.no = no;
-	if(!obs_sorted) {
+	bool lm_sorted = true;
+	for(int64_t a = 1; a < no && lm_sorted; ++ a)
+		lm_sorted = obs_lm[a - 1] <= obs_lm[a];
+	if(!obs_sorted && lm_sorted) {
+		const int nts2 = plan_threads(no);
+		run_threads(nts2, [&](int t) {
+			int64_t a = no * t / nts2, a1 = no * (t + 1) / nts2;
+			while(a > 0 && a < no && obs_lm[a] == obs_lm[a - 1])
+				++ a;
+			std::vector<std::pair<int32_t, int64_t> > run;
+			while(a < a1) {
+				int64_t e = a + 1;
+				while(e < no && obs_lm[e] == obs_lm[a])
+					++ e;
+				run.clear();
+				for(int64_t q = a; q < e; ++ q)
+					run.push_back(std::make_pair(obs_pose[q], obs_off[q]));
+				std::sort(run.begin(), run.end());
+				for(int64_t q = a; q < e; ++ q) {
+					obs_pose[q] = run[q - a].first;
+					obs_off[q] = run[q - a].second;
+				}
+				a = e;
+			}
+		});
+	} else if(!obs_sorted) {
 		std::vector<Obs> obs(no);
 		for(int64_t a = 0; a < no; ++ a)
 			obs[a] = {obs_lm[a], obs_pose[a], obs_off[a]};
@@ -641,7 +979,7 @@
 				int64_t out = b0;
 				for(int64_t c = i1; c < nc; ++ c) {
 					start[c] = out;
-					if(col_cnt[c + 1] || a_of_col[c] >= 0 || foreign[c]) {
+					if(col_cnt[c + 1] || a_of_col[c] != -1 || foreign[c]) {
 						ro.i1.push_back((int32_t)i1);
 						ro.i2.push_back((int32_t)c);
 						ro.aoff.push_back(a_of_col[c]);
@@ -834,13 +1172,17 @@
 		SaccItem &r = h.recs[q];
 		r.beg = item_beg[q];
 		r.end = item_end[q];
-		r.pad = 0;
+		r.a_tr = 0;
 		r.aoff = -1;
 		if(item_slot[q] >= 0) {
 			r.kind = 2;
 			r.dst = (int64_t)item_slot[q] * dp * dp;
 		} else {
 			r.aoff = add_A ? sblk_aoff[b] : -1;
+			if(r.aoff < -1) {
+				r.aoff = -2 - r.aoff;
+				r.a_tr = 1;
+			}
 			if(sparse_S) {
 				r.kind = 1;
 				r.dst = h.sblk_voff[b];
@@ -972,7 +1314,7 @@
 	for(size_t q = 0; q < h.recs.size(); ++ q) {
 		mix(((uint64_t)(uint32_t)h.recs[q].beg << 32) | (uint32_t)h.recs[q].end);
 		mix((uint64_t)h.recs[q].dst);
-		mix((uint64_t)h.recs[q].aoff + (uint64_t)h.recs[q].kind);
+		mix((uint64_t)h.recs[q].aoff + (uint64_t)h.recs[q].kind + ((uint64_t)h.recs[q].a_tr << 8));
 	}
 	for(size_t q = 0; q < h.xb.size(); ++ q)
 		mix((uint64_t)h.xb[q]);
@@ -983,9 +1325,51 @@
 
 void schur_tile_mask_host_probe(const Structure &st, int shard_rank, int shard_world, std::vector<uint64_t> &words)
 {
-	SchurPlanHost h;
-	schur_plan_host(st, shard_rank, shard_world, false, false, h);
-	words.swap(h.tile_mask);
+	(void)shard_rank;
+	(void)shard_world;
+	int dp, dl;
+	SPP_REQUIRE(schur_applicable(st, &dp, &dl), SPP_E_UNSUPPORTED,
+		"Schur mode needs exactly two block widths ({6,3} or {3,2}) and a block-diagonal landmark part");
+	std::vector<uint8_t> is_lm(st.nb);
+	std::vector<int32_t> pose_of(st.nb, -1);
+	int64_t nc = 0;
+	for(int64_t j = 0; j < st.nb; ++ j)
+		if(!(is_lm[j] = st.dim[j] == dl))
+			pose_of[j] = (int32_t)nc ++;
+	schur_tile_mask(st, is_lm, pose_of, dp, nc * dp, words);
+}
+
+bool schur_cam_order_host_probe(const Structure &st, int shard_rank, int shard_world, bool sparse_S, bool mis, const int64_t *order_in,
+	std::vector<int32_t> &cam_order, TileDagCost cost[2])
+{
+	if(!order_in) {
+		SchurPlanHost h;
+		schur_plan_host(st, shard_rank, shard_world, sparse_S || mis, mis, h);
+		std::vector<int32_t> cam_of(st.nb, -1);
+		int32_t nc = 0;
+		for(int64_t j = 0; j < st.nb; ++ j)
+			if(!h.is_lm[j])
+				cam_of[j] = nc ++;
+		cam_order.resize((size_t)nc);
+		bool used = false;
+		for(int32_t q = 0; q < nc; ++ q) {
+			cam_order[q] = cam_of[h.pose_block[q]];
+			used = used || cam_order[q] != q;
+		}
+		cost[0] = h.cam_cost[0];
+		cost[1] = h.cam_cost[1];
+		return used;
+	}
+	int dp, dl;
+	SPP_REQUIRE(!sparse_S && !mis && schur_applicable(st, &dp, &dl), SPP_E_UNSUPPORTED,
+		"the model of a given camera order needs the dense guided Schur mode ({6,3} or {3,2} block widths)");
+	std::vector<uint8_t> is_lm(st.nb, 0);
+	std::vector<int32_t> cam_of(st.nb, -1);
+	int64_t nc = 0;
+	for(int64_t j = 0; j < st.nb; ++ j)
+		if(!(is_lm[j] = st.dim[j] == dl))
+			cam_of[j] = (int32_t)nc ++;
+	return schur_cam_order(st, is_lm, cam_of, nc, dp, false, false, order_in, cam_order, cost);
 }
 
 void min_degree_order(int64_t nb, const int64_t *col_ptr, const int64_t *row_idx, std::vector<int64_t> &order)
```

Result: faster. 1.262 billion block-nnz/s (median of 6 runs) (+5.8%).
